# aksiksi/needle

Measured on AMD Instinct MI355X. Metric: episode-pairs/sec (analyze+search), higher is better.
Workload: dtype f64-certified (f32 first pass)

## Files before the change

include/needle_hip.h:

```cpp
#ifndef NEEDLE_HIP_H
#define NEEDLE_HIP_H

#include "needle.h"

#ifdef __cplusplus
extern "C" {
#endif

enum NeedleError needle_hip_device_count(int *count);
enum NeedleError needle_hip_set_device(int ordinal);
enum NeedleError needle_hip_synchronize(void);
enum NeedleError needle_hip_device_pci_bus_id(char out[32]);
void *needle_hip_stream(void);
const char *needle_hip_last_error_message(void);
const char *needle_hip_version(void);

enum NeedleError needle_hip_malloc(void **device_ptr, size_t bytes);
enum NeedleError needle_hip_free(void *device_ptr);
enum NeedleError needle_hip_memcpy_h2d(void *device_dst, const void *host_src, size_t bytes);
enum NeedleError needle_hip_memcpy_d2h(void *host_dst, const void *device_src, size_t bytes);
void needle_hip_host_free(void *ptr);
enum NeedleError needle_hip_host_alloc(void **host_ptr, size_t bytes);
enum NeedleError needle_hip_host_alloc_free(void *host_ptr);

double needle_hip_last_kernel_ms(const char *kernel);
void needle_hip_set_kernel_timing(const char *kernels);
size_t needle_hip_kernel_launches(const char *kernel);
enum NeedleError needle_hip_int_valu_ceiling(double *cells_per_second);
enum NeedleError needle_hip_scan_issued_evaluations(uint64_t *lane_evaluations, bool reset);
enum NeedleError needle_hip_scan_counts(uint64_t counts[2], bool reset);
enum NeedleError needle_hip_scan_last_launch(int32_t *form, uint64_t *matrix_products);
enum NeedleError needle_hip_epilogue_host_fallbacks(uint64_t *jobs, bool reset);

#define NEEDLE_HIP_MAX_CHANNELS 8
int needle_hip_fingerprint_sample_rate(void);
int needle_hip_fingerprint_delay_ms(void);
int needle_hip_fingerprint_item_duration_ms(void);
size_t needle_hip_fingerprint_num_items(size_t samples_per_channel);
size_t needle_hip_fingerprint_num_kept(size_t samples_per_channel, uint32_t step);

enum NeedleError needle_hip_fingerprint_host(const int16_t *const *pcm, const size_t *num_values,
                                             size_t num_streams, int channels, uint32_t step,
                                             uint32_t *const *items);

enum NeedleError needle_hip_fingerprint_device(const int16_t *d_pcm, const uint64_t *pcm_offsets,
                                               const uint64_t *num_values, size_t num_streams,
                                               int channels, uint32_t step, uint32_t *d_items,
                                               const uint64_t *item_offsets, bool sync);

enum NeedleError needle_hip_fingerprint_cert_stats(uint64_t counts[4], bool reset);

typedef struct NeedleHipCertAudit {
  uint64_t items, accepted, accepted_mismatches, mismatches;
  double max_error_over_s, max_s;
} NeedleHipCertAudit;
enum NeedleError needle_hip_fingerprint_audit_device(const int16_t *d_pcm, const uint64_t *pcm_offsets,
                                                     const uint64_t *num_values, size_t num_streams, int channels,
                                                     uint32_t step, const uint32_t *d_items, const uint64_t *item_offsets,
                                                     NeedleHipCertAudit *audit);

enum NeedleError needle_hip_fingerprint_debug(const int16_t *pcm, size_t num_values, int channels,
                                              double *chroma, double *features);

size_t needle_hip_resample_out_len(size_t samples_per_channel, int sample_rate);
enum NeedleError needle_hip_resample_host(const int16_t *const *pcm, const size_t *num_values, size_t num_streams,
                                          int channels, int sample_rate, int16_t *const *out);
enum NeedleHipResampleFamily {
  NEEDLE_HIP_RESAMPLE_IDENTITY = 0,
  NEEDLE_HIP_RESAMPLE_DEC = 1,
  NEEDLE_HIP_RESAMPLE_MFMA = 2,
  NEEDLE_HIP_RESAMPLE_QUAD = 3,
  NEEDLE_HIP_RESAMPLE_GENERAL = 4,
  NEEDLE_HIP_RESAMPLE_REFUSED = 5
};
typedef struct NeedleHipResamplePlan {
  int family;
  int L, M, T;
  int tile_outputs;
  int blocks_per_tile;
  int threads;
  int lds_bytes;
  int n;
  int row_mode;
  int rows_in_lds;
  int vec4;
  int groups;
  int pitch;
  int region_slots;
  int delta;
  int mfma_steps;
  int nblocks;
  int mf_splits, mf_waves, mf_groups;
  int mf_long_row;
  int mf_dup_lo, mf_dup_hi;
  int quad_splits, quads_per_split, quad_threads;
  int quad_rounds;
  int quad_small;
  int quad_steps;
  int dec_q;
} NeedleHipResamplePlan;
enum NeedleError needle_hip_resample_plan(int sample_rate, NeedleHipResamplePlan *out);
enum NeedleError needle_hip_downmix_host(const int16_t *const *pcm, const size_t *num_values, size_t num_streams,
                                         int channels, int16_t *const *out);

enum NeedleHipSampleFormat {
  NEEDLE_HIP_SAMPLE_U8 = 0,
  NEEDLE_HIP_SAMPLE_S16 = 1,
  NEEDLE_HIP_SAMPLE_S32 = 2,
  NEEDLE_HIP_SAMPLE_F32 = 3,
  NEEDLE_HIP_SAMPLE_F64 = 4,
  NEEDLE_HIP_SAMPLE_U8P = 5,
  NEEDLE_HIP_SAMPLE_S16P = 6,
  NEEDLE_HIP_SAMPLE_S32P = 7,
  NEEDLE_HIP_SAMPLE_F32P = 8,
// ... 61 lines not shown
  bool has_ending;
  uint64_t opening_start_ns, opening_end_ns;
  uint64_t ending_start_ns, ending_end_ns;
} NeedleHipSearchResult;

enum NeedleError needle_hip_comparator_run_with_frame_hashes(const struct NeedleAudioComparator *comparator,
                                                             const FrameHashes *const *frame_hashes,
                                                             size_t num_videos, bool display,
                                                             bool use_skip_files, bool write_skip_files,
                                                             NeedleHipSearchResult *results);

enum NeedleError needle_hip_comparator_results_from_runs(const struct NeedleAudioComparator *comparator,
                                                         const FrameHashes *const *frame_hashes, size_t num_videos,
                                                         const NeedleHipRun *runs, size_t num_runs, size_t first_video,
                                                         size_t video_count, NeedleHipSearchResult *results);

typedef struct NeedleHipIndex NeedleHipIndex;
enum NeedleError needle_hip_index_new(const struct NeedleAudioComparator *comparator, NeedleHipIndex **output);
void needle_hip_index_free(NeedleHipIndex *index);
size_t needle_hip_index_len(const NeedleHipIndex *index);
enum NeedleError needle_hip_index_add(NeedleHipIndex *index, const FrameHashes *const *frame_hashes, size_t k);
enum NeedleError needle_hip_index_results(const NeedleHipIndex *index, NeedleHipSearchResult *results, size_t n);
enum NeedleError needle_hip_index_pairs_searched(const NeedleHipIndex *index, uint64_t *total, uint64_t *last);
enum NeedleError needle_hip_index_remove(NeedleHipIndex *index, const size_t *positions, size_t k);
enum NeedleError needle_hip_index_replace(NeedleHipIndex *index, const size_t *positions, const FrameHashes *const *frame_hashes,
                                          size_t k);
enum NeedleError needle_hip_index_store_sizes(const NeedleHipIndex *index, uint64_t sizes[4]);

typedef struct NeedleHipLibrary NeedleHipLibrary;

enum NeedleError needle_hip_library_new(size_t num_videos, float opening_search_percentage, float hash_duration,
                                        NeedleHipLibrary **output);
void needle_hip_library_free(NeedleHipLibrary *library);
enum NeedleError needle_hip_library_include_endings(NeedleHipLibrary *library, float ending_search_percentage);
enum NeedleError needle_hip_library_set_sample_rate(NeedleHipLibrary *library, int sample_rate);
enum NeedleError needle_hip_library_set_sample_format(NeedleHipLibrary *library, int format);
size_t needle_hip_library_rows_per_video(const NeedleHipLibrary *library);
enum NeedleError needle_hip_library_set_pcm(NeedleHipLibrary *library, const int16_t *const *pcm,
                                            const size_t *num_values, int channels);
enum NeedleError needle_hip_library_set_pcm_device(NeedleHipLibrary *library, const int16_t *const *d_pcm,
                                                   const size_t *num_values, int channels);
enum NeedleError needle_hip_library_stream_pcm(NeedleHipLibrary *library, const int16_t *const *pcm,
                                               const size_t *num_values, int channels);
enum NeedleError needle_hip_library_analyze(NeedleHipLibrary *library, size_t first, size_t count, bool sync);
enum NeedleError needle_hip_library_hash_arena(NeedleHipLibrary *library, uint32_t **d_arena, size_t *stride);
enum NeedleError needle_hip_library_use_hash_arena(NeedleHipLibrary *library, uint32_t *d_arena, size_t rows,
                                                   size_t stride);
size_t needle_hip_library_num_pairs(const NeedleHipLibrary *library);
enum NeedleError needle_hip_library_search(NeedleHipLibrary *library, const struct NeedleAudioComparator *comparator,
                                           size_t first_pair, size_t num_pairs, NeedleHipRun *d_runs,
                                           uint32_t capacity, uint32_t *d_count, bool sync);
enum NeedleError needle_hip_library_fetch_runs_begin(NeedleHipLibrary *library, int slot, const NeedleHipRun *d_runs,
                                                     const uint32_t *d_count, uint32_t max_runs);
enum NeedleError needle_hip_library_fetch_runs_end(NeedleHipLibrary *library, int slot, const NeedleHipRun **runs,
                                                   uint32_t *num_runs);
enum NeedleError needle_hip_library_finalize(NeedleHipLibrary *library, const struct NeedleAudioComparator *comparator,
                                             const NeedleHipRun *runs, size_t num_runs,
                                             NeedleHipSearchResult *results);
enum NeedleError needle_hip_library_audit(NeedleHipLibrary *library, NeedleHipCertAudit *audit);
enum NeedleError needle_hip_library_frame_hashes(NeedleHipLibrary *library, size_t index, FrameHashes **output);

#define NEEDLE_HIP_COMM_ID_BYTES 128
enum NeedleError needle_hip_comm_create_id(uint8_t id[NEEDLE_HIP_COMM_ID_BYTES]);
enum NeedleError needle_hip_comm_init(const uint8_t id[NEEDLE_HIP_COMM_ID_BYTES], int rank, int world_size);
void needle_hip_comm_finalize(void);
int needle_hip_comm_rank(void);
int needle_hip_comm_world_size(void);
const char *needle_hip_comm_backend(void);
enum NeedleError needle_hip_comm_barrier(void);
enum NeedleError needle_hip_comm_all_gather_host(const void *send, void *recv, size_t bytes_per_rank);
void needle_hip_comm_shard(size_t units, int world_size, int rank, size_t *first, size_t *count);

enum NeedleError needle_hip_library_rank_videos(const NeedleHipLibrary *library, const size_t *num_values, int channels,
                                                int world_size, int rank, size_t *first_video, size_t *video_count);

enum NeedleError needle_hip_library_job_begin(NeedleHipLibrary *library, const struct NeedleAudioComparator *comparator,
                                              int slot);
enum NeedleError needle_hip_library_job_end(NeedleHipLibrary *library, const struct NeedleAudioComparator *comparator,
                                            int slot, NeedleHipSearchResult *results, size_t *num_runs);
enum NeedleError needle_hip_library_job_runs(const NeedleHipLibrary *library, int slot, const NeedleHipRun **runs,
                                             size_t *num_runs);
enum NeedleError needle_hip_library_job_comm_bytes(const NeedleHipLibrary *library, int slot, uint64_t bytes[4]);
enum NeedleError needle_hip_library_job_form(const NeedleHipLibrary *library, int slot, uint32_t form[4]);
int needle_hip_host_threads(void);

typedef struct NeedleHipFeeder NeedleHipFeeder;
enum NeedleError needle_hip_feeder_new(size_t lanes, int channels, int sample_rate, int format, uint32_t step,
                                       NeedleHipFeeder **output);
void needle_hip_feeder_free(NeedleHipFeeder *feeder);
enum NeedleError needle_hip_feeder_feed(NeedleHipFeeder *feeder, const void *const *pcm, const size_t *num_values);
enum NeedleError needle_hip_feeder_finish(NeedleHipFeeder *feeder, const size_t *lanes, size_t k);
enum NeedleError needle_hip_feeder_reset(NeedleHipFeeder *feeder, const size_t *lanes, size_t k);
enum NeedleError needle_hip_feeder_ready(NeedleHipFeeder *feeder, size_t lane, size_t *kept_items,
                                         uint64_t *samples_per_channel_fed, bool *finished);
enum NeedleError needle_hip_feeder_items(NeedleHipFeeder *feeder, size_t lane, size_t first, size_t count, uint32_t *items);
enum NeedleError needle_hip_feeder_frame_hashes(NeedleHipFeeder *feeder, size_t opening_lane, size_t ending_lane,
                                                uint64_t ending_seek_ns, float hash_duration, const char *md5, FrameHashes **output);
enum NeedleError needle_hip_feeder_state_bytes(const NeedleHipFeeder *feeder, uint64_t bytes[2]);
enum NeedleError needle_hip_feeder_set_audit(NeedleHipFeeder *feeder, bool on);
enum NeedleError needle_hip_feeder_audit(NeedleHipFeeder *feeder, size_t lane, NeedleHipCertAudit *audit);
size_t needle_hip_feeder_num_ready(uint64_t samples_per_channel_fed, int sample_rate, int channels, uint32_t step, bool finished);

typedef struct NeedleHipLaneFormat {
  int32_t channels;
  int32_t sample_rate;
  int32_t format;
} NeedleHipLaneFormat;
enum NeedleError needle_hip_feeder_new_lanes(const NeedleHipLaneFormat *formats, size_t lanes, uint32_t step, NeedleHipFeeder **output);
enum NeedleError needle_hip_feeder_lane_format(const NeedleHipFeeder *feeder, size_t lane, NeedleHipLaneFormat *format);
enum NeedleError needle_hip_feeder_reset_format(NeedleHipFeeder *feeder, const size_t *lanes, const NeedleHipLaneFormat *formats, size_t k);
enum NeedleError needle_hip_convert_mono_host(const void *const *pcm, const size_t *num_values, const NeedleHipLaneFormat *formats,
                                              size_t num_streams, int16_t *const *out);

typedef struct NeedleHipChannelMix {
  int32_t channels;
  int32_t coef[2][NEEDLE_HIP_MAX_CHANNELS];
} NeedleHipChannelMix;
enum NeedleError needle_hip_channel_mix_default(uint32_t channel_mask, NeedleHipChannelMix *out);
enum NeedleError needle_hip_rematrix_host(const void *const *pcm, const size_t *num_values, const NeedleHipLaneFormat *formats,
                                          const NeedleHipChannelMix *mixes, size_t num_streams, int16_t *const *out);
enum NeedleError needle_hip_analyzer_set_channel_mix(struct NeedleAudioAnalyzer *analyzer, const NeedleHipChannelMix *mix);
enum NeedleError needle_hip_analyzer_set_layout_downmix(struct NeedleAudioAnalyzer *analyzer, bool on);
enum NeedleError needle_hip_comparator_set_layout_downmix(struct NeedleAudioComparator *comparator, bool on);
enum NeedleError needle_hip_library_set_channel_mix(NeedleHipLibrary *library, const NeedleHipChannelMix *mix);
enum NeedleError needle_hip_feeder_set_lane_mix(NeedleHipFeeder *feeder, const size_t *lanes, const NeedleHipChannelMix *mixes, size_t k);

enum NeedleError needle_hip_feeder_switch_format(NeedleHipFeeder *feeder, const size_t *lanes, const NeedleHipLaneFormat *formats,
                                                 const NeedleHipChannelMix *mixes, size_t k);
typedef struct NeedleHipSegment {
  NeedleHipLaneFormat format;
  uint64_t frames;
} NeedleHipSegment;
enum NeedleError needle_hip_feeder_lane_segments(const NeedleHipFeeder *feeder, size_t lane, NeedleHipSegment *out, size_t cap, size_t *count);
size_t needle_hip_feeder_num_ready_segments(const NeedleHipSegment *segments, size_t count, uint32_t step, bool finished);

typedef struct NeedleHipMatcher NeedleHipMatcher;
enum NeedleError needle_hip_matcher_new(const uint32_t *hashes, size_t num_hashes, const NeedleHipSeq *sources,
                                        const uint32_t *min_len, size_t num_sources, size_t lanes, uint32_t threshold,
                                        NeedleHipMatcher **output);
void needle_hip_matcher_free(NeedleHipMatcher *matcher);
enum NeedleError needle_hip_matcher_feed(NeedleHipMatcher *matcher, const uint32_t *const *items, const size_t *num_items);
enum NeedleError needle_hip_matcher_feed_from_feeder(NeedleHipMatcher *matcher, NeedleHipFeeder *feeder);
enum NeedleError needle_hip_matcher_finish(NeedleHipMatcher *matcher, const size_t *lanes, size_t k);
enum NeedleError needle_hip_matcher_reset(NeedleHipMatcher *matcher, const size_t *lanes, size_t k);
enum NeedleError needle_hip_matcher_ready(NeedleHipMatcher *matcher, size_t lane, size_t *num_runs, uint64_t *items_fed,
                                          bool *finished);
enum NeedleError needle_hip_matcher_runs(NeedleHipMatcher *matcher, size_t lane, size_t first, size_t count, NeedleHipRun *runs);
enum NeedleError needle_hip_matcher_open(NeedleHipMatcher *matcher, size_t lane, NeedleHipRun **runs, size_t *num_runs);
enum NeedleError needle_hip_matcher_stats(const NeedleHipMatcher *matcher, uint64_t stats[4]);

typedef struct NeedleHipCrossMatcher NeedleHipCrossMatcher;
enum NeedleError needle_hip_crossmatcher_new(size_t lanes, size_t max_items, uint32_t min_len, uint32_t threshold,
                                             NeedleHipCrossMatcher **output);
enum NeedleError needle_hip_crossmatcher_new_regions(size_t videos, size_t regions, const size_t *max_items, const uint32_t *min_len,
                                                     uint32_t threshold, NeedleHipCrossMatcher **output);
enum NeedleError needle_hip_crossmatcher_new_resident(const uint32_t *hashes, size_t num_hashes, const NeedleHipSeq *resident,
                                                      size_t num_resident, size_t videos, size_t regions, const size_t *max_items,
                                                      const uint32_t *min_len, uint32_t threshold, NeedleHipCrossMatcher **output);
void needle_hip_crossmatcher_free(NeedleHipCrossMatcher *matcher);
enum NeedleError needle_hip_crossmatcher_feed(NeedleHipCrossMatcher *matcher, const uint32_t *const *items, const size_t *num_items);
enum NeedleError needle_hip_crossmatcher_feed_from_feeder(NeedleHipCrossMatcher *matcher, NeedleHipFeeder *feeder);
enum NeedleError needle_hip_crossmatcher_finish(NeedleHipCrossMatcher *matcher, const size_t *lanes, size_t k);
enum NeedleError needle_hip_crossmatcher_ready(NeedleHipCrossMatcher *matcher, size_t *num_runs, bool *complete);
enum NeedleError needle_hip_crossmatcher_lane(NeedleHipCrossMatcher *matcher, size_t lane, uint64_t *items_fed, bool *finished);
enum NeedleError needle_hip_crossmatcher_runs(NeedleHipCrossMatcher *matcher, size_t first, size_t count, NeedleHipRun *runs);
enum NeedleError needle_hip_crossmatcher_stats(const NeedleHipCrossMatcher *matcher, uint64_t stats[4]);
// ... 19 lines not shown
```

needle_amd/capi.py:

```python
from __future__ import annotations

import ctypes as C
import os
from dataclasses import dataclass
from typing import List, Optional, Sequence, Tuple

import numpy as np

NS = 1_000_000_000
LIB_PATH = os.environ.get("NEEDLE_CAPI_LIB") or os.path.join(os.path.dirname(os.path.abspath(__file__)), "lib", "libneedle_capi.so")

ERROR_NAMES = ["Ok", "InvalidUtf8String", "NullArgument", "InvalidArgument", "FrameHashDataNotFound",
               "FrameHashDataInvalidVersion", "InvalidFrameHashData", "ComparatorMinimumPaths",
               "AnalyzerInvalidHashPeriod", "AnalyzerInvalidHashDuration", "IOError", "Unknown"]

DEFAULT_HASH_MATCH_THRESHOLD = 10
DEFAULT_OPENING_SEARCH_PERCENTAGE = 0.50
DEFAULT_ENDING_SEARCH_PERCENTAGE = 0.25
DEFAULT_MIN_OPENING_DURATION = 20
DEFAULT_MIN_ENDING_DURATION = 20
DEFAULT_HASH_DURATION = 0.3
MAX_CHANNELS = 8


class NeedleError(RuntimeError):
    def __init__(self, code: int, detail: str = ""):
        self.code = code
        self.name = ERROR_NAMES[code] if 0 <= code < len(ERROR_NAMES) else str(code)
        super().__init__(f"NeedleError_{self.name}: {detail}")


class Seq(C.Structure):
    _fields_ = [("offset", C.c_uint32), ("len", C.c_uint32)]


class Problem(C.Structure):
    _fields_ = [("src_seq", C.c_uint32), ("dst_seq", C.c_uint32), ("min_len", C.c_uint32), ("tag", C.c_uint32)]


class Run(C.Structure):
    _fields_ = [("problem", C.c_uint32), ("src_end", C.c_uint32), ("dst_end", C.c_uint32), ("len", C.c_uint32),
                ("src_match_hash", C.c_uint32), ("dst_match_hash", C.c_uint32)]


class CSearchResult(C.Structure):
    _fields_ = [("has_result", C.c_bool), ("has_opening", C.c_bool), ("has_ending", C.c_bool),
                ("opening_start_ns", C.c_uint64), ("opening_end_ns", C.c_uint64),
                ("ending_start_ns", C.c_uint64), ("ending_end_ns", C.c_uint64)]


RUN_DTYPE = np.dtype([("problem", "<u4"), ("src_end", "<u4"), ("dst_end", "<u4"), ("len", "<u4"),
                      ("src_match_hash", "<u4"), ("dst_match_hash", "<u4")])
RUN_WORDS = 6

NEEDLE_H_SYMBOLS = [
    "needle_error_to_str", "needle_util_find_video_files", "needle_util_video_files_free",
    "needle_audio_analyzer_new_default", "needle_audio_analyzer_new", "needle_audio_analyzer_get_frame_hashes",
    "needle_audio_analyzer_free", "needle_audio_analyzer_print_paths", "needle_audio_analyzer_run",
    "needle_audio_comparator_new_default", "needle_audio_comparator_new", "needle_audio_comparator_free",
    "needle_audio_comparator_run"]
NEEDLE_HIP_H_SYMBOLS = [
    "needle_hip_device_count", "needle_hip_set_device", "needle_hip_synchronize", "needle_hip_stream",
    "needle_hip_device_pci_bus_id", "needle_hip_fingerprint_cert_stats", "needle_hip_scan_issued_evaluations",
    "needle_hip_last_error_message",
    "needle_hip_version", "needle_hip_malloc", "needle_hip_free", "needle_hip_memcpy_h2d", "needle_hip_memcpy_d2h",
    "needle_hip_host_free", "needle_hip_last_kernel_ms", "needle_hip_set_kernel_timing", "needle_hip_kernel_launches", "needle_hip_fingerprint_sample_rate",
    "needle_hip_fingerprint_delay_ms", "needle_hip_fingerprint_item_duration_ms", "needle_hip_fingerprint_num_items",
    "needle_hip_fingerprint_num_kept", "needle_hip_fingerprint_host", "needle_hip_fingerprint_device",
    "needle_hip_fingerprint_debug", "needle_hip_resample_out_len", "needle_hip_resample_host", "needle_hip_resample_plan",
    "needle_hip_downmix_host",
    "needle_hip_hamming_runs_device", "needle_hip_hamming_runs_host",
    "needle_hip_frame_hashes_new", "needle_hip_frame_hashes_free", "needle_hip_frame_hashes_len",
    "needle_hip_frame_hashes_copy", "needle_hip_frame_hashes_hash_duration_ns", "needle_hip_frame_hashes_md5",
    "needle_hip_frame_hashes_read", "needle_hip_frame_hashes_write", "needle_hip_header_md5",
    "needle_hip_analyzer_run_pcm", "needle_hip_comparator_run_with_frame_hashes", "needle_hip_library_new",
    "needle_hip_library_free", "needle_hip_library_include_endings", "needle_hip_library_set_sample_rate",
    "needle_hip_library_rows_per_video",
    "needle_hip_library_set_pcm", "needle_hip_library_set_pcm_device", "needle_hip_library_rank_videos",
    "needle_hip_library_analyze",
    "needle_hip_library_hash_arena", "needle_hip_library_use_hash_arena", "needle_hip_library_num_pairs", "needle_hip_library_search",
    "needle_hip_library_fetch_runs_begin", "needle_hip_library_fetch_runs_end",
    "needle_hip_library_finalize", "needle_hip_library_frame_hashes",
    "needle_hip_comm_create_id", "needle_hip_comm_init", "needle_hip_comm_finalize", "needle_hip_comm_rank",
    "needle_hip_comm_world_size", "needle_hip_comm_backend", "needle_hip_comm_barrier",
    "needle_hip_comm_all_gather_host", "needle_hip_comm_shard", "needle_hip_library_job_begin",
    "needle_hip_library_job_end", "needle_hip_library_stream_pcm", "needle_hip_host_alloc",
    "needle_hip_host_alloc_free", "needle_hip_int_valu_ceiling",
    "needle_hip_comparator_results_from_runs", "needle_hip_library_job_runs", "needle_hip_library_job_comm_bytes",
    "needle_hip_library_job_form",
    "needle_hip_host_threads", "needle_hip_fingerprint_audit_device", "needle_hip_library_audit",
    "needle_hip_scan_counts", "needle_hip_scan_last_launch", "needle_hip_epilogue_host_fallbacks",
    "needle_hip_index_new", "needle_hip_index_free", "needle_hip_index_len", "needle_hip_index_add",
    "needle_hip_index_results", "needle_hip_index_pairs_searched", "needle_hip_index_remove", "needle_hip_index_replace",
    "needle_hip_index_store_sizes", "needle_hip_index_crossmatcher_new", "needle_hip_index_add_matched",
    "needle_hip_index_pairs_scanned",
    "needle_hip_convert_host", "needle_hip_analyzer_run_pcm_format", "needle_hip_library_set_sample_format",
    "needle_hip_feeder_new", "needle_hip_feeder_free", "needle_hip_feeder_feed", "needle_hip_feeder_finish",
    "needle_hip_feeder_reset", "needle_hip_feeder_ready", "needle_hip_feeder_items", "needle_hip_feeder_frame_hashes",
    "needle_hip_feeder_state_bytes", "needle_hip_feeder_num_ready", "needle_hip_feeder_set_audit", "needle_hip_feeder_audit",
    "needle_hip_feeder_new_lanes", "needle_hip_feeder_lane_format", "needle_hip_feeder_reset_format", "needle_hip_convert_mono_host",
    "needle_hip_channel_mix_default", "needle_hip_rematrix_host", "needle_hip_analyzer_set_channel_mix",
    "needle_hip_analyzer_set_layout_downmix", "needle_hip_comparator_set_layout_downmix", "needle_hip_library_set_channel_mix",
    "needle_hip_feeder_set_lane_mix",
    "needle_hip_feeder_switch_format", "needle_hip_feeder_lane_segments", "needle_hip_feeder_num_ready_segments",
    "needle_hip_matcher_new", "needle_hip_matcher_free", "needle_hip_matcher_feed", "needle_hip_matcher_feed_from_feeder",
    "needle_hip_matcher_finish", "needle_hip_matcher_reset", "needle_hip_matcher_ready", "needle_hip_matcher_runs",
    "needle_hip_matcher_open", "needle_hip_matcher_stats",
    "needle_hip_crossmatcher_new", "needle_hip_crossmatcher_free", "needle_hip_crossmatcher_feed",
    "needle_hip_crossmatcher_feed_from_feeder", "needle_hip_crossmatcher_finish", "needle_hip_crossmatcher_ready",
    "needle_hip_crossmatcher_lane", "needle_hip_crossmatcher_runs", "needle_hip_crossmatcher_stats",
    "needle_hip_crossmatcher_state_bytes", "needle_hip_crossmatcher_new_regions",
    "needle_hip_crossmatcher_state_bytes_regions", "needle_hip_crossmatcher_shape",
    "needle_hip_crossmatcher_new_resident", "needle_hip_crossmatcher_state_bytes_resident", "needle_hip_crossmatcher_resident"]

SAMPLE_U8, SAMPLE_S16, SAMPLE_S32, SAMPLE_F32, SAMPLE_F64 = 0, 1, 2, 3, 4
SAMPLE_U8P, SAMPLE_S16P, SAMPLE_S32P, SAMPLE_F32P, SAMPLE_F64P = 5, 6, 7, 8, 9
_SAMPLE_DTYPES = [np.uint8, np.int16, np.int32, np.float32, np.float64]


def sample_format_dtype(sample_format: int):
    if not 0 <= sample_format <= 9:
        raise ValueError(f"unknown sample format {sample_format}")
    return np.dtype(_SAMPLE_DTYPES[sample_format % 5])


def sample_format_planar(sample_format: int) -> bool:
    return sample_format >= SAMPLE_U8P


def _format_pointers(pcm, channels: int, sample_format: int):
    dtype = sample_format_dtype(sample_format)
    keep, ptrs = [], []
    for p in pcm:
        if not sample_format_planar(sample_format):
            a = None if p is None else np.ascontiguousarray(p, dtype=dtype)
            keep.append(a)
            ptrs.append(None if a is None else a.ctypes.data)
        elif p is None:
            ptrs += [None] * channels
        else:
            planes = [np.ascontiguousarray(q, dtype=dtype) for q in p]
            if len(planes) != channels:
                raise ValueError(f"a planar stream needs {channels} planes, got {len(planes)}")
            keep += planes
            ptrs += [q.ctypes.data for q in planes]
    return keep, ptrs


class CLaneFormat(C.Structure):
    _fields_ = [("channels", C.c_int32), ("sample_rate", C.c_int32), ("format", C.c_int32)]


class CSegment(C.Structure):
    _fields_ = [("format", CLaneFormat), ("frames", C.c_uint64)]


class ChannelMix(C.Structure):
    _fields_ = [("channels", C.c_int32), ("coef", (C.c_int32 * MAX_CHANNELS) * 2)]

    @classmethod
    def of(cls, left: Sequence[int], right: Sequence[int], channels: Optional[int] = None) -> "ChannelMix":
        if len(left) != len(right) or len(left) > MAX_CHANNELS:
            raise ValueError(f"two rows of at most {MAX_CHANNELS} coefficients each")
        m = cls()
        m.channels = len(left) if channels is None else channels
        for c, (l, r) in enumerate(zip(left, right)):
            m.coef[0][c], m.coef[1][c] = int(l), int(r)
        return m

    def rows(self) -> Tuple[List[int], List[int]]:
        n = max(0, min(self.channels, MAX_CHANNELS))
        return list(self.coef[0][:n]), list(self.coef[1][:n])
# ... 220 lines not shown
    L.needle_hip_crossmatcher_runs.argtypes = [vp, sz, sz, vp]
    L.needle_hip_crossmatcher_stats.argtypes = [vp, C.POINTER(u64)]
    L.needle_hip_crossmatcher_state_bytes.argtypes = [sz, sz]
    L.needle_hip_crossmatcher_state_bytes.restype = sz
    L.needle_hip_crossmatcher_new_regions.argtypes = [sz, sz, C.POINTER(sz), C.POINTER(u32), u32, C.POINTER(vp)]
    L.needle_hip_crossmatcher_state_bytes_regions.argtypes = [sz, sz, C.POINTER(sz)]
    L.needle_hip_crossmatcher_state_bytes_regions.restype = sz
    L.needle_hip_crossmatcher_shape.argtypes = [vp, C.POINTER(sz), C.POINTER(sz)]
    L.needle_hip_crossmatcher_new_resident.argtypes = [vp, sz, vp, sz, sz, sz, C.POINTER(sz), C.POINTER(u32), u32, C.POINTER(vp)]
    L.needle_hip_crossmatcher_state_bytes_resident.argtypes = [vp, sz, sz, sz, C.POINTER(sz)]
    L.needle_hip_crossmatcher_state_bytes_resident.restype = sz
    L.needle_hip_crossmatcher_resident.argtypes = [vp, C.POINTER(sz)]
    _LIB = L
    return L


def check(code: int) -> None:
    if code != 0:
        raise NeedleError(code, (lib().needle_hip_last_error_message() or b"").decode(errors="replace"))


def error_to_str(code: int) -> str:
    return lib().needle_error_to_str(code).decode()


def device_count() -> int:
    n = C.c_int(0)
    check(lib().needle_hip_device_count(C.byref(n)))
    return n.value


def set_device(ordinal: int) -> None:
    check(lib().needle_hip_set_device(ordinal))


def device_pci_bus_id() -> str:
    buf = C.create_string_buffer(32)
    lib().needle_hip_device_pci_bus_id.argtypes = [C.c_char_p]
    check(lib().needle_hip_device_pci_bus_id(buf))
    return buf.value.decode()


def synchronize() -> None:
    check(lib().needle_hip_synchronize())


def stream_ptr() -> int:
    L = lib()
    L.needle_hip_stream.restype = C.c_void_p
    p = L.needle_hip_stream()
    if not p:
        raise RuntimeError("no HIP device: the library has no stream")
    return int(p)


def cert_stats(reset: bool = False) -> dict:
    v = (C.c_uint64 * 4)()
    lib().needle_hip_fingerprint_cert_stats.argtypes = [C.POINTER(C.c_uint64), C.c_bool]
    check(lib().needle_hip_fingerprint_cert_stats(v, reset))
    return {"items": int(v[0]), "items_recomputed": int(v[1]), "chunks": int(v[2]), "chunks_recomputed": int(v[3])}


def scan_issued_evaluations(reset: bool = False) -> int:
    v = C.c_uint64(0)
    lib().needle_hip_scan_issued_evaluations.argtypes = [C.POINTER(C.c_uint64), C.c_bool]
    check(lib().needle_hip_scan_issued_evaluations(C.byref(v), reset))
    return int(v.value)


def scan_counts(reset: bool = False) -> Tuple[int, int]:
    c = (C.c_uint64 * 2)()
    lib().needle_hip_scan_counts.argtypes = [C.POINTER(C.c_uint64), C.c_bool]
    check(lib().needle_hip_scan_counts(c, reset))
    return int(c[0]), int(c[1])


def scan_last_launch() -> Tuple[int, int]:
    form, products = C.c_int32(0), C.c_uint64(0)
    lib().needle_hip_scan_last_launch.argtypes = [C.POINTER(C.c_int32), C.POINTER(C.c_uint64)]
    check(lib().needle_hip_scan_last_launch(C.byref(form), C.byref(products)))
    return int(form.value), int(products.value)


def epilogue_host_fallbacks(reset: bool = False) -> int:
    jobs = C.c_uint64(0)
    lib().needle_hip_epilogue_host_fallbacks.argtypes = [C.POINTER(C.c_uint64), C.c_bool]
    check(lib().needle_hip_epilogue_host_fallbacks(C.byref(jobs), reset))
    return int(jobs.value)


def host_threads() -> int:
    lib().needle_hip_host_threads.restype = C.c_int
    return int(lib().needle_hip_host_threads())


def int_valu_ceiling() -> float:
    v = C.c_double(0.0)
    lib().needle_hip_int_valu_ceiling.argtypes = [C.POINTER(C.c_double)]
    check(lib().needle_hip_int_valu_ceiling(C.byref(v)))
    return v.value


def last_kernel_ms(name: str) -> float:
    return lib().needle_hip_last_kernel_ms(name.encode())


def kernel_launches(name: str) -> int:
    return int(lib().needle_hip_kernel_launches(name.encode()))


def set_kernel_timing(kernels: Optional[str]) -> None:
    lib().needle_hip_set_kernel_timing(kernels.encode() if kernels else None)


def _paths(paths: Sequence[str]):
    arr = (C.c_char_p * max(len(paths), 1))(*[p.encode() if isinstance(p, str) else p for p in paths])
    return C.cast(arr, C.POINTER(C.c_char_p)), arr


def header_md5(path: str) -> str:
    buf = C.create_string_buffer(33)
    check(lib().needle_hip_header_md5(path.encode(), buf))
    return buf.value.decode()


class FrameHashes:

    def __init__(self, handle: int, owned: bool, keepalive=None):
        self._h = C.c_void_p(handle)
        self._owned = owned
        self._keep = keepalive

    @staticmethod
    def new(opening: Sequence[Tuple[int, int]], ending: Sequence[Tuple[int, int]] = (), hash_duration_ns: int = 0,
            md5: str = "") -> "FrameHashes":
        oh = np.array([h for h, _ in opening], dtype=np.uint32)
        ot = np.array([t for _, t in opening], dtype=np.uint64)
        eh = np.array([h for h, _ in ending], dtype=np.uint32)
        et = np.array([t for _, t in ending], dtype=np.uint64)
        out = C.c_void_p()
        check(lib().needle_hip_frame_hashes_new(oh.ctypes.data, ot.ctypes.data, len(oh), eh.ctypes.data,
                                                et.ctypes.data, len(eh), hash_duration_ns, md5.encode(),
                                                C.byref(out)))
        return FrameHashes(out.value, True)

    @staticmethod
    def from_path(path: str) -> "FrameHashes":
        out = C.c_void_p()
        check(lib().needle_hip_frame_hashes_read(path.encode(), C.byref(out)))
        return FrameHashes(out.value, True)

    def write(self, path: str) -> None:
        check(lib().needle_hip_frame_hashes_write(self._h, path.encode()))

    def _data(self, ending: bool):
        n = lib().needle_hip_frame_hashes_len(self._h, ending)
        hashes = np.zeros(max(n, 1), dtype=np.uint32)
        ts = np.zeros(max(n, 1), dtype=np.uint64)
        check(lib().needle_hip_frame_hashes_copy(self._h, ending, hashes.ctypes.data, ts.ctypes.data, n))
        return hashes[:n], ts[:n]

    def opening_data(self):
        return self._data(False)

    def ending_data(self):
        return self._data(True)
# ... 880 lines not shown
        ptrs = (C.c_void_p * max(len(d_ptrs), self.n))(*[None if p is None else int(p) for p in d_ptrs])
        lens = (C.c_size_t * self.n)(*list(num_values))
        lib().needle_hip_library_set_pcm_device.argtypes = [C.c_void_p, C.POINTER(C.c_void_p), C.POINTER(C.c_size_t), C.c_int]
        check(lib().needle_hip_library_set_pcm_device(self._h, ptrs, lens, channels))

    def stream_pcm(self, pcm: Sequence[Optional[np.ndarray]], num_values: Sequence[int], channels: int = 1) -> None:
        arrs, ptrs = self._host_pointers(pcm, channels)
        lens = (C.c_size_t * self.n)(*list(num_values))
        check(lib().needle_hip_library_stream_pcm(self._h, ptrs, lens, channels))

    def analyze(self, first: int = 0, count: Optional[int] = None, sync: bool = True) -> None:
        check(lib().needle_hip_library_analyze(self._h, first, self.n - first if count is None else count, sync))

    def hash_arena(self) -> Tuple[int, int]:
        ptr = C.c_void_p()
        stride = C.c_size_t(0)
        check(lib().needle_hip_library_hash_arena(self._h, C.byref(ptr), C.byref(stride)))
        return ptr.value, stride.value

    def use_hash_arena(self, d_ptr: int, rows: int, stride: int) -> None:
        check(lib().needle_hip_library_use_hash_arena(self._h, d_ptr, rows, stride))

    def num_pairs(self) -> int:
        return lib().needle_hip_library_num_pairs(self._h)

    def search(self, comparator: Comparator, first_pair: int, num_pairs: int, d_runs: int, capacity: int,
               d_count: int, sync: bool = True) -> None:
        check(lib().needle_hip_library_search(self._h, comparator._h or comparator.handle(), first_pair, num_pairs,
                                              d_runs, capacity, d_count, sync))

    def fetch_runs_begin(self, slot: int, d_runs: int, d_count: int, max_runs: int) -> None:
        check(lib().needle_hip_library_fetch_runs_begin(self._h, slot, d_runs, d_count, max_runs))

    def fetch_runs_end(self, slot: int, max_runs: int) -> Tuple[np.ndarray, int]:
        ptr = C.c_void_p()
        total = C.c_uint32(0)
        check(lib().needle_hip_library_fetch_runs_end(self._h, slot, C.byref(ptr), C.byref(total)))
        k = min(total.value, max_runs)
        out = np.zeros(k, dtype=RUN_DTYPE)
        if k:
            C.memmove(out.ctypes.data, ptr.value, k * RUN_DTYPE.itemsize)
        return out, total.value

    def finalize(self, comparator: Comparator, runs: np.ndarray) -> List[Optional[SearchResult]]:
        runs = np.ascontiguousarray(runs, dtype=RUN_DTYPE)
        res = (CSearchResult * self.n)()
        check(lib().needle_hip_library_finalize(self._h, comparator._h or comparator.handle(), runs.ctypes.data,
                                                runs.size, res))
        return _results(res, self.n)

    def frame_hashes(self, index: int) -> FrameHashes:
        out = C.c_void_p()
        check(lib().needle_hip_library_frame_hashes(self._h, index, C.byref(out)))
        return FrameHashes(out.value, True)

    def job_begin(self, comparator: Comparator, slot: int = 0) -> None:
        check(lib().needle_hip_library_job_begin(self._h, comparator._h or comparator.handle(), slot))

    def job_end(self, comparator: Comparator, slot: int = 0) -> Tuple[List[Optional[SearchResult]], int]:
        res = (CSearchResult * self.n)()
        found = C.c_size_t(0)
        check(lib().needle_hip_library_job_end(self._h, comparator._h or comparator.handle(), slot, res, C.byref(found)))
        return _results(res, self.n), found.value

    def audit(self) -> dict:
        a = CCertAudit()
        lib().needle_hip_library_audit.argtypes = [C.c_void_p, C.POINTER(CCertAudit)]
        check(lib().needle_hip_library_audit(self._h, C.byref(a)))
        return a.as_dict()

    def job_runs(self, slot: int = 0) -> np.ndarray:
        ptr, total = C.c_void_p(), C.c_size_t(0)
        lib().needle_hip_library_job_runs.argtypes = [C.c_void_p, C.c_int, C.POINTER(C.c_void_p), C.POINTER(C.c_size_t)]
        check(lib().needle_hip_library_job_runs(self._h, slot, C.byref(ptr), C.byref(total)))
        out = np.zeros(total.value, dtype=RUN_DTYPE)
        if total.value:
            C.memmove(out.ctypes.data, ptr.value, out.nbytes)
        return out

    def job_form(self, slot: int = 0) -> dict:
        f = (C.c_uint32 * 4)()
        lib().needle_hip_library_job_form.argtypes = [C.c_void_p, C.c_int, C.POINTER(C.c_uint32)]
        check(lib().needle_hip_library_job_form(self._h, slot, f))
        return {"device_epilogue": bool(f[0]), "sharded_epilogue": bool(f[1]), "directed_runs": bool(f[2]), "scan_form": int(f[3])}

    def job_comm_bytes(self, slot: int = 0) -> dict:
        b = (C.c_uint64 * 4)()
        lib().needle_hip_library_job_comm_bytes.argtypes = [C.c_void_p, C.c_int, C.POINTER(C.c_uint64)]
        check(lib().needle_hip_library_job_comm_bytes(self._h, slot, b))
        return {"hash_rows": int(b[0]), "run_heads": int(b[1]), "results": int(b[2]), "scans_repeated": int(b[3])}

    def __del__(self):
        if getattr(self, "_h", None):
            lib().needle_hip_library_free(self._h)
            self._h = None


class PinnedArray:

    def __init__(self, count: int):
        p = C.c_void_p()
        check(lib().needle_hip_host_alloc(C.byref(p), max(count, 1) * 2))
        self.ptr = p.value
        self.array = np.ctypeslib.as_array((C.c_int16 * max(count, 1)).from_address(self.ptr))[:count]

    def __del__(self):
        if getattr(self, "ptr", None):
            self.array = None
            lib().needle_hip_host_alloc_free(self.ptr)
            self.ptr = None


class DeviceBuffer:

    def __init__(self, nbytes: int):
        p = C.c_void_p()
        check(lib().needle_hip_malloc(C.byref(p), nbytes))
        self.ptr = p.value
        self.nbytes = nbytes

    def to_host(self, dtype, count: int) -> np.ndarray:
        out = np.zeros(count, dtype=dtype)
        if count:
            check(lib().needle_hip_memcpy_d2h(out.ctypes.data, self.ptr, out.nbytes))
        return out

    def __del__(self):
        if getattr(self, "ptr", None):
            lib().needle_hip_free(self.ptr)
            self.ptr = None
```

needle_amd/csrc/capi.cpp:

```cpp
#include <dirent.h>
#include <hip/hip_runtime_api.h>
#include <sys/stat.h>

#include <algorithm>
#include <cstdio>
#include <cstdlib>
#include <chrono>
#include <cstring>
#include <fstream>
#include <new>

#include "crossmatch.h"
#include "epilogue.h"
#include "hipctx.h"
#include "feeder.h"
#include "index.h"
#include "matcher.h"
#include "needle_core.h"

using namespace needle;

struct FrameHashes {
  FrameHashesData d;
};
// ... 349 lines not shown

enum NeedleError needle_hip_malloc(void **device_ptr, size_t bytes) {
  if (!device_ptr) return NeedleError_NullArgument;
  return guarded([&]() -> NeedleError {
    Status s = ensure_device();
    if (!s.ok()) return report(s);
    if (hipMalloc(device_ptr, bytes ? bytes : 1) != hipSuccess)
      return report(Status::Make(NeedleError_Unknown, "hipMalloc failed for " + std::to_string(bytes) + " bytes"));
    return NeedleError_Ok;
  });
}

enum NeedleError needle_hip_free(void *device_ptr) {
  if (device_ptr && hipFree(device_ptr) != hipSuccess) return report(Status::Make(NeedleError_Unknown, "hipFree failed"));
  return NeedleError_Ok;
}

enum NeedleError needle_hip_memcpy_h2d(void *device_dst, const void *host_src, size_t bytes) {
  if (!device_dst || !host_src) return NeedleError_NullArgument;
  hipStream_t st = library_stream();
  if (hipMemcpyAsync(device_dst, host_src, bytes, hipMemcpyHostToDevice, st) != hipSuccess ||
      hipStreamSynchronize(st) != hipSuccess)
    return report(Status::Make(NeedleError_Unknown, "host-to-device copy failed"));
  return NeedleError_Ok;
}

enum NeedleError needle_hip_memcpy_d2h(void *host_dst, const void *device_src, size_t bytes) {
  if (!host_dst || !device_src) return NeedleError_NullArgument;
  hipStream_t st = library_stream();
  if (hipMemcpyAsync(host_dst, device_src, bytes, hipMemcpyDeviceToHost, st) != hipSuccess ||
      hipStreamSynchronize(st) != hipSuccess)
    return report(Status::Make(NeedleError_Unknown, "device-to-host copy failed"));
  return NeedleError_Ok;
}

void needle_hip_host_free(void *ptr) { std::free(ptr); }

enum NeedleError needle_hip_host_alloc(void **host_ptr, size_t bytes) {
  if (!host_ptr) return NeedleError_NullArgument;
  return guarded([&]() -> NeedleError {
    Status s = ensure_device();
    if (!s.ok()) return report(s);
    if (hipHostMalloc(host_ptr, bytes ? bytes : 1, hipHostMallocDefault) != hipSuccess)
      return report(Status::Make(NeedleError_Unknown, "pinned allocation of " + std::to_string(bytes) + " bytes failed"));
    return NeedleError_Ok;
  });
}

enum NeedleError needle_hip_host_alloc_free(void *host_ptr) {
  if (host_ptr && hipHostFree(host_ptr) != hipSuccess) return report(Status::Make(NeedleError_Unknown, "hipHostFree failed"));
  return NeedleError_Ok;
}

enum NeedleError needle_hip_fingerprint_cert_stats(uint64_t counts[4], bool reset) {
  if (!counts) return NeedleError_NullArgument;
  return guarded([&]() -> NeedleError {
    Status s = gpu_fingerprint_cert_stats(counts, reset);
    return s.ok() ? NeedleError_Ok : report(s);
  });
}

enum NeedleError needle_hip_scan_issued_evaluations(uint64_t *lane_evaluations, bool reset) {
  if (!lane_evaluations) return NeedleError_NullArgument;
  return guarded([&]() -> NeedleError {
    Status s = gpu_scan_issued_evaluations(lane_evaluations, reset);
    return s.ok() ? NeedleError_Ok : report(s);
  });
}

enum NeedleError needle_hip_scan_counts(uint64_t counts[2], bool reset) {
  if (!counts) return NeedleError_NullArgument;
  return guarded([&]() -> NeedleError {
    Status s = gpu_scan_issued_evaluations(&counts[0], reset, &counts[1]);
    return s.ok() ? NeedleError_Ok : report(s);
  });
}

enum NeedleError needle_hip_scan_last_launch(int32_t *form, uint64_t *matrix_products) {
  if (!form || !matrix_products) return NeedleError_NullArgument;
  gpu_scan_last_launch(form, matrix_products);
  return NeedleError_Ok;
}

enum NeedleError needle_hip_epilogue_host_fallbacks(uint64_t *jobs, bool reset) {
  if (!jobs) return NeedleError_NullArgument;
  *jobs = reset ? epilogue_host_fallbacks().exchange(0) : epilogue_host_fallbacks().load();
  return NeedleError_Ok;
}

enum NeedleError needle_hip_int_valu_ceiling(double *cells_per_second) {
  if (!cells_per_second) return NeedleError_NullArgument;
  return guarded([&]() -> NeedleError {
    Status s = gpu_int_valu_ceiling(cells_per_second);
    return s.ok() ? NeedleError_Ok : report(s);
  });
}

double needle_hip_last_kernel_ms(const char *kernel) { return kernel ? kernel_ms(kernel) : -1.0; }
void needle_hip_set_kernel_timing(const char *kernels) { set_kernel_timing(kernels); }
size_t needle_hip_kernel_launches(const char *kernel) { return kernel ? kernel_launches(kernel) : 0; }

int needle_hip_fingerprint_sample_rate(void) { return kSampleRate; }
int needle_hip_fingerprint_delay_ms(void) { return kDelayMs; }
int needle_hip_fingerprint_item_duration_ms(void) { return kItemDurationMs; }
size_t needle_hip_fingerprint_num_items(size_t samples_per_channel) { return num_items(samples_per_channel); }
size_t needle_hip_fingerprint_num_kept(size_t samples_per_channel, uint32_t step) {
  return num_kept(samples_per_channel, step);
}

enum NeedleError needle_hip_fingerprint_host(const int16_t *const *pcm, const size_t *num_values, size_t num_streams,
                                             int channels, uint32_t step, uint32_t *const *items) {
  if (!pcm || !num_values || !items) return NeedleError_NullArgument;
  return guarded([&]() -> NeedleError {
    std::vector<const int16_t *> p(pcm, pcm + num_streams);
    std::vector<size_t> n(num_values, num_values + num_streams);
    for (size_t i = 0; i < num_streams; i++)
      if ((!p[i] && n[i]) || !items[i]) return NeedleError_NullArgument;
    std::vector<std::vector<uint32_t>> out;
    Status s = gpu_fingerprint_host(p, n, channels, step, &out);
    if (!s.ok()) return report(s);
    for (size_t i = 0; i < num_streams; i++)
      if (!out[i].empty()) std::memcpy(items[i], out[i].data(), out[i].size() * sizeof(uint32_t));
    return NeedleError_Ok;
  });
}

enum NeedleError needle_hip_fingerprint_device(const int16_t *d_pcm, const uint64_t *pcm_offsets,
                                               const uint64_t *num_values, size_t num_streams, int channels,
                                               uint32_t step, uint32_t *d_items, const uint64_t *item_offsets,
                                               bool sync) {
  if (!d_pcm || !pcm_offsets || !num_values || !d_items || !item_offsets) return NeedleError_NullArgument;
  return guarded([&]() -> NeedleError {
    std::vector<StreamSpan> spans(num_streams);
    for (size_t i = 0; i < num_streams; i++) spans[i] = StreamSpan{pcm_offsets[i], num_values[i], item_offsets[i]};
    Status s = gpu_fingerprint_device(d_pcm, spans, channels, step, d_items, sync);
    return s.ok() ? NeedleError_Ok : report(s);
  });
}

enum NeedleError needle_hip_fingerprint_audit_device(const int16_t *d_pcm, const uint64_t *pcm_offsets, const uint64_t *num_values,
                                                     size_t num_streams, int channels, uint32_t step, const uint32_t *d_items,
                                                     const uint64_t *item_offsets, NeedleHipCertAudit *audit) {
  if (!d_pcm || !pcm_offsets || !num_values || !d_items || !item_offsets || !audit) return NeedleError_NullArgument;
  return guarded([&]() -> NeedleError {
    std::vector<StreamSpan> spans(num_streams);
    for (size_t i = 0; i < num_streams; i++) spans[i] = StreamSpan{pcm_offsets[i], num_values[i], item_offsets[i]};
    uint64_t c[4] = {0, 0, 0, 0};
    Status s = gpu_fingerprint_audit_device(d_pcm, spans, channels, step, d_items, c, &audit->max_error_over_s, &audit->max_s);
    if (!s.ok()) return report(s);
    audit->items = c[0];
    audit->accepted = c[1];
    audit->accepted_mismatches = c[2];
    audit->mismatches = c[3];
    return NeedleError_Ok;
  });
}

enum NeedleError needle_hip_fingerprint_debug(const int16_t *pcm, size_t num_values, int channels, double *chroma,
                                              double *features) {
  if (!pcm) return NeedleError_NullArgument;
  return guarded([&]() -> NeedleError {
    Status s = ensure_device();
    if (!s.ok()) return report(s);
    if (channels != 1 && channels != 2) return NeedleError_InvalidArgument;
    const size_t samples = num_values / (size_t)channels;
    const size_t frames = num_frames(samples), rows = frames >= 5 ? frames - 4 : 0, kept = num_items(samples);
// ... 867 lines not shown
```

needle_amd/csrc/common.h:

```cpp
#pragma once

#include <cstddef>
#include <cstdint>
#include <functional>
#include <string>
#include <vector>

#include "../../include/needle_hip.h"

struct ihipStream_t;

namespace needle {

struct Status {
  NeedleError code = NeedleError_Ok;
  std::string message;
  bool ok() const { return code == NeedleError_Ok; }
  static Status Ok() { return Status{}; }
  static Status Make(NeedleError c, std::string m) { return Status{c, std::move(m)}; }
};

NeedleError report(const Status &s);
void set_last_error(const std::string &m);
const char *last_error();
// ... 21 lines not shown

Status frame_hashes_read(const std::string &path, FrameHashesData *out);
Status frame_hashes_write(const std::string &path, const FrameHashesData &fh);
Status header_md5(const std::string &path, std::string *out);
std::string md5_hex(const uint8_t *data, size_t n);
std::string with_extension(const std::string &path, const std::string &ext);
std::string format_time(ns_t t);
std::string format_f32_json(float v);

unsigned usable_cpus();
unsigned host_threads();
void set_node_ranks(unsigned ranks);

constexpr int kSampleRate = 11025;
constexpr int kFrameSize = 4096;
constexpr int kHop = 1365;
constexpr int kBands = 12;
constexpr int kFirTaps = 5;
constexpr int kMaxFilterWidth = 16;
constexpr int kItemLatency = (kFirTaps - 1) + (kMaxFilterWidth - 1);
constexpr int kDelayMs = 2600;
constexpr int kItemDurationMs = 123;

inline size_t num_frames(size_t samples) { return samples < (size_t)kFrameSize ? 0 : (samples - kFrameSize) / kHop + 1; }
inline size_t num_items(size_t samples) {
  size_t f = num_frames(samples);
  return f > (size_t)kItemLatency ? f - kItemLatency : 0;
}
inline size_t num_kept(size_t samples, uint32_t step) {
  size_t n = num_items(samples);
  return step ? (n + step - 1) / step : 0;
}

bool step_for_hash_duration(ns_t hash_duration, uint32_t *step);
void attach_timestamps(const uint32_t *kept, size_t n_kept, uint32_t step, bool has_seek, ns_t seek_to,
                       std::vector<HashTs> *out);

struct WavData {
  int channels = 0;
  int sample_rate = 0;
  std::vector<int16_t> pcm;
};
Status wav_read(const std::string &path, WavData *out);
struct WavInfo {
  int channels = 0, sample_rate = 0;
  int format = 0, bits = 0;
  uint32_t channel_mask = 0;
  uint64_t data_offset = 0;
  uint64_t frames = 0;
};
Status wav_probe(const std::string &path, WavInfo *out);
Status wav_read_frames(const std::string &path, const WavInfo &info, uint64_t first, uint64_t count, int16_t *dst);

struct StreamSpan {
  uint64_t pcm_off;
  uint64_t num_values;
  uint64_t item_off;
};

Status gpu_fingerprint_device(const int16_t *d_pcm, const std::vector<StreamSpan> &streams, int channels,
                              uint32_t step, uint32_t *d_items, bool sync, double *d_chroma_dbg = nullptr,
                              double *d_feat_dbg = nullptr, size_t descriptor_slot = 0, int pipe = -1,
                              uint32_t *zero_word = nullptr, bool *zeroed = nullptr);
Status gpu_fingerprint_streamed_device(const std::vector<const int16_t *> &pcm, const std::vector<size_t> &num_values,
                                       int channels, uint32_t step, uint32_t *d_items,
                                       const std::vector<uint64_t> &item_off, int rate = kSampleRate);
Status gpu_fingerprint_host(const std::vector<const int16_t *> &pcm, const std::vector<size_t> &num_values,
                            int channels, uint32_t step, std::vector<std::vector<uint32_t>> *items,
                            int rate = kSampleRate);
using PcmReader = std::function<Status(size_t stream, uint64_t first_value, uint64_t num_values, int16_t *dst)>;
using StreamIssued = std::function<Status(size_t stream_index)>;
Status gpu_upload_pcm_streamed(const std::vector<size_t> &num_values, const std::vector<uint64_t> &dev_off,
                               const PcmReader &read, unsigned readers, int16_t *d_pcm, ::ihipStream_t *stream = nullptr,
                               const StreamIssued &issued = nullptr);
Status gpu_upload_pcm(const std::vector<const int16_t *> &pcm, const std::vector<size_t> &num_values,
                      const std::vector<uint64_t> &dev_off, int16_t *d_pcm, ::ihipStream_t *stream = nullptr,
                      const StreamIssued &issued = nullptr);
Status gpu_fingerprint_streamed(const std::vector<size_t> &num_values, const PcmReader &read, unsigned readers,
                                int channels, uint32_t step, std::vector<std::vector<uint32_t>> *items,
                                int rate = kSampleRate, const NeedleHipChannelMix *mix = nullptr);
Status gpu_hamming_runs_device(const uint32_t *d_hashes, const NeedleHipSeq *seqs, size_t num_seqs,
                               const NeedleHipProblem *problems, size_t num_problems, uint32_t threshold,
                               NeedleHipRun *d_runs, uint32_t capacity, uint32_t *d_count, bool sync,
                               bool count_is_zero = false);
Status gpu_hamming_runs_host(const uint32_t *hashes, size_t num_hashes, const NeedleHipSeq *seqs, size_t num_seqs,
                             const NeedleHipProblem *problems, size_t num_problems, uint32_t threshold,
                             std::vector<NeedleHipRun> *runs);

uint32_t *gpu_pinned_arena_acquire(size_t words);
void gpu_pinned_arena_release(uint32_t *arena);
void gpu_prefetch_hashes(const uint32_t *hashes, size_t num_hashes);

constexpr uint64_t kDeviceEpiloguePairs = 1u << 14;
constexpr uint32_t kDeviceEpilogueRuns = 1u << 14;

Status gpu_int_valu_ceiling(double *cells_per_second);
Status gpu_scan_issued_evaluations(uint64_t *lane_evaluations, bool reset, uint64_t *head_survivors = nullptr);
void gpu_scan_last_launch(int32_t *form, uint64_t *matrix_products);
Status gpu_fingerprint_cert_stats(uint64_t out[4], bool reset);
Status gpu_fingerprint_audit_device(const int16_t *d_pcm, const std::vector<StreamSpan> &spans, int channels, uint32_t step,
                                    const uint32_t *d_items, uint64_t out[4], double *max_ratio, double *max_sigma);

struct FeedLane {
  uint64_t pcm_off;
  uint64_t item_off;
  uint32_t row_base;
  uint32_t carried;
  uint32_t frames;
  uint32_t first_item;
  uint32_t kept;
  uint32_t lane;
};
constexpr size_t kFeedAuditWords = 6;
struct FeedAudit {
  double *rows64;
  uint64_t *counts;
};
Status gpu_fingerprint_feed_device(const int16_t *d_pcm, const std::vector<FeedLane> &lanes, int channels, uint32_t step,
                                   double *d_chroma, float *d_energy, double *d_chroma64, uint32_t *d_items,
                                   const FeedAudit *audit = nullptr);
bool gpu_fingerprint_f64_mode();

struct ResampleSpan {
  uint64_t in_off;
  uint64_t n_in;
  uint64_t out_off;
  const int16_t *src = nullptr;
  uint64_t t0 = 0, t1 = 0;
  uint64_t p0 = 0, p1 = 0;
};
size_t resample_out_len(size_t n_in, int rate);
struct ResampleTiling {
  int L = 1, M = 1, half = 0;
  uint64_t tile_outputs = 1;
};
Status resample_tiling(int rate, int channels, ResampleTiling *out);
Status resample_tiling_host(int rate, ResampleTiling *out);
Status resample_plan_host(int rate, NeedleHipResamplePlan *out);
void resample_piece(const ResampleTiling &t, uint64_t n_in, uint64_t t0, uint64_t t1, uint64_t *p0, uint64_t *p1);
Status gpu_resample_device(const int16_t *d_in, const std::vector<ResampleSpan> &spans, int channels, int rate,
                           int16_t *d_out, bool sync);
Status gpu_resample_host(const std::vector<const int16_t *> &pcm, const std::vector<size_t> &num_values, int channels,
                         int rate, std::vector<std::vector<int16_t>> *out);

struct DownmixSpan {
  const int16_t *src;
  int16_t *dst;
  uint64_t frames;
};
Status gpu_downmix_device(const std::vector<DownmixSpan> &spans, int channels, bool sync);
Status gpu_downmix_host(const std::vector<const int16_t *> &pcm, const std::vector<size_t> &num_values, int channels,
                        const std::vector<int16_t *> &out);

inline bool sample_format_valid(int format) { return format >= NEEDLE_HIP_SAMPLE_U8 && format <= NEEDLE_HIP_SAMPLE_F64P; }
inline bool sample_format_planar(int format) { return format >= NEEDLE_HIP_SAMPLE_U8P; }
inline size_t sample_format_width(int format) {
  constexpr size_t width[5] = {1, 2, 4, 4, 8};
  return width[format % 5];
}
inline size_t sample_format_planes(int format, int channels) { return sample_format_planar(format) ? (size_t)channels : 1; }
inline uint64_t sample_plane_units(uint64_t samples, size_t width) { return ((samples * width + 15) & ~(uint64_t)15) / 2; }
struct ConvertSpan {
  const void *src[NEEDLE_HIP_MAX_CHANNELS];
  int16_t *dst;
  uint64_t frames;
};
Status gpu_convert_device(const std::vector<ConvertSpan> &spans, int channels, int format, bool mix, bool sync);
Status gpu_upload_raw(const std::vector<const void *> &src, const std::vector<size_t> &bytes, const std::vector<uint64_t> &dev_off,
                      int16_t *d_raw, ::ihipStream_t *stream = nullptr, const StreamIssued &issued = nullptr);
Status gpu_fingerprint_host_format(const std::vector<const void *> &pcm, const std::vector<size_t> &num_values, int channels,
                                   int format, uint32_t step, std::vector<std::vector<uint32_t>> *items, int rate = kSampleRate,
                                   const NeedleHipChannelMix *mix = nullptr);
Status gpu_fingerprint_streamed_device_format(const std::vector<const void *> &pcm, const std::vector<size_t> &num_values,
                                              int channels, int format, uint32_t step, uint32_t *d_items,
                                              const std::vector<uint64_t> &item_off, int rate = kSampleRate,
                                              const NeedleHipChannelMix *mix = nullptr);
Status gpu_convert_host(const std::vector<const void *> &pcm, const std::vector<size_t> &num_values, int channels, int format,
                        const std::vector<int16_t *> &out);

struct IngestSpan {
  const void *src[NEEDLE_HIP_MAX_CHANNELS];
// ... 16 lines not shown
```

needle_amd/csrc/library.cpp:

```cpp
#include <hip/hip_runtime_api.h>

#include <algorithm>
#include <chrono>
#include <cstdio>
#include <cstdlib>
#include <cstring>
#include <map>
#include <new>
#include <tuple>

#include "comm.h"
#include "epilogue.h"
#include "hipctx.h"
#include "needle_core.h"

struct FrameHashes;
struct NeedleAudioComparator;

namespace needle {
const Comparator &comparator_of(const NeedleAudioComparator *c);
FrameHashes *make_frame_hashes(FrameHashesData &&d);
void fill_c_result(const VideoResult &v, NeedleHipSearchResult *r);
}

using namespace needle;

namespace {
struct Window {
  size_t values = 0;
  uint64_t pcm_off = ~0ull;
  uint32_t kept = 0;
  ns_t seek = 0;
};
}

struct NeedleHipLibrary {
  size_t n = 0;
  float opening_pct = DEFAULT_OPENING_SEARCH_PERCENTAGE;
  float ending_pct = DEFAULT_ENDING_SEARCH_PERCENTAGE;
  bool endings = false;
  ns_t hash_duration = 0;
  uint32_t step = 0;
  int channels = 1;
  int rate = kSampleRate;
  int format = NEEDLE_HIP_SAMPLE_S16;
  bool has_mix = false;
  NeedleHipChannelMix mix{};
  bool have_pcm = false;
  bool pcm_resident = false;
  std::vector<Window> win;
  size_t stride = 0;
  DeviceBuffer<int16_t> d_pcm;
  DeviceBuffer<uint32_t> d_arena;
  uint32_t *arena = nullptr;
  std::vector<std::vector<HashTs>> ts_cache;
  std::vector<uint32_t> min_len;
  ns_t min_len_for[2] = {~0ull, ~0ull};
  std::vector<NeedleHipProblem> problems;
  size_t problems_for[3] = {~(size_t)0, 0, 0};
  std::vector<FrameHashesData> shells;
  std::vector<uint32_t> shell_of;
  struct Fetch {
    void *host = nullptr;
    uint32_t max_runs = 0;
    hipEvent_t ready = nullptr, done = nullptr;
    const NeedleHipRun *d_runs = nullptr;
    const uint32_t *d_count = nullptr;
    bool pending = false;
  } fetch[2];
  struct Job {
    DeviceBuffer<uint8_t> d_slabs;
    DeviceBuffer<uint8_t> d_heads;
    uint32_t slab_runs = 0, head_runs = 0;
    int world = 0;
    void *host = nullptr;
    size_t host_bytes = 0;
    hipEvent_t searched = nullptr, done = nullptr;
    bool pending = false;
    std::vector<NeedleHipRun> merged;
    void *host_results = nullptr;
    size_t host_results_bytes = 0;
    bool device_epilogue = false, sharded = false;
    bool shape_fixed = false;
    const NeedleHipRun *last_runs = nullptr;
    size_t last_total = 0;
    DeviceBuffer<uint8_t> d_dir_send, d_dir_recv;
    DeviceBuffer<uint32_t> d_dir_counts;
    void *host_counts = nullptr;
    size_t host_counts_bytes = 0;
    std::vector<uint32_t> cap;
    bool ran_device_epilogue = false, ran_sharded = false;
    uint32_t scan_form = 0;
    bool counted = false;
    bool directed = false;
    std::vector<NeedleHipRun> fetched;
    bool fetched_valid = false;
    static size_t count_words(int world) { return ((size_t)world + 1 + 3) & ~(size_t)3; }
    uint64_t comm_bytes[4] = {0, 0, 0, 0};
    size_t slab_bytes() const { return kSlabHeader + (size_t)slab_runs * sizeof(NeedleHipRun); }
    size_t head_bytes() const { return kSlabHeader + (size_t)head_runs * sizeof(NeedleHipRun); }
  } job[2];
  static constexpr size_t kSlabHeader = 32;
  uint32_t slab_runs = 0;
  uint32_t last_max_count = 0;
  std::vector<uint32_t> dir_counts;
  int dir_world = 0;
  bool dir_unsupported = false;
  bool dir_cap_forced = false;
  size_t arena_rows = 0;
  const uint32_t *count_zeroed = nullptr;
  std::vector<uint32_t> row_len, row_ts;
  std::vector<uint64_t> row_seek, ts_tables;
  void ensure_row_tables() {
    if (row_len.size() == rows()) return;
    row_len.assign(rows(), 0);
    row_ts.assign(rows(), 0);
    row_seek.assign(rows(), 0);
    ts_tables.clear();
    std::map<uint32_t, uint32_t> offset_of;
    for (size_t row = 0; row < rows(); row++) {
      const Window &w = win[row];
      auto it = offset_of.find(w.kept);
      if (it == offset_of.end()) {
        it = offset_of.emplace(w.kept, (uint32_t)ts_tables.size()).first;
        for (const HashTs &h : timestamps(w.kept)) ts_tables.push_back(h.ts);
      }
      row_len[row] = w.kept;
      row_ts[row] = it->second;
      row_seek[row] = w.seek;
    }
  }
  ~NeedleHipLibrary() {
    for (Fetch &f : fetch) {
      if (f.host) (void)hipHostFree(f.host);
      if (f.done) (void)hipEventDestroy(f.done);
      if (f.ready) (void)hipEventDestroy(f.ready);
    }
    for (Job &j : job) {
      if (j.host_results) (void)hipHostFree(j.host_results);
      if (j.host_counts) (void)hipHostFree(j.host_counts);
      if (j.host) (void)hipHostFree(j.host);
      if (j.done) (void)hipEventDestroy(j.done);
      if (j.searched) (void)hipEventDestroy(j.searched);
    }
  }

  size_t regions() const { return endings ? 2 : 1; }
  size_t rows() const { return n * regions(); }
  size_t flat_block(int world) const { return rows() * stride / (size_t)std::max(world, 1); }
  bool flat_shardable(int world) const { return world <= 1 || (stride % 64 == 0 && (rows() * (stride / 64)) % (size_t)world == 0); }
  void ensure_shells() {
    if (shell_of.size() == n) return;
    shells.clear();
    shell_of.assign(n, 0);
    const size_t R = regions();
    std::map<std::tuple<uint32_t, ns_t, uint32_t, ns_t>, uint32_t> seen;
    for (size_t v = 0; v < n; v++) {
      const Window &wo = win[v * R];
      const Window we = endings ? win[v * R + 1] : Window{};
      const auto key = std::make_tuple(wo.kept, wo.seek, we.kept, we.seek);
      auto it = seen.find(key);
      if (it == seen.end()) {
        FrameHashesData d;
        d.opening = window_timestamps(wo);
        if (endings) d.ending = window_timestamps(we);
        d.hash_duration = hash_duration;
        it = seen.emplace(key, (uint32_t)shells.size()).first;
        shells.push_back(std::move(d));
      }
      shell_of[v] = it->second;
    }
  }
  std::vector<const FrameHashesData *> shell_pointers() {
    ensure_shells();
    std::vector<const FrameHashesData *> fh(n);
    for (size_t v = 0; v < n; v++) fh[v] = &shells[shell_of[v]];
    return fh;
  }

  const std::vector<HashTs> &timestamps(uint32_t k) {
    if (ts_cache.size() <= k) ts_cache.resize(k + 1);
    if (ts_cache[k].empty() && k) {
      std::vector<uint32_t> zeros(k, 0);
      attach_timestamps(zeros.data(), k, step, false, 0, &ts_cache[k]);
    }
    return ts_cache[k];
  }
// ... 86 lines not shown
}

namespace {
Status check_mix_channels(const NeedleHipLibrary *lib, int channels) {
  return lib->has_mix ? channel_mix_check(lib->mix, channels) : Status::Ok();
}

size_t resident_samples(size_t count, int rate) { return rate == kSampleRate ? count : resample_out_len(count, rate); }

Status plan_windows(NeedleHipLibrary *lib, const void *const *pcm, const size_t *num_values, int channels, bool resident,
                    std::vector<const void *> *src, std::vector<size_t> *len, std::vector<uint64_t> *dst,
                    std::vector<uint64_t> *rows_of_src, uint64_t *total_values) {
  Status s = ensure_device();
  if (!s.ok()) return s;
  const bool resampled = lib->rate != kSampleRate, converted = lib->format != NEEDLE_HIP_SAMPLE_S16 || lib->has_mix;
  const size_t planes = sample_format_planes(lib->format, channels), width = sample_format_width(lib->format);
  for (size_t v = 0; v < lib->n; v++)
    for (size_t c = 1; c < planes; c++)
      if (!pcm[v * planes + c] != !pcm[v * planes])
        return Status::Make(NeedleError_NullArgument, "video " + std::to_string(v) + " has NULL and non-NULL planes");
  lib->channels = channels > 2 || resampled || lib->has_mix ? 1 : channels;
  const size_t R = lib->regions();
  lib->win.assign(lib->rows(), Window{});
  uint64_t total = 0;
  uint32_t max_kept = 0;
  std::vector<size_t> first_sample(lib->rows(), 0), source_samples(lib->rows(), 0);
  for (size_t v = 0; v < lib->n; v++) {
    const size_t samples = num_values[v] / (size_t)channels;
    size_t open_samples = 0, end_first = 0;
    ns_t seek = 0;
    s = Analyzer::windows(samples, lib->rate, lib->opening_pct, lib->ending_pct, &open_samples, &end_first, &seek);
    if (!s.ok()) return s;
    for (size_t r = 0; r < R; r++) {
      Window &w = lib->win[v * R + r];
      const size_t count = r == 0 ? open_samples : samples - end_first;
      const size_t kept_samples = resident_samples(count, lib->rate);
      first_sample[v * R + r] = r == 0 ? 0 : end_first;
      source_samples[v * R + r] = count;
      w.values = kept_samples * (size_t)lib->channels;
      w.kept = (uint32_t)num_kept(kept_samples, lib->step);
      w.seek = r == 0 ? 0 : seek;
      max_kept = std::max(max_kept, w.kept);
      if (pcm[v * planes] && resident) {
        w.pcm_off = total;
        total += channels > 2 || resampled || converted ? (w.values + 7) & ~(uint64_t)7 : (w.values + 1) & ~(uint64_t)1;
      }
    }
  }
  size_t tiles_per_row = std::max<size_t>(1, ((size_t)max_kept + 63) / 64);
  while (comm_world() > 1 && (lib->rows() * tiles_per_row) % (size_t)comm_world()) tiles_per_row++;
  size_t stride = 64 * tiles_per_row;
  const size_t arena_rows = lib->rows();
  if ((uint64_t)arena_rows * stride > UINT32_MAX || (uint64_t)pair_count(lib->n) * R > UINT32_MAX)
    return Status::Make(NeedleError_InvalidArgument, "library too large for one job: more than 2^32 arena hashes or sequence pairs");
  const bool own_arena = lib->arena == lib->d_arena.ptr;
  if (!lib->arena || (own_arena && (stride != lib->stride || arena_rows != lib->arena_rows))) {
    if (!(s = lib->d_arena.reserve(arena_rows * stride)).ok()) return s;
    lib->arena = lib->d_arena.ptr;
    lib->arena_rows = arena_rows;
    lib->stride = stride;
    if (hipMemsetAsync(lib->arena, 0, arena_rows * stride * sizeof(uint32_t), library_stream()) != hipSuccess)
      return Status::Make(NeedleError_Unknown, "hipMemset failed");
  } else if (!own_arena && (stride > lib->stride || arena_rows > lib->arena_rows)) {
    return Status::Make(NeedleError_InvalidArgument, "the adopted hash arena is too small for these videos");
  }
  for (size_t v = 0; v < lib->n; v++) {
    for (size_t r = 0; r < R; r++) {
      const Window &w = lib->win[v * R + r];
      if (!pcm[v * planes] || !w.values) continue;
      for (size_t c = 0; c < planes; c++)
        src->push_back(static_cast<const uint8_t *>(pcm[v * planes + c]) +
                       first_sample[v * R + r] * (planes == 1 ? (size_t)channels : 1) * width);
      len->push_back(source_samples[v * R + r] * (size_t)channels);
      if (dst) dst->push_back(w.pcm_off);
      if (rows_of_src) rows_of_src->push_back(v * R + r);
    }
  }
  if (total_values) *total_values = total;
  lib->min_len.clear();
  lib->row_len.clear();
  lib->shells.clear();
  lib->shell_of.clear();
  lib->problems_for[0] = ~(size_t)0;
  return Status::Ok();
}

Status upload_mixed(NeedleHipLibrary *lib, const std::vector<const int16_t *> &src, const std::vector<size_t> &len,
                    const std::vector<uint64_t> &dst, int channels, DeviceBuffer<int16_t> *stage) {
  uint64_t max_values = 1ull << 30;
  if (const char *e = getenv("NEEDLE_HIP_MAX_BATCH_VALUES")) max_values = (uint64_t)std::max(1ll, atoll(e));
  const uint64_t C = (uint64_t)channels;
  const uint64_t piece = std::max<uint64_t>(8, max_values / C / 8 * 8);
  uint64_t total = 0;
  for (size_t l : len) total += (l + 7) & ~(uint64_t)7;
  const uint64_t cap = std::max<uint64_t>(std::min(total, max_values), 8 * C) + 8;
  Status s = stage->reserve(cap);
  if (!s.ok()) return s;
  std::vector<const int16_t *> up_src;
  std::vector<size_t> up_len;
  std::vector<uint64_t> up_off;
  std::vector<DownmixSpan> mix;
  uint64_t used = 0;
  auto flush = [&]() -> Status {
    Status fs = up_src.empty() ? Status::Ok() : gpu_upload_pcm(up_src, up_len, up_off, stage->ptr);
    if (fs.ok() && !mix.empty()) fs = gpu_downmix_device(mix, channels, false);
    up_src.clear();
    up_len.clear();
    up_off.clear();
    mix.clear();
    used = 0;
    return fs;
  };
  for (size_t i = 0; i < src.size(); i++) {
    const uint64_t frames = len[i] / C;
    for (uint64_t f = 0; f < frames; f += piece) {
      const uint64_t n = std::min(piece, frames - f), values = (n * C + 7) & ~(uint64_t)7;
      if (used + values > cap && !(s = flush()).ok()) return s;
      up_src.push_back(src[i] + f * C);
      up_len.push_back(n * C);
      up_off.push_back(used);
      mix.push_back(DownmixSpan{stage->ptr + used, lib->d_pcm.ptr + dst[i] + f, n});
      used += values;
    }
  }
  return flush();
}

Status upload_resampled(NeedleHipLibrary *lib, const std::vector<const int16_t *> &src, const std::vector<size_t> &len,
                        const std::vector<uint64_t> &dst, int channels, bool from_host, DeviceBuffer<int16_t> *stage) {
  const int rate = lib->rate, rs_channels = channels > 2 ? 1 : channels;
  const uint64_t C = (uint64_t)channels;
  ResampleTiling tl;
  Status s = resample_tiling(rate, rs_channels, &tl);
  if (!s.ok()) return s;
  if (!from_host && channels <= 2) {
    std::vector<ResampleSpan> spans;
    for (size_t i = 0; i < src.size(); i++) {
      ResampleSpan sp{0, len[i] / C, dst[i]};
      sp.src = src[i];
      spans.push_back(sp);
    }
    return gpu_resample_device(nullptr, spans, channels, rate, lib->d_pcm.ptr, false);
  }
  uint64_t max_values = 1ull << 30;
  if (const char *e = getenv("NEEDLE_HIP_MAX_BATCH_VALUES")) max_values = (uint64_t)std::max(1ll, atoll(e));
  const uint64_t per_sample = (from_host ? C : 0) + (channels > 2 ? 1 : 0);
  const uint64_t tile_in = tl.tile_outputs * (uint64_t)tl.M / (uint64_t)tl.L + 2 * (uint64_t)tl.half + 16;
  const uint64_t budget = std::max(max_values / per_sample, tile_in);
  const uint64_t piece_tiles = std::max<uint64_t>(1, (budget - 2 * (uint64_t)tl.half - 16) * (uint64_t)tl.L /
                                                         (tl.tile_outputs * (uint64_t)tl.M));
  auto staged = [&](uint64_t samples) {
    return (from_host ? (samples * C + 7) & ~(uint64_t)7 : 0) + (channels > 2 ? (samples + 7) & ~(uint64_t)7 : 0);
  };
  struct Piece {
    size_t i;
    uint64_t t0, t1, p0, p1;
  };
  std::vector<Piece> pieces;
  uint64_t total = 0, largest = 0;
  for (size_t i = 0; i < src.size(); i++) {
    const uint64_t n_in = len[i] / C, tiles = (resample_out_len(n_in, rate) + tl.tile_outputs - 1) / tl.tile_outputs;
    for (uint64_t t0 = 0; t0 < tiles; t0 += piece_tiles) {
      Piece pc{i, t0, std::min(tiles, t0 + piece_tiles), 0, 0};
      resample_piece(tl, n_in, pc.t0, pc.t1, &pc.p0, &pc.p1);
      pieces.push_back(pc);
      total += staged(pc.p1 - pc.p0);
// ... 296 lines not shown
}

enum NeedleError needle_hip_library_hash_arena(NeedleHipLibrary *lib, uint32_t **d_arena, size_t *stride) {
  if (!lib || !d_arena || !stride) return NeedleError_NullArgument;
  if (!lib->have_pcm) return NeedleError_InvalidArgument;
  *d_arena = lib->arena;
  *stride = lib->stride;
  return NeedleError_Ok;
}

size_t needle_hip_library_rows_per_video(const NeedleHipLibrary *lib) { return lib ? lib->regions() : 0; }

enum NeedleError needle_hip_library_use_hash_arena(NeedleHipLibrary *lib, uint32_t *d_arena, size_t rows, size_t stride) {
  if (!lib || !d_arena) return NeedleError_NullArgument;
  if (!lib->have_pcm || rows < lib->rows() || stride < lib->stride) return NeedleError_InvalidArgument;
  if ((uint64_t)rows * stride > UINT32_MAX) return NeedleError_InvalidArgument;
  lib->arena = d_arena;
  lib->arena_rows = rows;
  lib->stride = stride;
  lib->d_arena.release();
  return NeedleError_Ok;
}

size_t needle_hip_library_num_pairs(const NeedleHipLibrary *lib) { return lib ? pair_count(lib->n) : 0; }

enum NeedleError needle_hip_library_search(NeedleHipLibrary *lib, const struct NeedleAudioComparator *comparator,
                                           size_t first_pair, size_t num_pairs, NeedleHipRun *d_runs,
                                           uint32_t capacity, uint32_t *d_count, bool sync) {
  if (!lib || !comparator || !d_runs || !d_count) return NeedleError_NullArgument;
  const size_t np = pair_count(lib->n);
  if (!lib->have_pcm || first_pair > np || num_pairs > np - first_pair) return NeedleError_InvalidArgument;
  return guarded([&]() -> NeedleError {
    const auto t_enter = std::chrono::steady_clock::now();
    const Comparator &cmp = comparator_of(comparator);
    if (cmp.include_endings() && !lib->endings)
      return report(Status::Make(NeedleError_Unknown, "no ending hash data present"));
    const size_t R = lib->regions(), Rc = cmp.include_endings() ? 2 : 1;
    std::vector<NeedleHipSeq> seqs(lib->rows());
    for (size_t row = 0; row < lib->rows(); row++)
      seqs[row] = NeedleHipSeq{(uint32_t)(row * lib->stride), lib->win[row].kept};
    if (lib->min_len.size() != lib->rows() || lib->min_len_for[0] != cmp.min_opening_duration() ||
        lib->min_len_for[1] != cmp.min_ending_duration()) {
      lib->min_len.assign(lib->rows(), 0);
      for (size_t row = 0; row < lib->rows(); row++) {
        const bool opening = row % R == 0;
        lib->min_len[row] = row >= R && lib->win[row].kept == lib->win[row - R].kept
                                ? lib->min_len[row - R]
                                : cmp.min_run_length_for(lib->timestamps(lib->win[row].kept), opening);
      }
      lib->min_len_for[0] = cmp.min_opening_duration();
      lib->min_len_for[1] = cmp.min_ending_duration();
      lib->problems_for[0] = ~(size_t)0;
    }
    std::vector<NeedleHipProblem> &problems = lib->problems;
    const bool cached = lib->problems_for[0] == first_pair && lib->problems_for[1] == num_pairs && lib->problems_for[2] == Rc;
    if (!cached) {
      lib->problems_for[0] = ~(size_t)0;
      problems.clear();
      problems.reserve(num_pairs * Rc);
      size_t i = 0, j = 0;
      if (num_pairs) pair_at(lib->n, first_pair, &i, &j);
      for (size_t p = first_pair; p < first_pair + num_pairs; p++) {
        for (size_t r = 0; r < Rc; r++) {
          if (r == 1 && (lib->win[i * R + 1].kept == 0 || lib->win[j * R + 1].kept == 0))
            return report(Status::Make(NeedleError_Unknown, "no ending hash data present"));
          const uint32_t a = lib->min_len[i * R + r], b = lib->min_len[j * R + r];
          if (a == 0 || b == 0) continue;
          problems.push_back(NeedleHipProblem{(uint32_t)(i * R + r), (uint32_t)(j * R + r), std::max(a, b),
                                              (uint32_t)(p * Rc + r)});
        }
        if (++j == lib->n) j = ++i + 1;
      }
      lib->problems_for[0] = first_pair;
      lib->problems_for[1] = num_pairs;
      lib->problems_for[2] = Rc;
    }
    for (NeedleHipLibrary::Fetch &f : lib->fetch)
      if (f.pending && (f.d_runs == d_runs || f.d_count == d_count) &&
          hipStreamWaitEvent(library_stream(), f.done, 0) != hipSuccess)
        return report(Status::Make(NeedleError_Unknown, "stream wait failed"));
    const auto t_built = std::chrono::steady_clock::now();
    const bool count_is_zero = lib->count_zeroed == d_count;
    lib->count_zeroed = nullptr;
    Status s = gpu_hamming_runs_device(lib->arena, seqs.data(), seqs.size(), problems.data(), problems.size(),
                                       cmp.hash_match_threshold(), d_runs, capacity, d_count, sync, count_is_zero);
    if (getenv("NEEDLE_HIP_TRACE"))
      std::fprintf(stderr, "[needle_hip] search enqueue: %zu problems built in %.2f ms, launched in %.2f ms\n",
                   problems.size(), std::chrono::duration<double, std::milli>(t_built - t_enter).count(),
                   std::chrono::duration<double, std::milli>(std::chrono::steady_clock::now() - t_built).count());
    return s.ok() ? NeedleError_Ok : report(s);
  });
}

enum NeedleError needle_hip_library_fetch_runs_begin(NeedleHipLibrary *lib, int slot, const NeedleHipRun *d_runs,
                                                     const uint32_t *d_count, uint32_t max_runs) {
  if (!lib || !d_runs || !d_count) return NeedleError_NullArgument;
  if (slot < 0 || slot > 1 || max_runs == 0) return NeedleError_InvalidArgument;
  return guarded([&]() -> NeedleError {
    NeedleHipLibrary::Fetch &f = lib->fetch[slot];
    if (f.pending) return report(Status::Make(NeedleError_InvalidArgument, "fetch slot still pending"));
    const size_t bytes = 16 + (size_t)max_runs * sizeof(NeedleHipRun);
    if (f.max_runs < max_runs) {
      if (f.host) (void)hipHostFree(f.host);
      f.host = nullptr;
      if (hipHostMalloc(&f.host, bytes, hipHostMallocDefault) != hipSuccess)
        return report(Status::Make(NeedleError_Unknown, "pinned allocation failed"));
      f.max_runs = max_runs;
    }
    if (!f.done && hipEventCreateWithFlags(&f.done, hipEventDisableTiming) != hipSuccess)
      return report(Status::Make(NeedleError_Unknown, "event creation failed"));
    if (!f.ready && hipEventCreateWithFlags(&f.ready, hipEventDisableTiming) != hipSuccess)
      return report(Status::Make(NeedleError_Unknown, "event creation failed"));
    hipStream_t stream = library_stream(), down = download_stream();
    if (hipEventRecord(f.ready, stream) != hipSuccess || hipStreamWaitEvent(down, f.ready, 0) != hipSuccess ||
        hipMemcpyAsync(f.host, d_count, sizeof(uint32_t), hipMemcpyDeviceToHost, down) != hipSuccess ||
        hipMemcpyAsync(static_cast<char *>(f.host) + 16, d_runs, (size_t)max_runs * sizeof(NeedleHipRun),
                       hipMemcpyDeviceToHost, down) != hipSuccess ||
        hipEventRecord(f.done, down) != hipSuccess)
      return report(Status::Make(NeedleError_Unknown, "asynchronous run download failed"));
    f.d_runs = d_runs;
    f.d_count = d_count;
    f.pending = true;
    return NeedleError_Ok;
  });
}

enum NeedleError needle_hip_library_fetch_runs_end(NeedleHipLibrary *lib, int slot, const NeedleHipRun **runs,
                                                   uint32_t *num_runs) {
  if (!lib || !runs || !num_runs) return NeedleError_NullArgument;
  if (slot < 0 || slot > 1 || !lib->fetch[slot].pending) return NeedleError_InvalidArgument;
  return guarded([&]() -> NeedleError {
    NeedleHipLibrary::Fetch &f = lib->fetch[slot];
    if (hipEventSynchronize(f.done) != hipSuccess) return report(Status::Make(NeedleError_Unknown, "run download failed"));
    f.pending = false;
    *num_runs = *static_cast<const uint32_t *>(f.host);
    *runs = reinterpret_cast<const NeedleHipRun *>(static_cast<const char *>(f.host) + 16);
    return NeedleError_Ok;
  });
}

enum NeedleError needle_hip_library_finalize(NeedleHipLibrary *lib, const struct NeedleAudioComparator *comparator,
                                             const NeedleHipRun *runs, size_t num_runs,
                                             NeedleHipSearchResult *results) {
  if (!lib || !comparator || (!runs && num_runs) || !results) return NeedleError_NullArgument;
  if (!lib->have_pcm) return NeedleError_InvalidArgument;
  return guarded([&]() -> NeedleError {
    const Comparator &cmp = comparator_of(comparator);
    const std::vector<const FrameHashesData *> fh = lib->shell_pointers();
    std::vector<VideoResult> res;
    const auto t0 = std::chrono::steady_clock::now();
    Status s = cmp.results_from_runs(fh, runs, num_runs, false, false, false, &res);
    if (getenv("NEEDLE_HIP_TRACE"))
      std::fprintf(stderr, "[needle_hip] epilogue %zu runs: %.1f us\n", num_runs,
                   std::chrono::duration<double, std::micro>(std::chrono::steady_clock::now() - t0).count());
    if (!s.ok()) return report(s);
    for (size_t v = 0; v < lib->n; v++) fill_c_result(res[v], &results[v]);
    return NeedleError_Ok;
  });
}

enum NeedleError needle_hip_library_frame_hashes(NeedleHipLibrary *lib, size_t index, FrameHashes **output) {
  if (!lib || !output) return NeedleError_NullArgument;
  if (!lib->have_pcm || index >= lib->n) return NeedleError_InvalidArgument;
  return guarded([&]() -> NeedleError {
    const size_t R = lib->regions();
    FrameHashesData fh;
    hipStream_t stream = library_stream();
    for (size_t r = 0; r < R; r++) {
      const Window &w = lib->win[index * R + r];
      std::vector<uint32_t> host(w.kept);
      if (!host.empty() &&
          (hipMemcpyAsync(host.data(), lib->arena + (index * R + r) * lib->stride, host.size() * sizeof(uint32_t),
                          hipMemcpyDeviceToHost, stream) != hipSuccess ||
           hipStreamSynchronize(stream) != hipSuccess))
        return report(Status::Make(NeedleError_Unknown, "hash arena download failed"));
      std::vector<HashTs> ts = lib->window_timestamps(w);
      for (size_t k = 0; k < host.size(); k++) ts[k].hash = host[k];
      (r == 0 ? fh.opening : fh.ending) = std::move(ts);
    }
    fh.hash_duration = lib->hash_duration;
    *output = make_frame_hashes(std::move(fh));
    return NeedleError_Ok;
  });
}

}

namespace {

template <typename F>
void for_rows_of_block(const NeedleHipLibrary *lib, int world, int rank, F &&f) {
  const size_t B = lib->flat_block(world), begin = (size_t)rank * B, end = begin + B;
  if (!lib->stride) return;
  for (size_t row = begin / lib->stride; row < lib->rows() && row * lib->stride < end; row++) {
    const size_t r0 = row * lib->stride;
    const size_t c0 = begin > r0 ? begin - r0 : 0, c1 = std::min<size_t>(std::min(end - r0, lib->stride), lib->win[row].kept);
    if (c0 < c1) f(row, c0, c1);
  }
}

Status block_spans(const NeedleHipLibrary *lib, int world, int rank, std::vector<StreamSpan> *spans) {
  if (world <= 1) {
    for (size_t row = 0; row < lib->rows(); row++) {
      const Window &w = lib->win[row];
      if (w.pcm_off == ~0ull)
        return Status::Make(NeedleError_InvalidArgument, "video " + std::to_string(row / lib->regions()) + " has no PCM on this rank");
      spans->push_back(StreamSpan{w.pcm_off, w.values, (uint64_t)row * lib->stride});
    }
    return Status::Ok();
  }
  Status bad;
  for_rows_of_block(lib, world, rank, [&](size_t row, size_t c0, size_t c1) {
    const Window &w = lib->win[row];
    if (w.pcm_off == ~0ull) {
      bad = Status::Make(NeedleError_InvalidArgument, "video " + std::to_string(row / lib->regions()) +
                                                          " has no PCM on this rank (needle_hip_library_rank_videos names the videos a rank needs)");
      return;
    }
    const uint64_t x0 = (uint64_t)c0 * lib->step, frames = (uint64_t)(c1 - 1 - c0) * lib->step + 20;
    const uint64_t samples = (frames - 1) * (uint64_t)kHop + (uint64_t)kFrameSize;
    spans->push_back(StreamSpan{w.pcm_off + x0 * (uint64_t)kHop * (uint64_t)lib->channels, samples * (uint64_t)lib->channels,
                                (uint64_t)row * lib->stride + c0});
  });
  return bad;
}

NeedleError analyze_flat_block(NeedleHipLibrary *lib, int world, int rank, int slot, uint32_t *zero_word) {
  std::vector<StreamSpan> spans;
  bool zeroed = false;
  lib->count_zeroed = nullptr;
  Status s = block_spans(lib, world, rank, &spans);
  if (!s.ok()) return report(s);
  if (spans.empty()) return NeedleError_Ok;
  s = gpu_fingerprint_device(lib->d_pcm.ptr, spans, lib->channels, lib->step, lib->arena, false, nullptr, nullptr, 0, slot,
                             zero_word, &zeroed);
  if (s.ok() && zeroed) lib->count_zeroed = zero_word;
  return s.ok() ? NeedleError_Ok : report(s);
}

uint32_t round_up4(uint64_t v) { return (uint32_t)std::min<uint64_t>((v + 3) & ~(uint64_t)3, 0xfffffffcu); }

Status job_buffers(NeedleHipLibrary *lib, NeedleHipLibrary::Job &j, int world) {
  if (!j.searched) NEEDLE_HIP_TRY(hipEventCreateWithFlags(&j.searched, hipEventDisableTiming));
  if (!j.done) NEEDLE_HIP_TRY(hipEventCreateWithFlags(&j.done, hipEventDisableTiming));
  if (j.slab_runs != lib->slab_runs || j.world != world) {
    j.slab_runs = lib->slab_runs;
    j.world = world;
    j.d_slabs.release();
    Status s = j.d_slabs.reserve(j.slab_bytes());
    if (!s.ok()) return s;
  }
  uint32_t head = lib->last_max_count ? round_up4((uint64_t)lib->last_max_count + lib->last_max_count / 8 + 64) : 4096u;
  const char *forced = lib->last_max_count ? nullptr : getenv("NEEDLE_HIP_HEAD_RUNS");
  if (forced) head = round_up4((uint64_t)std::max(4, atoi(forced)));
  head = std::min(head, j.slab_runs);
  if (!forced && j.slab_bytes() * (size_t)world <= (1u << 20)) head = j.slab_runs;
  j.head_runs = head;
  const size_t want = j.head_bytes() * (size_t)world;
  if (world > 1) {
    Status s = j.d_heads.reserve(want);
    if (!s.ok()) return s;
  }
  if (want > j.host_bytes) {
    if (j.host) (void)hipHostFree(j.host);
    j.host = nullptr;
    j.host_bytes = 0;
    NEEDLE_HIP_TRY(hipHostMalloc(&j.host, want + want / 4, hipHostMallocDefault));
    j.host_bytes = want + want / 4;
  }
  return Status::Ok();
}

bool device_epilogue_wanted(const NeedleHipLibrary *lib, size_t comparator_regions) {
  if (const char *e = getenv("NEEDLE_HIP_DEVICE_EPILOGUE")) return atoi(e) != 0;
  return (uint64_t)pair_count(lib->n) * comparator_regions >= kDeviceEpiloguePairs || lib->last_max_count >= kDeviceEpilogueRuns;
}

Status fetch_directed(NeedleHipLibrary::Job &j, int world, int rank) {
  if (j.fetched_valid) return Status::Ok();
  const size_t W = (size_t)world, cw = NeedleHipLibrary::Job::count_words(world);
  const uint32_t *m = static_cast<const uint32_t *>(j.host_counts);
  size_t total = 0, off = 0;
  for (size_t r = 0; r < W; r++) total += std::min(m[r * cw + 1 + (size_t)rank], j.cap[r * W + (size_t)rank]);
  j.fetched.resize(total);
  size_t at = 0;
  for (size_t r = 0; r < W; r++) {
    const uint32_t cap = j.cap[r * W + (size_t)rank], have = std::min(m[r * cw + 1 + (size_t)rank], cap);
    if (have)
      NEEDLE_HIP_TRY(hipMemcpyAsync(j.fetched.data() + at, j.d_dir_recv.ptr + off + NeedleHipLibrary::kSlabHeader,
                                    (size_t)have * sizeof(NeedleHipRun), hipMemcpyDeviceToHost, download_stream()));
    at += have;
    off += NeedleHipLibrary::kSlabHeader + (size_t)cap * sizeof(NeedleHipRun);
  }
  NEEDLE_HIP_TRY(hipStreamSynchronize(download_stream()));
  j.fetched_valid = true;
  return Status::Ok();
}

NeedleError job_search_and_gather(NeedleHipLibrary *lib, const NeedleAudioComparator *comparator, NeedleHipLibrary::Job &j) {
  const int world = comm_world(), rank = comm_rank();
  size_t pfirst = 0, pcount = 0;
  shard_range(pair_count(lib->n), world, rank, &pfirst, &pcount);
  uint8_t *mine = j.d_slabs.ptr;
  NeedleError e = needle_hip_library_search(lib, comparator, pfirst, pcount,
                                            reinterpret_cast<NeedleHipRun *>(mine + NeedleHipLibrary::kSlabHeader), j.slab_runs,
                                            reinterpret_cast<uint32_t *>(mine), false);
  if (e != NeedleError_Ok) return e;
  {
    int32_t form = 0;
    uint64_t products = 0;
    gpu_scan_last_launch(&form, &products);
    j.scan_form = (uint32_t)form;
  }
  hipStream_t stream = library_stream(), down = download_stream();
  if (hipEventRecord(j.searched, stream) != hipSuccess || hipStreamWaitEvent(down, j.searched, 0) != hipSuccess)
    return report(Status::Make(NeedleError_Unknown, "stream ordering failed"));
  const Comparator &cmp = comparator_of(comparator);
  const size_t Rc = cmp.include_endings() ? 2 : 1;
  j.device_epilogue = device_epilogue_wanted(lib, Rc) && lib->n >= 2;
  j.shape_fixed = j.device_epilogue;
  if (j.device_epilogue) {
    uint64_t shard_from = 1u << 16;
    if (const char *e = getenv("NEEDLE_HIP_SHARD_EPILOGUE_PAIRS")) shard_from = (uint64_t)std::max(1, atoi(e));
    j.sharded = world > 1 && (getenv("NEEDLE_HIP_SHARD_EPILOGUE") ? atoi(getenv("NEEDLE_HIP_SHARD_EPILOGUE")) != 0
                                                                   : (uint64_t)pair_count(lib->n) * Rc >= shard_from);
  }
  j.counted = j.directed = false;
  j.cap.clear();
  j.fetched_valid = false;
  const char *dir_env = getenv("NEEDLE_HIP_DIRECTED_RUNS");
  const bool want_directed = world > 1 && world <= 64 && j.device_epilogue && j.sharded && !lib->dir_unsupported &&
                             !(dir_env && atoi(dir_env) == 0);
  std::vector<size_t> recv_off((size_t)world, 0), recv_bytes((size_t)world, 0);
  if (want_directed) {
    const size_t W = (size_t)world;
    const bool have = lib->dir_world == world && lib->dir_counts.size() == W * W;
    std::vector<uint32_t> cap(W * W, 0u);
    if (have)
      for (size_t k = 0; k < W * W; k++) cap[k] = round_up4((uint64_t)lib->dir_counts[k] + lib->dir_counts[k] / 8 + 64);
    if (const char *e = getenv("NEEDLE_HIP_TEST_DIRECTED_CAP"))
      if (have && !lib->dir_cap_forced) {
        std::fill(cap.begin(), cap.end(), round_up4((uint64_t)std::max(4, atoi(e))));
        lib->dir_cap_forced = true;
      }
    DirectPlan plan;
    std::memset(&plan, 0, sizeof(plan));
    std::vector<size_t> send_off(W), send_bytes(W);
    size_t off = 0, largest = 0;
    for (size_t q = 0; q < W; q++) {
      plan.offset[q] = (uint32_t)off;
      plan.capacity[q] = cap[(size_t)rank * W + q];
      send_off[q] = off;
      send_bytes[q] = NeedleHipLibrary::kSlabHeader + (size_t)plan.capacity[q] * sizeof(NeedleHipRun);
      off += send_bytes[q];
    }
    for (size_t k = 0; k < W * W; k++) largest = std::max(largest, NeedleHipLibrary::kSlabHeader + (size_t)cap[k] * sizeof(NeedleHipRun));
    if (off >= 0xFFFFFFF0ull) return report(Status::Make(NeedleError_InvalidArgument, "directed run exchange: blocks beyond 4 GiB"));
    const size_t cw = NeedleHipLibrary::Job::count_words(world);
    Status s = j.d_dir_send.reserve(off);
    if (s.ok()) s = j.d_dir_counts.reserve(cw * W);
    if (s.ok() && cw * W * sizeof(uint32_t) > j.host_counts_bytes) {
      if (j.host_counts) (void)hipHostFree(j.host_counts);
      j.host_counts = nullptr;
      j.host_counts_bytes = 0;
      if (hipHostMalloc(&j.host_counts, cw * W * sizeof(uint32_t), hipHostMallocDefault) != hipSuccess)
        s = Status::Make(NeedleError_Unknown, "pinned allocation failed");
      else
        j.host_counts_bytes = cw * W * sizeof(uint32_t);
    }
    if (s.ok())
      s = gpu_direct_runs(reinterpret_cast<const uint32_t *>(mine), reinterpret_cast<const NeedleHipRun *>(mine + NeedleHipLibrary::kSlabHeader),
                          j.slab_runs, (uint32_t)lib->n, (uint32_t)Rc, (uint32_t)shard_block(lib->n, world), world, j.d_dir_send.ptr, plan, down);
    if (!s.ok()) return report(s);
    uint32_t *row = j.d_dir_counts.ptr + (size_t)rank * cw;
    bool ok = hipMemsetAsync(row, 0, cw * sizeof(uint32_t), down) == hipSuccess &&
              hipMemcpyAsync(row, mine, sizeof(uint32_t), hipMemcpyDeviceToDevice, down) == hipSuccess;
    for (size_t q = 0; q < W && ok; q++)
      ok = hipMemcpyAsync(row + 1 + q, j.d_dir_send.ptr + send_off[q], sizeof(uint32_t), hipMemcpyDeviceToDevice, down) == hipSuccess;
    if (!ok) return report(Status::Make(NeedleError_Unknown, "directed run exchange: count row failed"));
    s = comm_all_gather(kSide, row, j.d_dir_counts.ptr, cw * sizeof(uint32_t), down);
    if (!s.ok()) return report(s);
    if (hipMemcpyAsync(j.host_counts, j.d_dir_counts.ptr, cw * W * sizeof(uint32_t), hipMemcpyDeviceToHost, down) != hipSuccess)
      return report(Status::Make(NeedleError_Unknown, "directed run exchange: count download failed"));
    j.counted = true;
    j.comm_bytes[1] += cw * W * sizeof(uint32_t);
    if (have) {
      size_t roff = 0;
      for (size_t r = 0; r < W; r++) {
        recv_off[r] = roff;
        recv_bytes[r] = NeedleHipLibrary::kSlabHeader + (size_t)cap[r * W + (size_t)rank] * sizeof(NeedleHipRun);
        roff += recv_bytes[r];
      }
      if (!(s = j.d_dir_recv.reserve(roff)).ok()) return report(s);
      s = comm_all_to_all_v(kSide, j.d_dir_send.ptr, send_off.data(), send_bytes.data(), j.d_dir_recv.ptr, recv_off.data(), recv_bytes.data(),
// ... 244 lines not shown
        const uint32_t *m = static_cast<const uint32_t *>(j.host_counts);
        for (size_t r = 0; r < W; r++) {
          counts[r] = m[r * cw];
          most = std::max(most, counts[r]);
        }
        if (most <= j.slab_runs) {
          bool fits = true;
          for (size_t r = 0; r < W && fits; r++)
            for (size_t q = 0; q < W && fits; q++) fits = m[r * cw + 1 + q] <= j.cap[r * W + q];
          take_matrix();
          lib->last_max_count = most;
          if (fits) break;
          NeedleError e = job_search_and_gather(lib, comparator, j);
          if (e != NeedleError_Ok) return e;
          j.comm_bytes[3]++;
          continue;
        }
      } else {
        for (int r = 0; r < world; r++) {
          counts[r] = *reinterpret_cast<const uint32_t *>(static_cast<const char *>(j.host) + (size_t)r * j.head_bytes());
          most = std::max(most, counts[r]);
        }
        if (most <= j.slab_runs && (world == 1 || most <= j.head_runs)) {
          lib->last_max_count = most;
          if (j.counted) take_matrix();
          break;
        }
        if (most <= j.slab_runs) {
          lib->last_max_count = most;
          Status s = job_buffers(lib, j, world);
          if (!s.ok()) return report(s);
          NeedleError e = job_search_and_gather(lib, comparator, j);
          if (e != NeedleError_Ok) return e;
          j.comm_bytes[3]++;
          continue;
        }
      }
      lib->slab_runs = round_up4((uint64_t)most + most / 4 + 64);
      lib->last_max_count = most;
      lib->dir_counts.clear();
      Status s = job_buffers(lib, j, world);
      if (!s.ok()) return report(s);
      NeedleError e = job_search_and_gather(lib, comparator, j);
      if (e != NeedleError_Ok) return e;
      j.comm_bytes[3]++;
    }
    j.pending = false;
    size_t total = 0;
    for (int r = 0; r < world; r++) total += counts[r];
    const NeedleHipRun *run_list = nullptr;
    if (j.directed)
      j.merged.clear();
    else if (world == 1 && counts[0] <= j.head_runs)
      run_list = reinterpret_cast<const NeedleHipRun *>(static_cast<const char *>(j.host) + NeedleHipLibrary::kSlabHeader);
    else
      j.merged.resize(total);
    size_t at = 0;
    bool tails = false;
    for (int r = 0; r < world && !run_list && !j.directed; r++) {
      const uint32_t head = std::min(counts[r], j.head_runs);
      std::memcpy(j.merged.data() + at, static_cast<const char *>(j.host) + (size_t)r * j.head_bytes() + NeedleHipLibrary::kSlabHeader,
                  (size_t)head * sizeof(NeedleHipRun));
      if (counts[r] > head) {
        tails = true;
        if (hipMemcpyAsync(j.merged.data() + at + head,
                           j.d_slabs.ptr + (size_t)r * j.slab_bytes() + NeedleHipLibrary::kSlabHeader + (size_t)head * sizeof(NeedleHipRun),
                           (size_t)(counts[r] - head) * sizeof(NeedleHipRun), hipMemcpyDeviceToHost, download_stream()) != hipSuccess)
          return report(Status::Make(NeedleError_Unknown, "run download failed"));
      }
      at += counts[r];
    }
    if (tails && hipStreamSynchronize(download_stream()) != hipSuccess)
      return report(Status::Make(NeedleError_Unknown, "run download failed"));
    if (num_runs) *num_runs = total;

    std::vector<VideoResult> res;
    const bool sharded = j.shape_fixed ? j.sharded : (world > 1 && shard_epilogue(total));
    size_t v0 = 0, vcount = lib->n;
    if (sharded) shard_range(lib->n, world, rank, &v0, &vcount);
    const auto t0 = std::chrono::steady_clock::now();
    if (!run_list && !j.directed) run_list = j.merged.data();
    j.last_runs = run_list;
    j.last_total = total;
    Status s;
    const NeedleHipSearchResult *device_results = nullptr;
    if (j.device_epilogue) {
      device_results = static_cast<const NeedleHipSearchResult *>(j.host_results);
      const uint32_t fail = *reinterpret_cast<const uint32_t *>(device_results + lib->n);
      if (fail & kEpilogueBucketTooLarge) {
        device_results = nullptr;
        note_epilogue_host_fallback("library job", total, vcount);
      }
      else if (fail != 0)
        s = Status::Make(NeedleError_Unknown, "overflow when subtracting durations (time_padding / hash_duration exceed the match end)");
    }
    j.ran_device_epilogue = device_results != nullptr;
    j.ran_sharded = sharded;
    if (!device_results) {
      const std::vector<const FrameHashesData *> fh = lib->shell_pointers();
      if (j.directed) {
        Status f = fetch_directed(j, world, rank);
        if (!f.ok()) return report(f);
        s = cmp.results_from_runs(fh, j.fetched.data(), j.fetched.size(), false, false, false, &res, v0, v0 + vcount);
      } else {
        s = cmp.results_from_runs(fh, run_list, total, false, false, false, &res, v0, v0 + vcount);
      }
    }
    if (getenv("NEEDLE_HIP_TRACE"))
      std::fprintf(stderr, "[needle_hip] rank %d epilogue %zu runs, videos [%zu, %zu): %.1f us\n", rank, total, v0, v0 + vcount,
                   std::chrono::duration<double, std::micro>(std::chrono::steady_clock::now() - t0).count());
    if (!sharded) {
      if (!s.ok()) return report(s);
      if (device_results)
        std::memcpy(results, device_results, lib->n * sizeof(NeedleHipSearchResult));
      else
        for (size_t v = 0; v < lib->n; v++) fill_c_result(res[v], &results[v]);
      return NeedleError_Ok;
    }
    const size_t b = shard_block(lib->n, world);
    struct Block {
      uint64_t failed;
    };
    const size_t block_bytes = sizeof(Block) + b * sizeof(NeedleHipSearchResult);
    std::vector<uint8_t> mine(block_bytes, 0), all(block_bytes * (size_t)world, 0);
    reinterpret_cast<Block *>(mine.data())->failed = s.ok() ? 0 : 1;
    if (s.ok() && device_results)
      std::memcpy(mine.data() + sizeof(Block), device_results + v0, vcount * sizeof(NeedleHipSearchResult));
    else if (s.ok())
      for (size_t k = 0; k < vcount; k++)
        fill_c_result(res[v0 + k], reinterpret_cast<NeedleHipSearchResult *>(mine.data() + sizeof(Block)) + k);
    Status g = comm_all_gather_host(mine.data(), all.data(), block_bytes);
    j.comm_bytes[2] += block_bytes * (uint64_t)world;
    if (!s.ok()) return report(s);
    if (!g.ok()) return report(g);
    for (int r = 0; r < world; r++) {
      const uint8_t *blk = all.data() + (size_t)r * block_bytes;
      if (reinterpret_cast<const Block *>(blk)->failed)
        return report(Status::Make(NeedleError_Unknown, "the epilogue failed on rank " + std::to_string(r)));
      size_t f = 0, c = 0;
      shard_range(lib->n, world, r, &f, &c);
      std::memcpy(results + f, blk + sizeof(Block), c * sizeof(NeedleHipSearchResult));
    }
    return NeedleError_Ok;
  });
}

enum NeedleError needle_hip_library_job_runs(const NeedleHipLibrary *lib, int slot, const NeedleHipRun **runs, size_t *num_runs) {
  if (!lib || !runs || !num_runs) return NeedleError_NullArgument;
  if (slot < 0 || slot > 1 || lib->job[slot].pending) return NeedleError_InvalidArgument;
  if (lib->job[slot].directed) {
    NeedleHipLibrary::Job &j = const_cast<NeedleHipLibrary *>(lib)->job[slot];
    Status s = fetch_directed(j, comm_world(), comm_rank());
    if (!s.ok()) return report(s);
    *runs = j.fetched.data();
    *num_runs = j.fetched.size();
    return NeedleError_Ok;
  }
  if (!lib->job[slot].last_runs && lib->job[slot].last_total) return NeedleError_InvalidArgument;
  *runs = lib->job[slot].last_runs;
  *num_runs = lib->job[slot].last_total;
  return NeedleError_Ok;
}

enum NeedleError needle_hip_library_job_form(const NeedleHipLibrary *lib, int slot, uint32_t form[4]) {
  if (!lib || !form) return NeedleError_NullArgument;
  if (slot < 0 || slot > 1 || lib->job[slot].pending) return NeedleError_InvalidArgument;
  const NeedleHipLibrary::Job &j = lib->job[slot];
  form[0] = j.ran_device_epilogue ? 1u : 0u;
  form[1] = j.ran_sharded ? 1u : 0u;
  form[2] = j.directed ? 1u : 0u;
  form[3] = j.scan_form;
  return NeedleError_Ok;
}

enum NeedleError needle_hip_library_job_comm_bytes(const NeedleHipLibrary *lib, int slot, uint64_t bytes[4]) {
  if (!lib || !bytes) return NeedleError_NullArgument;
  if (slot < 0 || slot > 1) return NeedleError_InvalidArgument;
  std::copy(lib->job[slot].comm_bytes, lib->job[slot].comm_bytes + 4, bytes);
  return NeedleError_Ok;
}

int needle_hip_host_threads(void) { return (int)host_threads(); }

enum NeedleError needle_hip_library_audit(NeedleHipLibrary *lib, NeedleHipCertAudit *audit) {
  if (!lib || !audit) return NeedleError_NullArgument;
  if (!lib->have_pcm || !lib->pcm_resident) return NeedleError_InvalidArgument;
  return guarded([&]() -> NeedleError {
    std::vector<StreamSpan> spans;
    Status s = block_spans(lib, comm_world(), comm_rank(), &spans);
    if (!s.ok()) return report(s);
    uint64_t c[4] = {0, 0, 0, 0};
    *audit = NeedleHipCertAudit{};
    if (spans.empty()) return NeedleError_Ok;
    s = gpu_fingerprint_audit_device(lib->d_pcm.ptr, spans, lib->channels, lib->step, lib->arena, c, &audit->max_error_over_s,
                                     &audit->max_s);
    if (!s.ok()) return report(s);
    audit->items = c[0];
    audit->accepted = c[1];
    audit->accepted_mismatches = c[2];
    audit->mismatches = c[3];
    return NeedleError_Ok;
  });
}

}
```

needle_amd/csrc/search.hip:

```cpp
#include "epilogue.h"
#include "hipctx.h"
#include "simhash_wave.h"

#include <algorithm>
#include <atomic>
#include <cstdio>
#include <cstdlib>
#include <cstring>
#include <mutex>
#include <unordered_map>

namespace needle {

namespace {

constexpr int kDiagsPerBlock = 256;
constexpr int kBandR = 7, kBandU = 3;
constexpr int kBandB = 64 * kBandR;
constexpr int kSampleW = 8;
constexpr int kSampleHead = 3;
__host__ __device__ constexpr int head_row(int k, int W, int H = kSampleHead) {
  return H == 3 ? (k == 0 ? 0 : (k == 1 ? W / 2 : W - 1)) : (k * (W - 1)) / (H - 1);
}
__host__ __device__ constexpr bool is_head_row(int s, int W, int H = kSampleHead) {
  for (int k = 0; k < H; k++)
    if (head_row(k, W, H) == s) return true;
  return false;
}
__host__ __device__ constexpr int tail_row(int k, int W, int H = kSampleHead) {
  int seen = 0;
  for (int s = 0; s < W; s++) {
    if (is_head_row(s, W, H)) continue;
    if (seen == k) return s;
    seen++;
  }
  return W - 1;
}

struct SearchProblem {
  uint32_t src_off, n;
  uint32_t dst_off, m;
  uint32_t min_len, tag;
  uint32_t block_base;
  uint32_t pad;
};

template <bool STAGED>
__global__ __launch_bounds__(256) void hamming_runs_kernel(const uint32_t *__restrict__ hashes,
                                                           const SearchProblem *__restrict__ problems,
                                                           int num_problems, uint32_t first_problem, uint32_t threshold,
                                                           NeedleHipRun *__restrict__ runs, uint32_t capacity,
                                                           uint32_t *__restrict__ count) {
  extern __shared__ uint32_t lds[];
  int lo = 0, hi = num_problems - 1;
  while (lo < hi) {
    int mid = (lo + hi + 1) >> 1;
    if (problems[mid].block_base <= blockIdx.x) lo = mid; else hi = mid - 1;
  }
  const SearchProblem pr = problems[lo];
  const int n = (int)pr.n, m = (int)pr.m;
  const uint32_t *s = hashes + pr.src_off, *t = hashes + pr.dst_off;
  if (STAGED) {
    for (int i = threadIdx.x; i < n; i += blockDim.x) lds[i] = s[i];
    for (int j = threadIdx.x; j < m; j += blockDim.x) lds[n + j] = t[j];
    __syncthreads();
    s = lds;
    t = lds + n;
  }

  const int dd = (int)(blockIdx.x - pr.block_base) * kDiagsPerBlock + (int)threadIdx.x;
  const int num_diags = n + m - 3;
  if (dd >= num_diags) return;
  const int d = dd - (n - 2);
  const int i_lo = d < 0 ? 1 - d : 1;
  const int i_hi = min(n - 1, m - 1 - d);
  const uint32_t min_len = pr.min_len;
  uint32_t run = 0;
  for (int i = i_lo; i <= i_hi; i++) {
    const bool match = (uint32_t)__popc(s[i] ^ t[i + d]) <= threshold;
    if (match) {
      run++;
    } else {
      if (run >= min_len) {
        const uint32_t slot = atomicAdd(count, 1u);
        if (slot < capacity)
          runs[slot] = NeedleHipRun{first_problem + (uint32_t)lo, (uint32_t)(i - 1), (uint32_t)(i - 1 + d), run, 0u, 0u};
      }
      run = 0;
    }
  }
  if (run >= min_len) {
    const uint32_t slot = atomicAdd(count, 1u);
    if (slot < capacity)
      runs[slot] = NeedleHipRun{first_problem + (uint32_t)lo, (uint32_t)i_hi, (uint32_t)(i_hi + d), run, 0u, 0u};
  }
}

template <int R, int U>
__global__ __launch_bounds__(256) void hamming_runs_band_kernel(const uint32_t *__restrict__ hashes,
                                                                const SearchProblem *__restrict__ problems,
                                                                int num_problems, uint32_t threshold,
                                                                NeedleHipRun *__restrict__ runs, uint32_t capacity,
                                                                uint32_t *__restrict__ count) {
// ... 73 lines not shown
        const uint32_t c = (uint32_t)__popc(sv ^ W[(r + s) % R]);
        Z[r] = (c <= threshold) ? Z[r] : row;
        if (r == 0) W[s % R] = nxt[s];
      }
    }
    bool any = false;
#pragma unroll
    for (int r = 0; r < R; r++) any |= (i + K - 1 - Z[r] >= flag_len);
    if (__any(any)) checkpoint(i + K - 1);
  }
  for (; i <= i_end; i++) {
    const uint32_t sv = src[i];
#pragma unroll
    for (int r = 0; r < R; r++) {
      const uint32_t c = (uint32_t)__popc(sv ^ W[r]);
      Z[r] = (c <= threshold) ? Z[r] : i;
    }
#pragma unroll
    for (int r = 0; r + 1 < R; r++) W[r] = W[r + 1];
    W[R - 1] = lds[B + i + d_l + R];
  }
}

__device__ __forceinline__ void wave_lds_fence_search() {
  __builtin_amdgcn_fence(__ATOMIC_RELEASE, "wavefront");
  __builtin_amdgcn_wave_barrier();
  __builtin_amdgcn_fence(__ATOMIC_ACQUIRE, "wavefront");
}

template <int R, int W, bool COUNT = false, int H = kSampleHead, bool LEGACY = false>
__global__ __launch_bounds__(256) void hamming_runs_sampled_kernel(const uint32_t *__restrict__ hashes,
                                                                   const SearchProblem *__restrict__ problems,
                                                                   int num_problems, uint32_t threshold,
                                                                   NeedleHipRun *__restrict__ runs,
                                                                   uint32_t capacity, uint32_t *__restrict__ count,
                                                                   int bands_per_wave, int sparse_max,
                                                                   unsigned long long *__restrict__ eval_groups) {
  constexpr int B = 64 * R;
  unsigned long long groups = 0, survived = 0;
  extern __shared__ uint32_t lds[];
  __builtin_amdgcn_s_setprio(3);
  int lo = 0, hi = num_problems - 1;
  while (lo < hi) {
    int mid = (lo + hi + 1) >> 1;
    if (problems[mid].block_base <= blockIdx.x) lo = mid; else hi = mid - 1;
  }
  const SearchProblem pr = problems[lo];
  const int n = (int)pr.n, m = (int)pr.m;
  const uint32_t *__restrict__ src = hashes + pr.src_off;
  const uint32_t *__restrict__ dst = hashes + pr.dst_off;
  uint32_t *ldst = lds;
  for (int k = threadIdx.x; k < B; k += blockDim.x) {
    ldst[k] = 0u;
    ldst[B + m + k] = 0u;
  }
  {
    constexpr int kU = 8;
    const int nt = (int)blockDim.x;
    int k = threadIdx.x;
    for (; k + (kU - 1) * nt < m; k += kU * nt) {
      uint32_t v[kU];
#pragma unroll
      for (int u = 0; u < kU; u++) v[u] = dst[k + u * nt];
#pragma unroll
      for (int u = 0; u < kU; u++) ldst[B + k + u * nt] = v[u];
    }
    for (; k < m; k += nt) ldst[B + k] = dst[k];
  }
  const uint32_t *__restrict__ lsrc = src;
  __syncthreads();

  const int wave = __builtin_amdgcn_readfirstlane((int)(threadIdx.x >> 6));
  const int lane = (int)(threadIdx.x & 63);
  const int min_len = (int)pr.min_len;
  const int P = min_len - W + 1;
  const uint32_t bias = 31u - min(threshold, 31u);
  uint32_t held_b = 0u, held_e = 0u, held_len = 0u;
  int held = 0;
  auto flush_runs = [&]() {
    if (held == 0) return;
    uint32_t base = 0u;
    if (lane == 0) base = atomicAdd(count, (uint32_t)held);
    base = (uint32_t)__builtin_amdgcn_readfirstlane((int)base);
    if (lane < held && base + (uint32_t)lane < capacity)
      runs[base + (uint32_t)lane] = NeedleHipRun{(uint32_t)lo, held_b, held_e, held_len, 0u, 0u};
    held = 0;
  };
  auto emit_run = [&](const uint32_t b, const uint32_t e, const uint32_t len) {
    const bool mine = lane == held;
    held_b = mine ? b : held_b;
    held_e = mine ? e : held_e;
    held_len = mine ? len : held_len;
    if (++held == 64) flush_runs();
  };
  const int slots = 4 * bands_per_wave;
  const int total_bands = (n + m - 3 + B - 1) / B;
  const int nb = (total_bands + slots - 1) / slots;
  const int b_in_pair = (int)(blockIdx.x - pr.block_base);
  for (int round = 0; round < bands_per_wave; round++) {
  const int q = (round * 4 + wave + lo) % slots;
  const int band = q * nb + b_in_pair;
  const int D0 = band * B - (n - 2);
  if (band >= total_bands || D0 > m - 2) continue;
  const int i_start = max(1, 2 - D0 - B);
  const int i_end = min(n - 1, m - 1 - D0);
  const int d_l = D0 + lane * R;

  int k0 = (i_start - 1 + P - 1) / P;
  for (int w0 = 1 + k0 * P; w0 + W - 1 <= i_end; w0 += P) {
    uint32_t E[W + R - 1];
#pragma unroll
    for (int q = 0; q < W + R - 1; q++) E[q] = ldst[B + w0 + d_l + q];
    uint32_t sv[W];
#pragma unroll
    for (int s = 0; s < W; s++) sv[s] = src[w0 + s];
    bool ok[R];
    uint32_t miss[R];
#pragma unroll
    for (int r = 0; r < R; r++) miss[r] = 0u;
#pragma unroll
    for (int k = 0; k < H; k++) {
      const int s = head_row(k, W, H);
#pragma unroll
      for (int r = 0; r < R; r++) miss[r] |= (uint32_t)__popc(sv[s] ^ E[s + r]) + bias;
    }
#pragma unroll
    for (int r = 0; r < R; r++) ok[r] = miss[r] < 32u;
    if (COUNT) groups += H * R;
    auto resolve = [&](const int d) {
      const int ilo = d < 0 ? 1 - d : 1;
      const int ihi = min(n - 1, m - 1 - d);
      if (w0 < ilo || w0 + W - 1 > ihi) return;
      int e = w0 + W;
      bool ended = false;
      const int fwd_limit = min(ihi, w0 + P + W - 1);
      while (e <= fwd_limit) {
        const int row = e + lane;
        const bool bad = row <= fwd_limit && (uint32_t)__popc(lsrc[row] ^ ldst[B + row + d]) > threshold;
        if (COUNT) groups += 1;
        const unsigned long long mm = __ballot(bad);
        if (mm) {
          e += __ffsll((long long)mm) - 1;
          ended = true;
          break;
        }
        e += 64;
      }
      if (!ended) {
        if (fwd_limit == w0 + P + W - 1) return;
        e = ihi + 1;
      }
      const int b = e - 1;
      int a = ilo;
      int q = w0 - 1;
      while (q >= ilo) {
        const int row = q - lane;
        const bool bad = row >= ilo && (uint32_t)__popc(lsrc[row] ^ ldst[B + row + d]) > threshold;
        if (COUNT) groups += 1;
        const unsigned long long mm = __ballot(bad);
        if (mm) {
          a = q - (__ffsll((long long)mm) - 1) + 1;
          break;
        }
        q -= 64;
      }
      const int len = b - a + 1;
      if (len >= min_len) emit_run((uint32_t)b, (uint32_t)(b + d), (uint32_t)len);
    };
// ... 57 lines not shown
      const int s = tail_row(k, W, H);
#pragma unroll
      for (int r = 0; r < R; r++) miss[r] |= (uint32_t)__popc(sv[s] ^ E[s + r]) + bias;
    }
#pragma unroll
    for (int r = 0; r < R; r++) ok[r] = miss[r] < 32u;
    if (COUNT) groups += (W - H) * R;
#pragma unroll
    for (int r = 0; r < R; r++) {
      unsigned long long cand = __ballot(ok[r]);
      while (cand) {
        const int src_lane = __ffsll((long long)cand) - 1;
        cand &= cand - 1;
        resolve(D0 + src_lane * R + r);
      }
    }
    }
  }
  }
  flush_runs();
  if (COUNT && lane == 0) {
    atomicAdd(eval_groups, groups);
    atomicAdd(eval_groups + 1, survived);
  }
}

__host__ __device__ constexpr int mfma_windows(int n, int min_len, int W) {
  return (n - 1 - W) >= 0 && min_len - W + 1 > 0 ? (n - 1 - W) / (min_len - W + 1) + 1 : 0;
}
typedef int mfma_v4i __attribute__((ext_vector_type(4)));
typedef int mfma_v8i __attribute__((ext_vector_type(8)));
typedef float mfma_v16f __attribute__((ext_vector_type(16)));

#include "scan_mfma_kernel.h"


__global__ __launch_bounds__(256) void simhash_runs_kernel(const uint32_t *__restrict__ hashes,
                                                           const SearchProblem *__restrict__ problems,
                                                           NeedleHipRun *__restrict__ runs, uint32_t capacity,
                                                           const uint32_t *__restrict__ count) {
  const uint32_t total = min(*count, capacity);
  const uint32_t wave = (blockIdx.x * blockDim.x + threadIdx.x) >> 6, waves = (gridDim.x * blockDim.x) >> 6;
  const uint32_t lane = threadIdx.x & 63;
  __builtin_amdgcn_s_setprio(3);
  const TransposeLane t = transpose_lane(lane);
  for (uint32_t k = wave; k < total; k += waves) {
    const NeedleHipRun r = runs[k];
    const SearchProblem pr = problems[r.problem];
    const uint32_t src_hash = wave_simhash32(hashes + pr.src_off + (r.src_end - r.len), r.len + 1u, lane, t);
    const uint32_t dst_hash = wave_simhash32(hashes + pr.dst_off + (r.dst_end - r.len), r.len + 1u, lane, t);
    if (lane == 0) {
      runs[k].problem = pr.tag;
      runs[k].src_match_hash = src_hash;
      runs[k].dst_match_hash = dst_hash;
    }
  }
}

struct ScanShape {
  int w = kSampleW, h = kSampleHead;
};
ScanShape scan_shape() {
  ScanShape sh;
  if (const char *e = getenv("NEEDLE_HIP_SCAN_SHAPE")) {
    int w = 0, h = 0;
    if (std::sscanf(e, "%d,%d", &w, &h) == 2 && (w == 4 || w == 8 || w == 16) && h >= 2 && h <= 4 && h < w) {
      sh.w = w;
      sh.h = h;
    }
  }
  return sh;
}
using SampledKernel = void (*)(const uint32_t *, const SearchProblem *, int, uint32_t, NeedleHipRun *, uint32_t, uint32_t *, int, int,
                               unsigned long long *);
template <bool COUNT>
SampledKernel sampled_kernel(ScanShape sh, bool legacy) {
#define NEEDLE_SHAPE(W_, H_) \
  if (sh.w == W_ && sh.h == H_) return hamming_runs_sampled_kernel<kBandR, W_, COUNT, H_, true>;
  NEEDLE_SHAPE(4, 2) NEEDLE_SHAPE(4, 3) NEEDLE_SHAPE(8, 2) NEEDLE_SHAPE(8, 4) NEEDLE_SHAPE(16, 2) NEEDLE_SHAPE(16, 3) NEEDLE_SHAPE(16, 4)
#undef NEEDLE_SHAPE
  if (legacy) return hamming_runs_sampled_kernel<kBandR, kSampleW, COUNT, kSampleHead, true>;
  return hamming_runs_sampled_kernel<kBandR, kSampleW, COUNT, kSampleHead, false>;
}

struct SearchPlan {
  std::vector<NeedleHipSeq> seqs;
  std::vector<NeedleHipProblem> problems;
  int mode[8] = {0, 0, 0, 0, 0, 0, 0, 0};
  std::vector<SearchProblem> meta;
  size_t staged = 0;
  uint64_t oversize_blocks = 0;
  uint64_t blocks = 0;
  size_t lds_bytes = 0;
  bool sampled = false, fast = false, mfma = false;
  int mfma_waves = 0, mfma_splits = 1;
  std::vector<M2ImageSeq> image_seqs;
  uint32_t image_windows = 0, image_min_len = 0;
  uint64_t mfma_products = 0;
  int bands_per_wave = 1;
  bool valid = false;
  bool matches(const NeedleHipSeq *s, size_t ns, const NeedleHipProblem *p, size_t np, const int *m) const {
    return valid && seqs.size() == ns && problems.size() == np && std::memcmp(mode, m, sizeof(mode)) == 0 &&
           std::memcmp(seqs.data(), s, ns * sizeof(NeedleHipSeq)) == 0 &&
           std::memcmp(problems.data(), p, np * sizeof(NeedleHipProblem)) == 0;
  }
};

int device_cus() {
  int cus = 256, dev = 0;
  if (hipGetDevice(&dev) == hipSuccess) (void)hipDeviceGetAttribute(&cus, hipDeviceAttributeMultiprocessorCount, dev);
  return cus > 0 ? cus : 256;
}

Status build_plan(const NeedleHipSeq *seqs, size_t num_seqs, const NeedleHipProblem *problems, size_t num_problems,
                  const int *mode, SearchPlan *plan) {
  plan->valid = false;
  std::vector<SearchProblem> &meta = plan->meta;
  meta.clear();
  meta.reserve(num_problems);
  uint64_t blocks = 0;
  for (size_t p = 0; p < num_problems; p++) {
    const NeedleHipProblem &pr = problems[p];
    if (pr.src_seq >= num_seqs || pr.dst_seq >= num_seqs)
      return Status::Make(NeedleError_InvalidArgument, "hamming_runs: problem references a missing sequence");
    if (pr.min_len == 0) return Status::Make(NeedleError_InvalidArgument, "hamming_runs: min_len must be >= 1");
    const NeedleHipSeq &a = seqs[pr.src_seq], &b = seqs[pr.dst_seq];
    if (a.len < 2 || b.len < 2) continue;
    SearchProblem m;
    m.src_off = a.offset;
    m.n = a.len;
    m.dst_off = b.offset;
    m.m = b.len;
    m.min_len = pr.min_len;
    m.tag = pr.tag;
    m.block_base = 0;
    m.pad = 0;
    meta.push_back(m);
  }
  plan->staged = 0;
  plan->oversize_blocks = 0;
  if (!meta.empty()) {
    uint32_t smallest = 0xFFFFFFFFu;
    for (const SearchProblem &m : meta) smallest = std::min(smallest, m.min_len);
    const bool generic_only = mode[0] != 0;
    const bool sampled = !generic_only && smallest >= (uint32_t)(2 * scan_shape().w - 1 + 8) && mode[1] == 0 && mode[3] == 0;
    const bool fast = !generic_only && !sampled && smallest >= (uint32_t)(kBandR * kBandU);
    const size_t lds_limit = (size_t)mode[5];
    auto windows_of = [&](const SearchProblem &m) { return (uint64_t)mfma_windows((int)m.n, (int)m.min_len, kSampleW); };
    auto same_group = [](const SearchProblem &a, const SearchProblem &b) {
      return a.dst_off == b.dst_off && a.m == b.m && a.min_len == b.min_len;
    };
    const int waves = mode[6];
    const size_t group_budget = waves == 4 ? 53760 : waves == 8 ? 81920 : 163840;
    const size_t max_members = (size_t)kM2Members;
    auto group_need = [&](const SearchProblem &a, uint64_t windows) { return m2_lds_words(a.m, windows, waves) * sizeof(uint32_t); };
    bool mfma = sampled && mode[4] == 1;
    const size_t mfma_from = 2048;
    const bool candidate = sampled && (mode[4] == 1 || (mode[4] == 2 && meta.size() >= mfma_from));
    if (candidate) {
      std::stable_sort(meta.begin(), meta.end(), [](const SearchProblem &a, const SearchProblem &b) {
        if (a.dst_off != b.dst_off) return a.dst_off < b.dst_off;
        if (a.m != b.m) return a.m < b.m;
        return a.min_len < b.min_len;
      });
      if (!mfma) {
        uint64_t windows = 0, rows = 0;
        for (size_t i = 0; i < meta.size(); i++) {
          uint64_t w = windows_of(meta[i]);
          for (size_t k = 1; k < max_members && i + 1 < meta.size() && same_group(meta[i], meta[i + 1]) &&
                             group_need(meta[i], w + windows_of(meta[i + 1])) <= group_budget; k++)
            w += windows_of(meta[++i]);
          windows += w;
          rows += (w + 31) / 32 * 32;
        }
        mfma = rows > 0 && 10 * windows >= 7 * rows;
      }
    }
    auto lds_need = [&](const SearchProblem &m) {
      if (mfma) return group_need(m, windows_of(m));
      return ((fast || sampled) ? (size_t)m.m + 2 * kBandB : (size_t)m.n + m.m) * sizeof(uint32_t);
    };
    auto mfma_packable = [&](const SearchProblem &m) { return m.m < 65536u && windows_of(m) < 8192u && m.n < (1u << 28); };
    auto stageable = [&](const SearchProblem &m) { return lds_need(m) <= lds_limit && (!mfma || mfma_packable(m)); };
    std::stable_partition(meta.begin(), meta.end(), stageable);
    size_t staged = 0;
    while (staged < meta.size() && stageable(meta[staged])) staged++;
    size_t lds_bytes = 0;
    int bands_per_wave = 1;
    size_t groups = 0;
    if (mfma) {
      const bool single = (mode[7] & 0x100) != 0;
      for (size_t i = 0; i < staged;) {
        SearchProblem &a = meta[i];
        a.pad = 0;
        uint64_t windows = windows_of(a);
        size_t k = 1;
        while (!single && k < max_members && i + k < staged && same_group(a, meta[i + k]) &&
               windows + windows_of(meta[i + k]) < 8192 &&
               group_need(a, windows + windows_of(meta[i + k])) <= group_budget) {
          windows += windows_of(meta[i + k]);
          meta[i + k].pad = 0x80000000u;
          k++;
        }
        a.pad = (uint32_t)(k - 1);
        i += k;
        groups++;
      }
    }
    if (mfma) {
      if (staged >= ((size_t)1 << 23)) return Status::Make(NeedleError_InvalidArgument, "hamming_runs: too many problems for one launch");
      size_t g = 0;
      for (size_t i = 0; i < staged; i++)
        if (!(meta[i].pad & 0x80000000u)) meta[g++].pad |= (uint32_t)i << 8;
    }
    int splits = 1;
    if (mfma && groups > 0) {
      const uint64_t slots = (uint64_t)device_cus() * (uint64_t)(waves == 4 ? 3 : waves == 8 ? 2 : 1);
      splits = (int)std::min<uint64_t>(8, std::max<uint64_t>(1, (2 * slots + groups - 1) / groups));
      if (mode[7] & 0x7F) splits = mode[7] & 0x7F;
    }
    if (fast || sampled) {
      uint64_t fb = 0, total_bands = 0;
      for (size_t i = 0; i < staged; i++) total_bands += ((uint64_t)meta[i].n + meta[i].m - 3 + kBandB - 1) / kBandB;
      if (sampled)
        while (bands_per_wave < 8 && total_bands / (4 * (uint64_t)bands_per_wave * 2) >= 16384) bands_per_wave *= 2;
      if (mode[2] > 0) bands_per_wave = mode[2];
      for (size_t i = 0; i < staged; i++) {
        SearchProblem &m = meta[i];
        m.block_base = (uint32_t)fb;
        if (mfma && (m.pad & 0x80000000u)) continue;
        const uint64_t diags = (uint64_t)m.n + m.m - 3;
        const uint64_t bands = (diags + kBandB - 1) / kBandB;
        const uint64_t per_block = 4 * (uint64_t)(sampled ? bands_per_wave : 1);
        fb += mfma ? (uint64_t)splits : (bands + per_block - 1) / per_block;
        if (mfma) {
          uint64_t windows = windows_of(m);
          for (uint32_t f = 1; f <= (m.pad & 0xFFu); f++) windows += windows_of(meta[i + f]);
          lds_bytes = std::max(lds_bytes, group_need(m, windows));
        } else {
          lds_bytes = std::max(lds_bytes, lds_need(m));
        }
      }
      blocks = fb;
    } else {
      for (size_t i = 0; i < staged; i++) {
        SearchProblem &m = meta[i];
        m.block_base = (uint32_t)blocks;
        blocks += ((uint64_t)m.n + m.m - 3 + kDiagsPerBlock - 1) / kDiagsPerBlock;
        lds_bytes = std::max(lds_bytes, lds_need(m));
      }
    }
    uint64_t ob = 0;
    for (size_t i = staged; i < meta.size(); i++) {
      meta[i].block_base = (uint32_t)ob;
      ob += ((uint64_t)meta[i].n + meta[i].m - 3 + kDiagsPerBlock - 1) / kDiagsPerBlock;
    }
    if (blocks > 0x7FFFFFFFull || ob > 0x7FFFFFFFull)
      return Status::Make(NeedleError_InvalidArgument, "hamming_runs: too many problems for one launch");
    plan->staged = staged;
    plan->oversize_blocks = ob;
    plan->sampled = sampled;
    plan->mfma = mfma;
    plan->mfma_products = 0;
    if (mfma)
      for (size_t i = 0; i < staged; i++) {
        const SearchProblem &m = meta[i];
        if (m.pad & 0x80000000u) continue;
        uint64_t w = windows_of(m);
        for (uint32_t f = 1; f <= (m.pad & 0xFFu); f++) w += windows_of(meta[i + f]);
        if (w > 0 && m.m >= (uint32_t)kSampleW + 1) {
          uint64_t col_blocks = ((uint64_t)m.m - kSampleW) / 32 + 1;
          col_blocks = (col_blocks + kM2ColBlocks - 1) / kM2ColBlocks * kM2ColBlocks;
          plan->mfma_products += (w + 31) / 32 * col_blocks * (kM2Heads / 2);
        }
      }
    plan->image_seqs.clear();
    plan->image_windows = plan->image_min_len = 0;
    if (mfma && staged > 0 && !(mode[7] & 0x200)) {
      bool one = true;
      for (size_t i = 1; i < staged && one; i++) one = meta[i].min_len == meta[0].min_len;
      if (one) {
        std::unordered_map<uint64_t, uint32_t> first_of;
        uint64_t total = 0;
        for (size_t i = 0; i < staged; i++) {
          const uint64_t key = ((uint64_t)meta[i].src_off << 32) | meta[i].n;
          auto it = first_of.find(key);
          if (it == first_of.end()) {
            const uint32_t w = (uint32_t)windows_of(meta[i]);
            it = first_of.emplace(key, (uint32_t)total).first;
            plan->image_seqs.push_back(M2ImageSeq{meta[i].src_off, meta[i].n, (uint32_t)total, w});
            total += w;
          }
          meta[i].block_base = it->second;
        }
        if (total == 0 || total * kM2ImageWords * sizeof(uint32_t) > ((uint64_t)1 << 31)) {
          plan->image_seqs.clear();
        } else {
          plan->image_windows = (uint32_t)total;
          plan->image_min_len = meta[0].min_len;
        }
      }
    }
    plan->fast = fast;
    plan->mfma_waves = waves;
    plan->mfma_splits = splits;
    plan->bands_per_wave = bands_per_wave;
    plan->lds_bytes = lds_bytes;
  }
  plan->blocks = blocks;
  plan->seqs.assign(seqs, seqs + num_seqs);
  plan->problems.assign(problems, problems + num_problems);
  std::memcpy(plan->mode, mode, sizeof(plan->mode));
  plan->valid = true;
  return Status::Ok();
}

int mfma_request(uint32_t threshold) {
  if (threshold > 15u || scan_shape().w != kSampleW || getenv("NEEDLE_HIP_SCAN_SHAPE") || getenv("NEEDLE_HIP_SCAN_COUNT")) return 0;
  const char *e = getenv("NEEDLE_HIP_SCAN_MFMA");
  if (!e) return 2;
  return atoi(e) != 0 ? 1 : 0;
}

int mfma_waves() {
  int waves = 8;
  if (const char *e = getenv("NEEDLE_HIP_MFMA_WAVES")) {
    const int w = atoi(e);
    if (w == 4 || w == 8 || w == 12 || w == 16) waves = w;
  }
  return waves;
}
using Mfma2Kernel = void (*)(const uint32_t *, const SearchProblem *, int, uint32_t, NeedleHipRun *, uint32_t, uint32_t *, int, const uint32_t *);
Mfma2Kernel mfma2_kernel(int waves) {
  return waves == 4 ? hamming_runs_mfma2_kernel<kSampleW, 4, 3> : waves == 16 ? hamming_runs_mfma2_kernel<kSampleW, 16, 4>
       : waves == 12 ? hamming_runs_mfma2_kernel<kSampleW, 12, 3> : hamming_runs_mfma2_kernel<kSampleW, 8, 4>;
}

std::atomic<int32_t> g_last_form{0};
std::atomic<uint64_t> g_last_products{0};

struct SearchWorkspace {
  DeviceBuffer<SearchProblem> problems;
  PinnedStage stage;
  DescriptorUpload<SearchProblem> upload;
  SearchPlan plan;
  DeviceBuffer<M2ImageSeq> image_seqs;
  PinnedStage image_stage;
  DescriptorUpload<M2ImageSeq> image_upload;
  DeviceBuffer<uint32_t> images;
  bool lds_attr_set = false;
  unsigned long long *eval_groups = nullptr;
};
std::mutex g_ws_mu;
std::map<int, SearchWorkspace *> g_ws;

SearchWorkspace *workspace() {
  int dev = 0;
  (void)hipGetDevice(&dev);
  std::lock_guard<std::mutex> lock(g_ws_mu);
  auto it = g_ws.find(dev);
  if (it != g_ws.end()) return it->second;
  SearchWorkspace *w = new SearchWorkspace();
  g_ws[dev] = w;
  return w;
}


}

void gpu_scan_last_launch(int32_t *form, uint64_t *matrix_products) {
  *form = g_last_form.load();
  *matrix_products = g_last_products.load();
}

Status gpu_hamming_runs_device(const uint32_t *d_hashes, const NeedleHipSeq *seqs, size_t num_seqs,
                               const NeedleHipProblem *problems, size_t num_problems, uint32_t threshold,
                               NeedleHipRun *d_runs, uint32_t capacity, uint32_t *d_count, bool sync, bool count_is_zero) {
  std::lock_guard<std::recursive_mutex> gpu_lock(gpu_mutex());
  Status s = ensure_device();
  if (!s.ok()) return s;
  hipStream_t stream = library_stream();
  if (!count_is_zero) NEEDLE_HIP_TRY(hipMemsetAsync(d_count, 0, sizeof(uint32_t), stream));
  const int mode[8] = {getenv("NEEDLE_HIP_GENERIC_SEARCH") != nullptr, getenv("NEEDLE_HIP_BAND_SEARCH") != nullptr,
                       getenv("NEEDLE_HIP_BANDS_PER_WAVE") ? std::max(1, atoi(getenv("NEEDLE_HIP_BANDS_PER_WAVE"))) : 0,
                       threshold > 31u,
                       mfma_request(threshold),
                       getenv("NEEDLE_HIP_SEARCH_LDS_LIMIT") ? std::max(1, atoi(getenv("NEEDLE_HIP_SEARCH_LDS_LIMIT"))) : 160 * 1024,
                       mfma_waves(),
                       (getenv("NEEDLE_HIP_MFMA_SPLITS") ? std::max(1, std::min(64, atoi(getenv("NEEDLE_HIP_MFMA_SPLITS")))) : 0) |
                           (getenv("NEEDLE_HIP_MFMA_SINGLE") ? 0x100 : 0) | (getenv("NEEDLE_HIP_MFMA_NO_IMAGES") ? 0x200 : 0)};
  SearchWorkspace *ws = workspace();
  SearchPlan &plan = ws->plan;
  const bool reuse = plan.matches(seqs, num_seqs, problems, num_problems, mode);
  if (!reuse && !(s = build_plan(seqs, num_seqs, problems, num_problems, mode, &plan)).ok()) return s;
  const std::vector<SearchProblem> &meta = plan.meta;
  const uint64_t blocks = plan.blocks;
  const size_t lds_bytes = plan.lds_bytes;
  const bool sampled = plan.sampled, fast = plan.fast;
  const int bands_per_wave = plan.bands_per_wave;
  if (!meta.empty()) {
    if (!(reuse && ws->upload.resident_at == ws->problems.ptr && ws->problems.ptr) &&
        !(s = ws->upload.put(&ws->problems, &ws->stage, meta, stream)).ok())
      return s;
    if (lds_bytes > 64 * 1024 && !ws->lds_attr_set) {
      NEEDLE_HIP_TRY(hipFuncSetAttribute(reinterpret_cast<const void *>(hamming_runs_kernel<true>),
                                         hipFuncAttributeMaxDynamicSharedMemorySize, 160 * 1024));
      NEEDLE_HIP_TRY(hipFuncSetAttribute(reinterpret_cast<const void *>(hamming_runs_band_kernel<kBandR, kBandU>),
                                         hipFuncAttributeMaxDynamicSharedMemorySize, 160 * 1024));
      for (int w : {4, 8, 12, 16})
        NEEDLE_HIP_TRY(hipFuncSetAttribute(reinterpret_cast<const void *>(mfma2_kernel(w)),
                                           hipFuncAttributeMaxDynamicSharedMemorySize, 160 * 1024));
      for (int w : {4, 8, 16})
        for (int h : {2, 3, 4}) {
          if (h >= w) continue;
          for (bool legacy : {false, true}) {
            NEEDLE_HIP_TRY(hipFuncSetAttribute(reinterpret_cast<const void *>(sampled_kernel<false>(ScanShape{w, h}, legacy)),
                                               hipFuncAttributeMaxDynamicSharedMemorySize, 160 * 1024));
            NEEDLE_HIP_TRY(hipFuncSetAttribute(reinterpret_cast<const void *>(sampled_kernel<true>(ScanShape{w, h}, legacy)),
                                               hipFuncAttributeMaxDynamicSharedMemorySize, 160 * 1024));
          }
        }
      ws->lds_attr_set = true;
    }
    const int staged = (int)plan.staged, oversize = (int)(meta.size() - plan.staged);
    g_last_form.store(staged > 0 ? (sampled ? (plan.mfma ? 4 : 3) : fast ? 2 : 1) : 1);
    g_last_products.store(staged > 0 && plan.mfma ? plan.mfma_products : 0);
    if (staged > 0) {
      KernelTimer timer("hamming_runs");
      if (sampled) {
        int sparse_max = -1;
        if (const char *e = getenv("NEEDLE_HIP_SPARSE_MAX")) sparse_max = std::max(0, atoi(e));
        if (getenv("NEEDLE_HIP_SCAN_COUNT")) {
          if (!ws->eval_groups) {
            NEEDLE_HIP_TRY(hipMalloc((void **)&ws->eval_groups, 2 * sizeof(unsigned long long)));
            NEEDLE_HIP_TRY(hipMemsetAsync(ws->eval_groups, 0, 2 * sizeof(unsigned long long), stream));
          }
          hipLaunchKernelGGL(sampled_kernel<true>(scan_shape(), sparse_max >= 0), dim3((uint32_t)blocks), dim3(256), lds_bytes, stream, d_hashes,
                             ws->problems.ptr, staged, threshold, d_runs, capacity, d_count, bands_per_wave, sparse_max,
                             ws->eval_groups);
        } else if (plan.mfma) {
          const uint32_t *images = nullptr;
          if (!plan.image_seqs.empty()) {
            if (!(s = ws->image_upload.put(&ws->image_seqs, &ws->image_stage, plan.image_seqs, stream)).ok() ||
                !(s = ws->images.reserve((size_t)plan.image_windows * kM2ImageWords)).ok())
              return s;
            const uint32_t grid = (uint32_t)std::min<uint64_t>(8192, ((uint64_t)plan.image_windows * kM2Rows + 255) / 256);
            hipLaunchKernelGGL(m2_window_images_kernel<kSampleW>, dim3(grid), dim3(256), 0, stream, d_hashes, ws->image_seqs.ptr,
                               (int)plan.image_seqs.size(), plan.image_windows, plan.image_min_len, ws->images.ptr);
            images = ws->images.ptr;
          }
          hipLaunchKernelGGL(mfma2_kernel(plan.mfma_waves), dim3((uint32_t)blocks), dim3(64 * plan.mfma_waves),
                             lds_bytes, stream, d_hashes, ws->problems.ptr, staged, threshold, d_runs, capacity, d_count,
                             plan.mfma_splits, images);
#if NEEDLE_M2_LAB & 8
          {
            unsigned long long c[8], z[8] = {};
            (void)hipStreamSynchronize(stream);
            (void)hipMemcpyFromSymbol(c, HIP_SYMBOL(m2_dbg), sizeof c);
            (void)hipMemcpyToSymbol(HIP_SYMBOL(m2_dbg), z, sizeof z);
            fprintf(stderr, "m2 counts: resolve calls %llu, trips %llu, mismatches handled %llu, walks continued %llu, extra forward trips %llu, "
                            "windows past the tail rows %llu, items %llu, windows past the head rows %llu\n", c[0], c[1], c[2], c[3], c[4], c[5], c[6], c[7]);
          }
#endif
        } else {
          hipLaunchKernelGGL(sampled_kernel<false>(scan_shape(), sparse_max >= 0), dim3((uint32_t)blocks), dim3(256), lds_bytes, stream, d_hashes,
                             ws->problems.ptr, staged, threshold, d_runs, capacity, d_count, bands_per_wave, sparse_max,
                             (unsigned long long *)nullptr);
        }
      }
      else if (fast)
        hipLaunchKernelGGL((hamming_runs_band_kernel<kBandR, kBandU>), dim3((uint32_t)blocks), dim3(256), lds_bytes,
                           stream, d_hashes, ws->problems.ptr, staged, threshold, d_runs, capacity, d_count);
      else
        hipLaunchKernelGGL(hamming_runs_kernel<true>, dim3((uint32_t)blocks), dim3(256), lds_bytes, stream, d_hashes,
                           ws->problems.ptr, staged, 0u, threshold, d_runs, capacity, d_count);
    }
    if (oversize > 0) {
      KernelTimer timer("hamming_runs_unstaged");
      hipLaunchKernelGGL(hamming_runs_kernel<false>, dim3((uint32_t)plan.oversize_blocks), dim3(256), 0, stream, d_hashes,
                         ws->problems.ptr + staged, oversize, (uint32_t)staged, threshold, d_runs, capacity, d_count);
    }
    {
      KernelTimer timer("simhash_runs");
      hipLaunchKernelGGL(simhash_runs_kernel, dim3(2048), dim3(256), 0, stream, d_hashes, ws->problems.ptr, d_runs,
                         capacity, d_count);
    }
    NEEDLE_HIP_TRY(hipGetLastError());
  }
  if (sync) NEEDLE_HIP_TRY(hipStreamSynchronize(stream));
  return Status::Ok();
}

Status gpu_scan_issued_evaluations(uint64_t *lane_evaluations, bool reset, uint64_t *head_survivors) {
  std::lock_guard<std::recursive_mutex> gpu_lock(gpu_mutex());
  Status s = ensure_device();
  if (!s.ok()) return s;
  SearchWorkspace *ws = workspace();
  unsigned long long groups[2] = {0, 0};
  hipStream_t stream = library_stream();
  if (ws->eval_groups) {
    NEEDLE_HIP_TRY(hipMemcpyAsync(groups, ws->eval_groups, sizeof(groups), hipMemcpyDeviceToHost, stream));
    if (reset) NEEDLE_HIP_TRY(hipMemsetAsync(ws->eval_groups, 0, sizeof(groups), stream));
    NEEDLE_HIP_TRY(hipStreamSynchronize(stream));
  }
  *lane_evaluations = (uint64_t)groups[0] * 64u;
  if (head_survivors) *head_survivors = (uint64_t)groups[1];
  return Status::Ok();
}

namespace {
struct HostCallBuffers {
  DeviceBuffer<uint32_t> d_hashes, d_count;
  DeviceBuffer<NeedleHipRun> d_runs;
  void *pinned = nullptr;
  size_t pinned_bytes = 0;
  uint32_t *arena = nullptr;
  size_t arena_words = 0;
  bool arena_out = false;
  const uint32_t *sent = nullptr;
  size_t sent_words = 0;
};
HostCallBuffers *host_call_buffers() {
  static std::map<int, HostCallBuffers *> all;
  int dev = 0;
  (void)hipGetDevice(&dev);
  HostCallBuffers *&hb = all[dev];
  if (!hb) hb = new HostCallBuffers();
  return hb;
}
}

uint32_t *gpu_pinned_arena_acquire(size_t words) {
  std::lock_guard<std::recursive_mutex> gpu_lock(gpu_mutex());
  if (!ensure_device().ok()) return nullptr;
  HostCallBuffers *hb = host_call_buffers();
  if (hb->arena_out || getenv("NEEDLE_HIP_PAGEABLE_ARENA")) return nullptr;
  if (words > hb->arena_words) {
    if (hb->arena) (void)hipHostFree(hb->arena);
    hb->arena = nullptr;
    hb->arena_words = 0;
    void *p = nullptr;
    const size_t want = words + words / 8 + 1024;
    if (hipHostMalloc(&p, want * sizeof(uint32_t), hipHostMallocDefault) != hipSuccess) {
      (void)hipGetLastError();
      return nullptr;
    }
    hb->arena = static_cast<uint32_t *>(p);
    hb->arena_words = want;
  }
// ... 228 lines not shown
```

rust/needle-hip/src/ffi.rs:

```rust
#![allow(non_camel_case_types, dead_code)]

use std::os::raw::{c_char, c_int, c_void};

#[repr(C)]
#[derive(Clone, Copy, Debug, PartialEq, Eq)]
pub enum NeedleError {
    Ok = 0,
    InvalidUtf8String,
    NullArgument,
    InvalidArgument,
    FrameHashDataNotFound,
    FrameHashDataInvalidVersion,
    InvalidFrameHashData,
    ComparatorMinimumPaths,
    AnalyzerInvalidHashPeriod,
    AnalyzerInvalidHashDuration,
    IOError,
    Unknown,
}

#[repr(C)]
pub struct NeedleAudioAnalyzer {
    _private: [u8; 0],
}
// ... 91 lines not shown
    pub fn format(&self) -> NeedleHipLaneFormat {
        self.format
    }
    pub fn frames(&self) -> u64 {
        self.frames
    }
}

#[repr(C)]
#[derive(Clone, Copy, Debug, Default, PartialEq, Eq)]
pub struct NeedleHipChannelMix {
    pub(crate) channels: i32,
    pub(crate) coef: [[i32; 8]; 2],
}

impl NeedleHipChannelMix {
    pub fn new(left: &[i32], right: &[i32]) -> Self {
        assert!(left.len() == right.len() && left.len() <= 8, "two rows of at most 8 coefficients each");
        let mut m = Self { channels: left.len() as i32, coef: [[0; 8]; 2] };
        m.coef[0][..left.len()].copy_from_slice(left);
        m.coef[1][..right.len()].copy_from_slice(right);
        m
    }
    pub fn channels(&self) -> i32 {
        self.channels
    }
    pub fn row(&self, output: usize) -> &[i32] {
        &self.coef[output][..self.channels.clamp(0, 8) as usize]
    }
}

extern "C" {
    pub fn needle_error_to_str(error: NeedleError) -> *const c_char;
    pub fn needle_audio_analyzer_new(
        paths: *const *const c_char,
        num_paths: usize,
        opening_search_percentage: f32,
        ending_search_percentage: f32,
        include_endings: bool,
        threaded_decoding: bool,
        force: bool,
        output: *mut *mut NeedleAudioAnalyzer,
    ) -> NeedleError;
    pub fn needle_audio_analyzer_free(analyzer: *const NeedleAudioAnalyzer);
    pub fn needle_audio_analyzer_get_frame_hashes(
        analyzer: *const NeedleAudioAnalyzer,
        index: usize,
        output: *mut *const FrameHashes,
    ) -> NeedleError;
    pub fn needle_audio_analyzer_run(
        analyzer: *mut NeedleAudioAnalyzer,
        hash_duration: f32,
        persist: bool,
        threading: bool,
    ) -> NeedleError;
    pub fn needle_audio_comparator_new(
        paths: *const *const c_char,
        num_paths: usize,
        include_endings: bool,
        hash_match_threshold: u16,
        min_opening_duration: u16,
        min_ending_duration: u16,
        time_padding: f32,
        output: *mut *const NeedleAudioComparator,
    ) -> NeedleError;
    pub fn needle_audio_comparator_free(comparator: *const NeedleAudioComparator);
    pub fn needle_audio_comparator_run(
        comparator: *const NeedleAudioComparator,
        analyze: bool,
        display: bool,
        use_skip_files: bool,
        write_skip_files: bool,
        threading: bool,
    ) -> NeedleError;

    pub fn needle_hip_last_error_message() -> *const c_char;
    pub fn needle_hip_device_count(count: *mut c_int) -> NeedleError;
    pub fn needle_hip_set_device(ordinal: c_int) -> NeedleError;
    pub fn needle_hip_synchronize() -> NeedleError;
    pub fn needle_hip_device_pci_bus_id(out: *mut c_char) -> NeedleError;
    pub fn needle_hip_fingerprint_cert_stats(counts: *mut u64, reset: bool) -> NeedleError;
    pub fn needle_hip_scan_issued_evaluations(lane_evaluations: *mut u64, reset: bool) -> NeedleError;
    pub fn needle_hip_scan_last_launch(form: *mut i32, matrix_products: *mut u64) -> NeedleError;
    pub fn needle_hip_epilogue_host_fallbacks(jobs: *mut u64, reset: bool) -> NeedleError;
    pub fn needle_hip_stream() -> *mut c_void;
    pub fn needle_hip_analyzer_run_pcm(
        analyzer: *mut NeedleAudioAnalyzer,
        pcm: *const *const i16,
        num_values: *const usize,
        channels: c_int,
        sample_rate: c_int,
        hash_duration: f32,
        persist: bool,
    ) -> NeedleError;
    pub fn needle_hip_analyzer_run_pcm_format(
        analyzer: *mut NeedleAudioAnalyzer,
        pcm: *const *const c_void,
        num_values: *const usize,
        channels: c_int,
        sample_rate: c_int,
        format: c_int,
        hash_duration: f32,
        persist: bool,
    ) -> NeedleError;
    pub fn needle_hip_comparator_run_with_frame_hashes(
        comparator: *const NeedleAudioComparator,
        frame_hashes: *const *const FrameHashes,
        num_videos: usize,
        display: bool,
        use_skip_files: bool,
        write_skip_files: bool,
        results: *mut NeedleHipSearchResult,
    ) -> NeedleError;
    pub fn needle_hip_frame_hashes_new(
        opening_hashes: *const u32,
        opening_ts_ns: *const u64,
        num_opening: usize,
        ending_hashes: *const u32,
        ending_ts_ns: *const u64,
        num_ending: usize,
        hash_duration_ns: u64,
        md5: *const c_char,
        output: *mut *mut FrameHashes,
    ) -> NeedleError;
    pub fn needle_hip_frame_hashes_free(frame_hashes: *mut FrameHashes);
    pub fn needle_hip_frame_hashes_len(frame_hashes: *const FrameHashes, ending: bool) -> usize;
    pub fn needle_hip_frame_hashes_copy(
        frame_hashes: *const FrameHashes,
        ending: bool,
        hashes: *mut u32,
        ts_ns: *mut u64,
        capacity: usize,
    ) -> NeedleError;
    pub fn needle_hip_frame_hashes_hash_duration_ns(frame_hashes: *const FrameHashes) -> u64;
    pub fn needle_hip_frame_hashes_md5(frame_hashes: *const FrameHashes) -> *const c_char;
    pub fn needle_hip_frame_hashes_read(path: *const c_char, output: *mut *mut FrameHashes) -> NeedleError;
    pub fn needle_hip_frame_hashes_write(frame_hashes: *const FrameHashes, path: *const c_char) -> NeedleError;
    pub fn needle_hip_comm_create_id(id: *mut u8) -> NeedleError;
    pub fn needle_hip_comm_init(id: *const u8, rank: c_int, world_size: c_int) -> NeedleError;
    pub fn needle_hip_comm_finalize();
    pub fn needle_hip_comm_rank() -> c_int;
    pub fn needle_hip_comm_world_size() -> c_int;
    pub fn needle_hip_comm_barrier() -> NeedleError;
    pub fn needle_hip_comm_all_gather_host(send: *const c_void, recv: *mut c_void, bytes_per_rank: usize) -> NeedleError;
    pub fn needle_hip_comm_shard(units: usize, world_size: c_int, rank: c_int, first: *mut usize, count: *mut usize);
    pub fn needle_hip_library_new(
        num_videos: usize,
        opening_search_percentage: f32,
        hash_duration: f32,
        output: *mut *mut NeedleHipLibrary,
    ) -> NeedleError;
    pub fn needle_hip_library_free(library: *mut NeedleHipLibrary);
    pub fn needle_hip_index_new(comparator: *const NeedleAudioComparator, output: *mut *mut NeedleHipIndex) -> NeedleError;
    pub fn needle_hip_index_free(index: *mut NeedleHipIndex);
    pub fn needle_hip_index_len(index: *const NeedleHipIndex) -> usize;
    pub fn needle_hip_index_add(index: *mut NeedleHipIndex, frame_hashes: *const *const FrameHashes, k: usize) -> NeedleError;
    pub fn needle_hip_index_results(index: *const NeedleHipIndex, results: *mut NeedleHipSearchResult, n: usize) -> NeedleError;
    pub fn needle_hip_index_pairs_searched(index: *const NeedleHipIndex, total: *mut u64, last: *mut u64) -> NeedleError;
    pub fn needle_hip_index_remove(index: *mut NeedleHipIndex, positions: *const usize, k: usize) -> NeedleError;
    pub fn needle_hip_index_replace(
        index: *mut NeedleHipIndex,
        positions: *const usize,
        frame_hashes: *const *const FrameHashes,
        k: usize,
    ) -> NeedleError;
    pub fn needle_hip_index_store_sizes(index: *const NeedleHipIndex, sizes: *mut u64) -> NeedleError;
// ... 1 lines not shown
        index: *mut NeedleHipIndex,
        videos: usize,
        max_items: *const usize,
        min_len: *const u32,
        output: *mut *mut NeedleHipCrossMatcher,
    ) -> NeedleError;
    pub fn needle_hip_index_add_matched(
        index: *mut NeedleHipIndex,
        matcher: *mut NeedleHipCrossMatcher,
        frame_hashes: *const *const FrameHashes,
        k: usize,
    ) -> NeedleError;
    pub fn needle_hip_index_pairs_scanned(index: *const NeedleHipIndex, total: *mut u64, last: *mut u64) -> NeedleError;
    pub fn needle_hip_downmix_host(
        pcm: *const *const i16,
        num_values: *const usize,
        num_streams: usize,
        channels: c_int,
        out: *const *mut i16,
    ) -> NeedleError;
    pub fn needle_hip_convert_host(
        pcm: *const *const c_void,
        num_values: *const usize,
        num_streams: usize,
        channels: c_int,
        format: c_int,
        out: *const *mut i16,
    ) -> NeedleError;
    pub fn needle_hip_library_set_sample_format(library: *mut NeedleHipLibrary, format: c_int) -> NeedleError;
    pub fn needle_hip_library_include_endings(library: *mut NeedleHipLibrary, ending_search_percentage: f32) -> NeedleError;
    pub fn needle_hip_library_set_sample_rate(library: *mut NeedleHipLibrary, sample_rate: c_int) -> NeedleError;
    pub fn needle_hip_library_set_pcm(
        library: *mut NeedleHipLibrary,
        pcm: *const *const i16,
        num_values: *const usize,
        channels: c_int,
    ) -> NeedleError;
    pub fn needle_hip_library_rank_videos(
        library: *const NeedleHipLibrary,
        num_values: *const usize,
        channels: c_int,
        world_size: c_int,
        rank: c_int,
        first_video: *mut usize,
        video_count: *mut usize,
    ) -> NeedleError;
    pub fn needle_hip_library_set_pcm_device(
        library: *mut NeedleHipLibrary,
        d_pcm: *const *const i16,
        num_values: *const usize,
        channels: c_int,
    ) -> NeedleError;
    pub fn needle_hip_library_stream_pcm(
        library: *mut NeedleHipLibrary,
        pcm: *const *const i16,
        num_values: *const usize,
        channels: c_int,
    ) -> NeedleError;
    pub fn needle_hip_library_job_begin(
        library: *mut NeedleHipLibrary,
        comparator: *const NeedleAudioComparator,
        slot: c_int,
    ) -> NeedleError;
    pub fn needle_hip_library_job_end(
        library: *mut NeedleHipLibrary,
        comparator: *const NeedleAudioComparator,
        slot: c_int,
        results: *mut NeedleHipSearchResult,
        num_runs: *mut usize,
    ) -> NeedleError;
    pub fn needle_hip_library_frame_hashes(
        library: *mut NeedleHipLibrary,
        index: usize,
        output: *mut *mut FrameHashes,
    ) -> NeedleError;
    pub fn needle_hip_library_job_runs(
        library: *const NeedleHipLibrary,
        slot: c_int,
        runs: *mut *const NeedleHipRun,
        num_runs: *mut usize,
    ) -> NeedleError;
    pub fn needle_hip_library_job_comm_bytes(library: *const NeedleHipLibrary, slot: c_int, bytes: *mut u64) -> NeedleError;
    pub fn needle_hip_library_job_form(library: *const NeedleHipLibrary, slot: c_int, form: *mut u32) -> NeedleError;
    pub fn needle_hip_library_audit(library: *mut NeedleHipLibrary, audit: *mut NeedleHipCertAudit) -> NeedleError;
    pub fn needle_hip_host_threads() -> c_int;
    pub fn needle_hip_host_alloc(host_ptr: *mut *mut c_void, bytes: usize) -> NeedleError;
    pub fn needle_hip_host_alloc_free(host_ptr: *mut c_void) -> NeedleError;
    pub fn needle_hip_feeder_new(
        lanes: usize,
        channels: c_int,
        sample_rate: c_int,
        format: c_int,
        step: u32,
        output: *mut *mut NeedleHipFeeder,
    ) -> NeedleError;
    pub fn needle_hip_feeder_new_lanes(formats: *const NeedleHipLaneFormat, lanes: usize, step: u32, output: *mut *mut NeedleHipFeeder) -> NeedleError;
    pub fn needle_hip_feeder_lane_format(feeder: *const NeedleHipFeeder, lane: usize, format: *mut NeedleHipLaneFormat) -> NeedleError;
    pub fn needle_hip_feeder_reset_format(
        feeder: *mut NeedleHipFeeder,
        lanes: *const usize,
        formats: *const NeedleHipLaneFormat,
        k: usize,
    ) -> NeedleError;
    pub fn needle_hip_convert_mono_host(
        pcm: *const *const c_void,
        num_values: *const usize,
        formats: *const NeedleHipLaneFormat,
        num_streams: usize,
        out: *const *mut i16,
    ) -> NeedleError;
    pub fn needle_hip_channel_mix_default(channel_mask: u32, out: *mut NeedleHipChannelMix) -> NeedleError;
    pub fn needle_hip_rematrix_host(
        pcm: *const *const c_void,
        num_values: *const usize,
        formats: *const NeedleHipLaneFormat,
        mixes: *const NeedleHipChannelMix,
        num_streams: usize,
        out: *const *mut i16,
    ) -> NeedleError;
    pub fn needle_hip_analyzer_set_channel_mix(analyzer: *mut NeedleAudioAnalyzer, mix: *const NeedleHipChannelMix) -> NeedleError;
    pub fn needle_hip_analyzer_set_layout_downmix(analyzer: *mut NeedleAudioAnalyzer, on: bool) -> NeedleError;
    pub fn needle_hip_comparator_set_layout_downmix(comparator: *mut NeedleAudioComparator, on: bool) -> NeedleError;
    pub fn needle_hip_library_set_channel_mix(library: *mut NeedleHipLibrary, mix: *const NeedleHipChannelMix) -> NeedleError;
    pub fn needle_hip_feeder_set_lane_mix(
        feeder: *mut NeedleHipFeeder,
        lanes: *const usize,
        mixes: *const NeedleHipChannelMix,
        k: usize,
    ) -> NeedleError;
    pub fn needle_hip_feeder_switch_format(
        feeder: *mut NeedleHipFeeder,
        lanes: *const usize,
        formats: *const NeedleHipLaneFormat,
        mixes: *const NeedleHipChannelMix,
        k: usize,
    ) -> NeedleError;
    pub fn needle_hip_feeder_lane_segments(
        feeder: *const NeedleHipFeeder,
        lane: usize,
        out: *mut NeedleHipSegment,
        cap: usize,
        count: *mut usize,
    ) -> NeedleError;
    pub fn needle_hip_feeder_num_ready_segments(segments: *const NeedleHipSegment, count: usize, step: u32, finished: bool) -> usize;
    pub fn needle_hip_feeder_free(feeder: *mut NeedleHipFeeder);
    pub fn needle_hip_feeder_feed(feeder: *mut NeedleHipFeeder, pcm: *const *const c_void, num_values: *const usize) -> NeedleError;
    pub fn needle_hip_feeder_finish(feeder: *mut NeedleHipFeeder, lanes: *const usize, k: usize) -> NeedleError;
    pub fn needle_hip_feeder_reset(feeder: *mut NeedleHipFeeder, lanes: *const usize, k: usize) -> NeedleError;
    pub fn needle_hip_feeder_ready(
        feeder: *mut NeedleHipFeeder,
        lane: usize,
        kept_items: *mut usize,
        samples_per_channel_fed: *mut u64,
        finished: *mut bool,
    ) -> NeedleError;
    pub fn needle_hip_feeder_items(feeder: *mut NeedleHipFeeder, lane: usize, first: usize, count: usize, items: *mut u32) -> NeedleError;
    pub fn needle_hip_feeder_frame_hashes(
        feeder: *mut NeedleHipFeeder,
        opening_lane: usize,
        ending_lane: usize,
        ending_seek_ns: u64,
        hash_duration: f32,
        md5: *const c_char,
        output: *mut *mut FrameHashes,
    ) -> NeedleError;
    pub fn needle_hip_feeder_state_bytes(feeder: *const NeedleHipFeeder, bytes: *mut u64) -> NeedleError;
// ... 84 lines not shown
```

Baseline: 710,100.

## Route crowded search problems to a narrow-band sampled scan kernel

Counts runs per problem tag after each search. Tags with at least a threshold of runs are marked crowded, and on the next search those problems go to a separate launch of the sampled kernel with a one-row band instead of the wide band. This is meant to cut per-wave serialization and load imbalance on problems that emit many runs, at the cost of an extra kernel launch, host-side per-problem bookkeeping and plan invalidation whenever the crowd hints change. The run id written for non-wide bands now comes from the problem index stored in the pad field.

```diff
diff --git a/include/needle_hip.h b/include/needle_hip.h
--- a/include/needle_hip.h
+++ b/include/needle_hip.h
@@ -30,6 +30,7 @@
 enum NeedleError needle_hip_scan_issued_evaluations(uint64_t *lane_evaluations, bool reset);
 enum NeedleError needle_hip_scan_counts(uint64_t counts[2], bool reset);
 enum NeedleError needle_hip_scan_last_launch(int32_t *form, uint64_t *matrix_products);
+enum NeedleError needle_hip_scan_last_crowded(uint32_t *crowded_problems);
 enum NeedleError needle_hip_epilogue_host_fallbacks(uint64_t *jobs, bool reset);
 
 #define NEEDLE_HIP_MAX_CHANNELS 8
@@ -257,6 +258,7 @@
                                              size_t *num_runs);
 enum NeedleError needle_hip_library_job_comm_bytes(const NeedleHipLibrary *library, int slot, uint64_t bytes[4]);
 enum NeedleError needle_hip_library_job_form(const NeedleHipLibrary *library, int slot, uint32_t form[4]);
+enum NeedleError needle_hip_library_job_crowded(const NeedleHipLibrary *library, int slot, uint32_t *crowded_problems);
 int needle_hip_host_threads(void);
 
 typedef struct NeedleHipFeeder NeedleHipFeeder;
diff --git a/needle_amd/capi.py b/needle_amd/capi.py
--- a/needle_amd/capi.py
+++ b/needle_amd/capi.py
@@ -87,7 +87,7 @@
     "needle_hip_library_job_end", "needle_hip_library_stream_pcm", "needle_hip_host_alloc",
     "needle_hip_host_alloc_free", "needle_hip_int_valu_ceiling",
     "needle_hip_comparator_results_from_runs", "needle_hip_library_job_runs", "needle_hip_library_job_comm_bytes",
-    "needle_hip_library_job_form",
+    "needle_hip_library_job_form", "needle_hip_library_job_crowded", "needle_hip_scan_last_crowded",
     "needle_hip_host_threads", "needle_hip_fingerprint_audit_device", "needle_hip_library_audit",
     "needle_hip_scan_counts", "needle_hip_scan_last_launch", "needle_hip_epilogue_host_fallbacks",
     "needle_hip_index_new", "needle_hip_index_free", "needle_hip_index_len", "needle_hip_index_add",
@@ -474,6 +474,13 @@
     return int(form.value), int(products.value)
 
 
+def scan_last_crowded() -> int:
+    n = C.c_uint32(0)
+    lib().needle_hip_scan_last_crowded.argtypes = [C.POINTER(C.c_uint32)]
+    check(lib().needle_hip_scan_last_crowded(C.byref(n)))
+    return int(n.value)
+
+
 def epilogue_host_fallbacks(reset: bool = False) -> int:
     jobs = C.c_uint64(0)
     lib().needle_hip_epilogue_host_fallbacks.argtypes = [C.POINTER(C.c_uint64), C.c_bool]
@@ -1520,7 +1527,11 @@
         f = (C.c_uint32 * 4)()
         lib().needle_hip_library_job_form.argtypes = [C.c_void_p, C.c_int, C.POINTER(C.c_uint32)]
         check(lib().needle_hip_library_job_form(self._h, slot, f))
-        return {"device_epilogue": bool(f[0]), "sharded_epilogue": bool(f[1]), "directed_runs": bool(f[2]), "scan_form": int(f[3])}
+        crowded = C.c_uint32(0)
+        lib().needle_hip_library_job_crowded.argtypes = [C.c_void_p, C.c_int, C.POINTER(C.c_uint32)]
+        check(lib().needle_hip_library_job_crowded(self._h, slot, C.byref(crowded)))
+        return {"device_epilogue": bool(f[0]), "sharded_epilogue": bool(f[1]), "directed_runs": bool(f[2]), "scan_form": int(f[3]),
+                "crowded_problems": int(crowded.value)}
 
     def job_comm_bytes(self, slot: int = 0) -> dict:
         b = (C.c_uint64 * 4)()
diff --git a/needle_amd/csrc/capi.cpp b/needle_amd/csrc/capi.cpp
--- a/needle_amd/csrc/capi.cpp
+++ b/needle_amd/csrc/capi.cpp
@@ -455,6 +455,14 @@
   return NeedleError_Ok;
 }
 
+enum NeedleError needle_hip_scan_last_crowded(uint32_t *crowded_problems) {
+  if (!crowded_problems) return NeedleError_NullArgument;
+  int32_t form = 0;
+  uint64_t products = 0;
+  gpu_scan_last_launch(&form, &products, crowded_problems);
+  return NeedleError_Ok;
+}
+
 enum NeedleError needle_hip_epilogue_host_fallbacks(uint64_t *jobs, bool reset) {
   if (!jobs) return NeedleError_NullArgument;
   *jobs = reset ? epilogue_host_fallbacks().exchange(0) : epilogue_host_fallbacks().load();
diff --git a/needle_amd/csrc/common.h b/needle_amd/csrc/common.h
--- a/needle_amd/csrc/common.h
+++ b/needle_amd/csrc/common.h
@@ -127,7 +127,9 @@
 Status gpu_hamming_runs_device(const uint32_t *d_hashes, const NeedleHipSeq *seqs, size_t num_seqs,
                                const NeedleHipProblem *problems, size_t num_problems, uint32_t threshold,
                                NeedleHipRun *d_runs, uint32_t capacity, uint32_t *d_count, bool sync,
-                               bool count_is_zero = false);
+                               bool count_is_zero = false, const uint8_t *crowd = nullptr);
+constexpr uint32_t kScanCrowdRuns = 16;
+constexpr size_t kScanMatrixFromProblems = 2048;
 Status gpu_hamming_runs_host(const uint32_t *hashes, size_t num_hashes, const NeedleHipSeq *seqs, size_t num_seqs,
                              const NeedleHipProblem *problems, size_t num_problems, uint32_t threshold,
                              std::vector<NeedleHipRun> *runs);
@@ -141,7 +143,7 @@
 
 Status gpu_int_valu_ceiling(double *cells_per_second);
 Status gpu_scan_issued_evaluations(uint64_t *lane_evaluations, bool reset, uint64_t *head_survivors = nullptr);
-void gpu_scan_last_launch(int32_t *form, uint64_t *matrix_products);
+void gpu_scan_last_launch(int32_t *form, uint64_t *matrix_products, uint32_t *crowded_problems = nullptr);
 Status gpu_fingerprint_cert_stats(uint64_t out[4], bool reset);
 Status gpu_fingerprint_audit_device(const int16_t *d_pcm, const std::vector<StreamSpan> &spans, int channels, uint32_t step,
                                     const uint32_t *d_items, uint64_t out[4], double *max_ratio, double *max_sigma);
diff --git a/needle_amd/csrc/library.cpp b/needle_amd/csrc/library.cpp
--- a/needle_amd/csrc/library.cpp
+++ b/needle_amd/csrc/library.cpp
@@ -91,6 +91,7 @@
     std::vector<uint32_t> cap;
     bool ran_device_epilogue = false, ran_sharded = false;
     uint32_t scan_form = 0;
+    uint32_t scan_crowded = 0;
     bool counted = false;
     bool directed = false;
     std::vector<NeedleHipRun> fetched;
@@ -103,6 +104,9 @@
   static constexpr size_t kSlabHeader = 32;
   uint32_t slab_runs = 0;
   uint32_t last_max_count = 0;
+  std::vector<uint8_t> crowd;
+  std::vector<uint8_t> crowd_of_problem;
+  std::vector<uint32_t> crowd_counts;
   std::vector<uint32_t> dir_counts;
   int dir_world = 0;
   bool dir_unsupported = false;
@@ -355,6 +359,7 @@
   lib->shells.clear();
   lib->shell_of.clear();
   lib->problems_for[0] = ~(size_t)0;
+  lib->crowd.clear();
   return Status::Ok();
 }
 
@@ -817,8 +822,15 @@
     const auto t_built = std::chrono::steady_clock::now();
     const bool count_is_zero = lib->count_zeroed == d_count;
     lib->count_zeroed = nullptr;
+    const uint8_t *crowd = nullptr;
+    if (!lib->crowd.empty() && problems.size() < kScanMatrixFromProblems) {
+      lib->crowd_of_problem.resize(problems.size());
+      for (size_t k = 0; k < problems.size(); k++)
+        lib->crowd_of_problem[k] = problems[k].tag < lib->crowd.size() ? lib->crowd[problems[k].tag] : 0;
+      crowd = lib->crowd_of_problem.data();
+    }
     Status s = gpu_hamming_runs_device(lib->arena, seqs.data(), seqs.size(), problems.data(), problems.size(),
-                                       cmp.hash_match_threshold(), d_runs, capacity, d_count, sync, count_is_zero);
+                                       cmp.hash_match_threshold(), d_runs, capacity, d_count, sync, count_is_zero, crowd);
     if (getenv("NEEDLE_HIP_TRACE"))
       std::fprintf(stderr, "[needle_hip] search enqueue: %zu problems built in %.2f ms, launched in %.2f ms\n",
                    problems.size(), std::chrono::duration<double, std::milli>(t_built - t_enter).count(),
@@ -973,6 +985,11 @@
   return s.ok() ? NeedleError_Ok : report(s);
 }
 
+uint32_t crowd_runs_threshold() {
+  if (const char *e = getenv("NEEDLE_HIP_SCAN_CROWD_RUNS")) return (uint32_t)std::max(1, atoi(e));
+  return kScanCrowdRuns;
+}
+
 uint32_t round_up4(uint64_t v) { return (uint32_t)std::min<uint64_t>((v + 3) & ~(uint64_t)3, 0xfffffffcu); }
 
 Status job_buffers(NeedleHipLibrary *lib, NeedleHipLibrary::Job &j, int world) {
@@ -1044,7 +1061,7 @@
   {
     int32_t form = 0;
     uint64_t products = 0;
-    gpu_scan_last_launch(&form, &products);
+    gpu_scan_last_launch(&form, &products, &j.scan_crowded);
     j.scan_form = (uint32_t)form;
   }
   hipStream_t stream = library_stream(), down = download_stream();
@@ -1455,6 +1472,19 @@
     if (!run_list && !j.directed) run_list = j.merged.data();
     j.last_runs = run_list;
     j.last_total = total;
+    {
+      const size_t tags = pair_count(lib->n) * (cmp.include_endings() ? 2 : 1);
+      if (j.directed || tags >= kScanMatrixFromProblems) {
+        lib->crowd.clear();
+      } else {
+        lib->crowd_counts.assign(tags, 0u);
+        for (size_t k = 0; k < total; k++)
+          if (run_list[k].problem < tags) lib->crowd_counts[run_list[k].problem]++;
+        lib->crowd.resize(tags);
+        const uint32_t crowd_from = crowd_runs_threshold();
+        for (size_t t = 0; t < tags; t++) lib->crowd[t] = lib->crowd_counts[t] >= crowd_from;
+      }
+    }
     Status s;
     const NeedleHipSearchResult *device_results = nullptr;
     if (j.device_epilogue) {
@@ -1546,6 +1576,13 @@
   return NeedleError_Ok;
 }
 
+enum NeedleError needle_hip_library_job_crowded(const NeedleHipLibrary *lib, int slot, uint32_t *crowded_problems) {
+  if (!lib || !crowded_problems) return NeedleError_NullArgument;
+  if (slot < 0 || slot > 1 || lib->job[slot].pending) return NeedleError_InvalidArgument;
+  *crowded_problems = lib->job[slot].scan_crowded;
+  return NeedleError_Ok;
+}
+
 enum NeedleError needle_hip_library_job_comm_bytes(const NeedleHipLibrary *lib, int slot, uint64_t bytes[4]) {
   if (!lib || !bytes) return NeedleError_NullArgument;
   if (slot < 0 || slot > 1) return NeedleError_InvalidArgument;
diff --git a/needle_amd/csrc/search.hip b/needle_amd/csrc/search.hip
--- a/needle_amd/csrc/search.hip
+++ b/needle_amd/csrc/search.hip
@@ -19,6 +19,7 @@
 constexpr int kBandB = 64 * kBandR;
 constexpr int kSampleW = 8;
 constexpr int kSampleHead = 3;
+constexpr int kCrowdR = 1;
 __host__ __device__ constexpr int head_row(int k, int W, int H = kSampleHead) {
   return H == 3 ? (k == 0 ? 0 : (k == 1 ? W / 2 : W - 1)) : (k * (W - 1)) / (H - 1);
 }
@@ -258,8 +259,10 @@
     uint32_t base = 0u;
     if (lane == 0) base = atomicAdd(count, (uint32_t)held);
     base = (uint32_t)__builtin_amdgcn_readfirstlane((int)base);
+    uint32_t id;
+    if constexpr (R == kBandR) id = (uint32_t)lo; else id = pr.pad;
     if (lane < held && base + (uint32_t)lane < capacity)
-      runs[base + (uint32_t)lane] = NeedleHipRun{(uint32_t)lo, held_b, held_e, held_len, 0u, 0u};
+      runs[base + (uint32_t)lane] = NeedleHipRun{id, held_b, held_e, held_len, 0u, 0u};
     held = 0;
   };
   auto emit_run = [&](const uint32_t b, const uint32_t e, const uint32_t len) {
@@ -483,13 +486,21 @@
   if (legacy) return hamming_runs_sampled_kernel<kBandR, kSampleW, COUNT, kSampleHead, true>;
   return hamming_runs_sampled_kernel<kBandR, kSampleW, COUNT, kSampleHead, false>;
 }
+template <bool COUNT>
+SampledKernel narrow_kernel() {
+  return hamming_runs_sampled_kernel<kCrowdR, kSampleW, COUNT, kSampleHead, false>;
+}
 
 struct SearchPlan {
   std::vector<NeedleHipSeq> seqs;
   std::vector<NeedleHipProblem> problems;
-  int mode[8] = {0, 0, 0, 0, 0, 0, 0, 0};
+  std::vector<uint8_t> crowd;
+  int mode[9] = {0, 0, 0, 0, 0, 0, 0, 0, 0};
   std::vector<SearchProblem> meta;
   size_t staged = 0;
+  size_t crowded = 0;
+  uint64_t crowd_blocks = 0;
+  size_t crowd_lds_bytes = 0;
   uint64_t oversize_blocks = 0;
   uint64_t blocks = 0;
   size_t lds_bytes = 0;
@@ -500,7 +511,8 @@
   uint64_t mfma_products = 0;
   int bands_per_wave = 1;
   bool valid = false;
-  bool matches(const NeedleHipSeq *s, size_t ns, const NeedleHipProblem *p, size_t np, const int *m) const {
+  bool matches(const NeedleHipSeq *s, size_t ns, const NeedleHipProblem *p, size_t np, const int *m, const uint8_t *hint) const {
+    if (m[8] == 2 && (hint ? crowd.size() != np || std::memcmp(crowd.data(), hint, np) != 0 : !crowd.empty())) return false;
     return valid && seqs.size() == ns && problems.size() == np && std::memcmp(mode, m, sizeof(mode)) == 0 &&
            std::memcmp(seqs.data(), s, ns * sizeof(NeedleHipSeq)) == 0 &&
            std::memcmp(problems.data(), p, np * sizeof(NeedleHipProblem)) == 0;
@@ -514,7 +526,7 @@
 }
 
 Status build_plan(const NeedleHipSeq *seqs, size_t num_seqs, const NeedleHipProblem *problems, size_t num_problems,
-                  const int *mode, SearchPlan *plan) {
+                  const int *mode, const uint8_t *crowd, SearchPlan *plan) {
   plan->valid = false;
   std::vector<SearchProblem> &meta = plan->meta;
   meta.clear();
@@ -535,11 +547,14 @@
     m.min_len = pr.min_len;
     m.tag = pr.tag;
     m.block_base = 0;
-    m.pad = 0;
+    m.pad = mode[8] == 1 || (mode[8] == 2 && crowd && crowd[p]) ? 1u : 0u;
     meta.push_back(m);
   }
   plan->staged = 0;
   plan->oversize_blocks = 0;
+  plan->crowded = 0;
+  plan->crowd_blocks = 0;
+  plan->crowd_lds_bytes = 0;
   if (!meta.empty()) {
     uint32_t smallest = 0xFFFFFFFFu;
     for (const SearchProblem &m : meta) smallest = std::min(smallest, m.min_len);
@@ -556,7 +571,7 @@
     const size_t max_members = (size_t)kM2Members;
     auto group_need = [&](const SearchProblem &a, uint64_t windows) { return m2_lds_words(a.m, windows, waves) * sizeof(uint32_t); };
     bool mfma = sampled && mode[4] == 1;
-    const size_t mfma_from = 2048;
+    const size_t mfma_from = kScanMatrixFromProblems;
     const bool candidate = sampled && (mode[4] == 1 || (mode[4] == 2 && meta.size() >= mfma_from));
     if (candidate) {
       std::stable_sort(meta.begin(), meta.end(), [](const SearchProblem &a, const SearchProblem &b) {
@@ -586,6 +601,14 @@
     std::stable_partition(meta.begin(), meta.end(), stageable);
     size_t staged = 0;
     while (staged < meta.size() && stageable(meta[staged])) staged++;
+    size_t crowded = 0;
+    if (sampled && !candidate) {
+      const auto first = std::stable_partition(meta.begin(), meta.begin() + (ptrdiff_t)staged, [](const SearchProblem &m) { return m.pad == 0u; });
+      crowded = staged - (size_t)(first - meta.begin());
+    }
+    if (!mfma)
+      for (size_t i = 0; i < meta.size(); i++) meta[i].pad = (uint32_t)i;
+    const size_t wide = staged - crowded;
     size_t lds_bytes = 0;
     int bands_per_wave = 1;
     size_t groups = 0;
@@ -622,11 +645,11 @@
     }
     if (fast || sampled) {
       uint64_t fb = 0, total_bands = 0;
-      for (size_t i = 0; i < staged; i++) total_bands += ((uint64_t)meta[i].n + meta[i].m - 3 + kBandB - 1) / kBandB;
+      for (size_t i = 0; i < wide; i++) total_bands += ((uint64_t)meta[i].n + meta[i].m - 3 + kBandB - 1) / kBandB;
       if (sampled)
         while (bands_per_wave < 8 && total_bands / (4 * (uint64_t)bands_per_wave * 2) >= 16384) bands_per_wave *= 2;
       if (mode[2] > 0) bands_per_wave = mode[2];
-      for (size_t i = 0; i < staged; i++) {
+      for (size_t i = 0; i < wide; i++) {
         SearchProblem &m = meta[i];
         m.block_base = (uint32_t)fb;
         if (mfma && (m.pad & 0x80000000u)) continue;
@@ -643,6 +666,15 @@
         }
       }
       blocks = fb;
+      uint64_t cb = 0;
+      const uint64_t narrow_b = 64 * (uint64_t)kCrowdR;
+      for (size_t i = wide; i < staged; i++) {
+        SearchProblem &m = meta[i];
+        m.block_base = (uint32_t)cb;
+        cb += (((uint64_t)m.n + m.m - 3 + narrow_b - 1) / narrow_b + 3) / 4;
+        plan->crowd_lds_bytes = std::max(plan->crowd_lds_bytes, ((size_t)m.m + 2 * (size_t)narrow_b) * sizeof(uint32_t));
+      }
+      plan->crowd_blocks = cb;
     } else {
       for (size_t i = 0; i < staged; i++) {
         SearchProblem &m = meta[i];
@@ -656,9 +688,10 @@
       meta[i].block_base = (uint32_t)ob;
       ob += ((uint64_t)meta[i].n + meta[i].m - 3 + kDiagsPerBlock - 1) / kDiagsPerBlock;
     }
-    if (blocks > 0x7FFFFFFFull || ob > 0x7FFFFFFFull)
+    if (blocks > 0x7FFFFFFFull || ob > 0x7FFFFFFFull || plan->crowd_blocks > 0x7FFFFFFFull)
       return Status::Make(NeedleError_InvalidArgument, "hamming_runs: too many problems for one launch");
     plan->staged = staged;
+    plan->crowded = crowded;
     plan->oversize_blocks = ob;
     plan->sampled = sampled;
     plan->mfma = mfma;
@@ -711,6 +744,8 @@
   plan->blocks = blocks;
   plan->seqs.assign(seqs, seqs + num_seqs);
   plan->problems.assign(problems, problems + num_problems);
+  plan->crowd.clear();
+  if (mode[8] == 2 && crowd) plan->crowd.assign(crowd, crowd + num_problems);
   std::memcpy(plan->mode, mode, sizeof(plan->mode));
   plan->valid = true;
   return Status::Ok();
@@ -739,6 +774,14 @@
 
 std::atomic<int32_t> g_last_form{0};
 std::atomic<uint64_t> g_last_products{0};
+std::atomic<uint32_t> g_last_crowded{0};
+
+int crowd_request() {
+  if (getenv("NEEDLE_HIP_SCAN_SHAPE") || getenv("NEEDLE_HIP_SPARSE_MAX")) return 0;
+  const char *e = getenv("NEEDLE_HIP_SCAN_CROWD");
+  if (!e) return 2;
+  return atoi(e) != 0 ? 1 : 0;
+}
 
 struct SearchWorkspace {
   DeviceBuffer<SearchProblem> problems;
@@ -769,31 +812,34 @@
 
 }
 
-void gpu_scan_last_launch(int32_t *form, uint64_t *matrix_products) {
+void gpu_scan_last_launch(int32_t *form, uint64_t *matrix_products, uint32_t *crowded_problems) {
   *form = g_last_form.load();
   *matrix_products = g_last_products.load();
+  if (crowded_problems) *crowded_problems = g_last_crowded.load();
 }
 
 Status gpu_hamming_runs_device(const uint32_t *d_hashes, const NeedleHipSeq *seqs, size_t num_seqs,
                                const NeedleHipProblem *problems, size_t num_problems, uint32_t threshold,
-                               NeedleHipRun *d_runs, uint32_t capacity, uint32_t *d_count, bool sync, bool count_is_zero) {
+                               NeedleHipRun *d_runs, uint32_t capacity, uint32_t *d_count, bool sync, bool count_is_zero,
+                               const uint8_t *crowd) {
   std::lock_guard<std::recursive_mutex> gpu_lock(gpu_mutex());
   Status s = ensure_device();
   if (!s.ok()) return s;
   hipStream_t stream = library_stream();
   if (!count_is_zero) NEEDLE_HIP_TRY(hipMemsetAsync(d_count, 0, sizeof(uint32_t), stream));
-  const int mode[8] = {getenv("NEEDLE_HIP_GENERIC_SEARCH") != nullptr, getenv("NEEDLE_HIP_BAND_SEARCH") != nullptr,
+  const int mode[9] = {getenv("NEEDLE_HIP_GENERIC_SEARCH") != nullptr, getenv("NEEDLE_HIP_BAND_SEARCH") != nullptr,
                        getenv("NEEDLE_HIP_BANDS_PER_WAVE") ? std::max(1, atoi(getenv("NEEDLE_HIP_BANDS_PER_WAVE"))) : 0,
                        threshold > 31u,
                        mfma_request(threshold),
                        getenv("NEEDLE_HIP_SEARCH_LDS_LIMIT") ? std::max(1, atoi(getenv("NEEDLE_HIP_SEARCH_LDS_LIMIT"))) : 160 * 1024,
                        mfma_waves(),
                        (getenv("NEEDLE_HIP_MFMA_SPLITS") ? std::max(1, std::min(64, atoi(getenv("NEEDLE_HIP_MFMA_SPLITS")))) : 0) |
-                           (getenv("NEEDLE_HIP_MFMA_SINGLE") ? 0x100 : 0) | (getenv("NEEDLE_HIP_MFMA_NO_IMAGES") ? 0x200 : 0)};
+                           (getenv("NEEDLE_HIP_MFMA_SINGLE") ? 0x100 : 0) | (getenv("NEEDLE_HIP_MFMA_NO_IMAGES") ? 0x200 : 0),
+                       crowd_request()};
   SearchWorkspace *ws = workspace();
   SearchPlan &plan = ws->plan;
-  const bool reuse = plan.matches(seqs, num_seqs, problems, num_problems, mode);
-  if (!reuse && !(s = build_plan(seqs, num_seqs, problems, num_problems, mode, &plan)).ok()) return s;
+  const bool reuse = plan.matches(seqs, num_seqs, problems, num_problems, mode, crowd);
+  if (!reuse && !(s = build_plan(seqs, num_seqs, problems, num_problems, mode, crowd, &plan)).ok()) return s;
   const std::vector<SearchProblem> &meta = plan.meta;
   const uint64_t blocks = plan.blocks;
   const size_t lds_bytes = plan.lds_bytes;
@@ -803,7 +849,7 @@
     if (!(reuse && ws->upload.resident_at == ws->problems.ptr && ws->problems.ptr) &&
         !(s = ws->upload.put(&ws->problems, &ws->stage, meta, stream)).ok())
       return s;
-    if (lds_bytes > 64 * 1024 && !ws->lds_attr_set) {
+    if (std::max(lds_bytes, plan.crowd_lds_bytes) > 64 * 1024 && !ws->lds_attr_set) {
       NEEDLE_HIP_TRY(hipFuncSetAttribute(reinterpret_cast<const void *>(hamming_runs_kernel<true>),
                                          hipFuncAttributeMaxDynamicSharedMemorySize, 160 * 1024));
       NEEDLE_HIP_TRY(hipFuncSetAttribute(reinterpret_cast<const void *>(hamming_runs_band_kernel<kBandR, kBandU>),
@@ -821,23 +867,37 @@
                                                hipFuncAttributeMaxDynamicSharedMemorySize, 160 * 1024));
           }
         }
+      NEEDLE_HIP_TRY(hipFuncSetAttribute(reinterpret_cast<const void *>(narrow_kernel<false>()),
+                                         hipFuncAttributeMaxDynamicSharedMemorySize, 160 * 1024));
+      NEEDLE_HIP_TRY(hipFuncSetAttribute(reinterpret_cast<const void *>(narrow_kernel<true>()),
+                                         hipFuncAttributeMaxDynamicSharedMemorySize, 160 * 1024));
       ws->lds_attr_set = true;
     }
     const int staged = (int)plan.staged, oversize = (int)(meta.size() - plan.staged);
     g_last_form.store(staged > 0 ? (sampled ? (plan.mfma ? 4 : 3) : fast ? 2 : 1) : 1);
     g_last_products.store(staged > 0 && plan.mfma ? plan.mfma_products : 0);
+    g_last_crowded.store((uint32_t)plan.crowded);
     if (staged > 0) {
       KernelTimer timer("hamming_runs");
-      if (sampled) {
+      const bool counting = getenv("NEEDLE_HIP_SCAN_COUNT") != nullptr;
+      if (counting && sampled && !ws->eval_groups) {
+        NEEDLE_HIP_TRY(hipMalloc((void **)&ws->eval_groups, 2 * sizeof(unsigned long long)));
+        NEEDLE_HIP_TRY(hipMemsetAsync(ws->eval_groups, 0, 2 * sizeof(unsigned long long), stream));
+      }
+      if (plan.crowded > 0) {
+        const int wide = staged - (int)plan.crowded;
+        hipLaunchKernelGGL(counting ? narrow_kernel<true>() : narrow_kernel<false>(), dim3((uint32_t)plan.crowd_blocks),
+                           dim3(256), plan.crowd_lds_bytes, stream, d_hashes, ws->problems.ptr + wide, (int)plan.crowded, threshold,
+                           d_runs, capacity, d_count, 1, -1, counting ? ws->eval_groups : (unsigned long long *)nullptr);
+      }
+      if (blocks == 0) {
+      } else if (sampled) {
         int sparse_max = -1;
         if (const char *e = getenv("NEEDLE_HIP_SPARSE_MAX")) sparse_max = std::max(0, atoi(e));
-        if (getenv("NEEDLE_HIP_SCAN_COUNT")) {
-          if (!ws->eval_groups) {
-            NEEDLE_HIP_TRY(hipMalloc((void **)&ws->eval_groups, 2 * sizeof(unsigned long long)));
-            NEEDLE_HIP_TRY(hipMemsetAsync(ws->eval_groups, 0, 2 * sizeof(unsigned long long), stream));
-          }
+        const int wide = staged - (int)plan.crowded;
+        if (counting) {
           hipLaunchKernelGGL(sampled_kernel<true>(scan_shape(), sparse_max >= 0), dim3((uint32_t)blocks), dim3(256), lds_bytes, stream, d_hashes,
-                             ws->problems.ptr, staged, threshold, d_runs, capacity, d_count, bands_per_wave, sparse_max,
+                             ws->problems.ptr, wide, threshold, d_runs, capacity, d_count, bands_per_wave, sparse_max,
                              ws->eval_groups);
         } else if (plan.mfma) {
           const uint32_t *images = nullptr;
@@ -865,7 +925,7 @@
 #endif
         } else {
           hipLaunchKernelGGL(sampled_kernel<false>(scan_shape(), sparse_max >= 0), dim3((uint32_t)blocks), dim3(256), lds_bytes, stream, d_hashes,
-                             ws->problems.ptr, staged, threshold, d_runs, capacity, d_count, bands_per_wave, sparse_max,
+                             ws->problems.ptr, wide, threshold, d_runs, capacity, d_count, bands_per_wave, sparse_max,
                              (unsigned long long *)nullptr);
         }
       }
diff --git a/rust/needle-hip/src/ffi.rs b/rust/needle-hip/src/ffi.rs
--- a/rust/needle-hip/src/ffi.rs
+++ b/rust/needle-hip/src/ffi.rs
@@ -197,6 +197,7 @@
     pub fn needle_hip_fingerprint_cert_stats(counts: *mut u64, reset: bool) -> NeedleError;
     pub fn needle_hip_scan_issued_evaluations(lane_evaluations: *mut u64, reset: bool) -> NeedleError;
     pub fn needle_hip_scan_last_launch(form: *mut i32, matrix_products: *mut u64) -> NeedleError;
+    pub fn needle_hip_scan_last_crowded(crowded_problems: *mut u32) -> NeedleError;
     pub fn needle_hip_epilogue_host_fallbacks(jobs: *mut u64, reset: bool) -> NeedleError;
     pub fn needle_hip_stream() -> *mut c_void;
     pub fn needle_hip_analyzer_run_pcm(
@@ -364,6 +365,7 @@
     ) -> NeedleError;
     pub fn needle_hip_library_job_comm_bytes(library: *const NeedleHipLibrary, slot: c_int, bytes: *mut u64) -> NeedleError;
     pub fn needle_hip_library_job_form(library: *const NeedleHipLibrary, slot: c_int, form: *mut u32) -> NeedleError;
+    pub fn needle_hip_library_job_crowded(library: *const NeedleHipLibrary, slot: c_int, crowded_problems: *mut u32) -> NeedleError;
     pub fn needle_hip_library_audit(library: *mut NeedleHipLibrary, audit: *mut NeedleHipCertAudit) -> NeedleError;
     pub fn needle_hip_host_threads() -> c_int;
     pub fn needle_hip_host_alloc(host_ptr: *mut *mut c_void, bytes: usize) -> NeedleError;
```

Result: no change. 715,500, median of 5 (+0.8%).
